# videosegmentation/video_segment

Measured on AMD Instinct MI355X. Metric: over-segmented frames/sec at 1080p, higher is better.
Workload: dtype f32

## Files before the change

include/vsg.h:

```cpp
#ifndef VSG_H_
#define VSG_H_

#include <stddef.h>
#include <stdint.h>

#ifdef __cplusplus
extern "C" {
#endif

#define VSG_OK 0
#define VSG_ERR_INVALID -1
#define VSG_ERR_DEVICE -2
#define VSG_ERR_STATE -3
#define VSG_ERR_INTERNAL -4

#define VSG_MEM_HOST 0
#define VSG_MEM_DEVICE 1

typedef struct vsg_stream vsg_stream;
typedef struct vsg_graph vsg_graph;

typedef struct vsg_options {
  int presmoothing;
  float frac_min_region_size;
  int chunk_size;
  float chunk_overlap_ratio;
  int num_constraint_frames;
  int enforce_n4_connectivity;
  int enforce_spatial_connectedness;
  int color_distance;
  int device;
  int two_stage_oversegment;
  int compute_vectorization;
} vsg_options;

typedef struct vsg_timings {
  float preprocess_ms;
  float edges_ms;
  float sort_ms;
  float merge_ms;
  float readout_ms;
  float host_post_ms;
  int64_t edges_total;
  int64_t edges_active;
  int64_t merges;
  int64_t preprocess_launches;
  int64_t edge_launches;
  float wave_kernel_ms;
  int64_t wave_kernel_launches;
  int64_t wave_kernel_edges;
  float filter_kernel_ms;
  int64_t filter_kernel_launches;
  float spine_kernel_ms;
  int64_t spine_kernel_launches;
  int64_t spine_kernel_edges;
} vsg_timings;

typedef struct vsg_diagnostics {
  double segment_wall_ms;
  double prepare_ms;
  double constrained_merge_ms;
  int64_t stages;
  int64_t optimistic_stages, rollbacks;
  int64_t slab_growths;
  double slab_growth_ms;
  int64_t spine_pool_growths;
  double spine_pool_growth_ms;
  int64_t runtime_mallocs;
  double runtime_malloc_ms;
  int64_t runtime_frees;
  double runtime_free_ms;
  int64_t cache_hits;
  int64_t device_syncs;
  double device_sync_ms;
  int64_t mail_waits;
  double mail_wait_ms;
  double mail_wait_longest_ms;
  int mail_mode;
} vsg_diagnostics;

typedef struct vsg_merge_paths {
  int64_t hub_stages;
  int64_t hub_absorbed;
  int64_t hub_cuts;
  int64_t hub_cuts_in_groups;
  int64_t hub_parts_in_later_bucket;
  int64_t spine_side_cuts;
  int64_t hub_retries;
  int64_t hub_reasons[6];
  int64_t hub_exclusion_reruns;
  int64_t hub_off_reruns;
  int64_t group_halvings;
  int64_t conservative_replays;
} vsg_merge_paths;

typedef struct vsg_spine_paths {
  int64_t replays;
  int64_t components;
  int64_t nested_replays;
  int64_t deepest_level;
  int64_t forest_rounds;
  int64_t forest_rounds_ahead;
  int64_t forest_compactions_ahead;
  int64_t forest_compactions_sync;
  int64_t forest_lists_refused;
  int64_t ranked_by_sampling;
  int64_t ranked_plain;
  int64_t rank_sampling_refused;
  int64_t jump_loops_ended_early;
  int64_t streamed_passes;
  int64_t streamed_refused;
  int64_t pool_fallbacks[4];
  int64_t top_level_fallbacks;
  int64_t nested_fallbacks;
  int64_t assumption_reruns;
  int64_t limit_bucket_moves;
  int64_t low_bucket_failures[2];
  int64_t low_bucket_skips[2];
  int64_t zero_pool_flips;
  int64_t windows_run;
  int64_t rle_stages;
  int64_t wide_launches;
  int64_t group_stages;
  int64_t sorts_hand;
  int64_t sorts_library;
} vsg_spine_paths;

typedef struct vsg_boundary_paths {
  int64_t halo_planes_in_pool;
} vsg_boundary_paths;

typedef struct vsg_memory_stats {
  int64_t bytes_in_use;
  int64_t bytes_in_use_peak;
  int64_t bytes_cached;
  int64_t limit_bytes;
  int64_t runtime_mallocs, runtime_frees, cache_hits, device_syncs;
  double runtime_malloc_ms, runtime_free_ms, device_sync_ms;
} vsg_memory_stats;
int vsg_device_memory_stats(int device, vsg_memory_stats* out);
int vsg_device_memory_trim(int device);
int vsg_device_memory_limit(int device, int64_t bytes);

const char* vsg_last_error(void);
int vsg_version(void);
void vsg_default_options(vsg_options* o);
int vsg_device_count(void);

int vsg_vectorize_id_image(const int32_t* ids, int width, int height, const uint8_t** data,
                           size_t* len);

int vsg_stream_create(const vsg_options* o, int width, int height, vsg_stream** out);
void vsg_stream_destroy(vsg_stream* s);
int vsg_stream_process_frame(vsg_stream* s, int flush, const uint8_t* bgr, size_t stride,
                             const float* flow, int has_flow_stream, int mem, int* num_results);
int vsg_stream_chunk_size(const vsg_stream* s);
int vsg_stream_result_bytes(vsg_stream* s, int i, const uint8_t** data, size_t* len);
int vsg_stream_result_id_image(vsg_stream* s, int i, int32_t* out);
int vsg_stream_last_merge_stats(const vsg_stream* s, int64_t* forced_regular_small);
int vsg_stream_keep_node_states(vsg_stream* s, int on);
int vsg_stream_last_node_states(const vsg_stream* s, int64_t* n, const int32_t** root, const float** mean,
                                const int32_t** size, const int32_t** constraint, const uint8_t** flags);
int vsg_stream_last_timings(const vsg_stream* s, vsg_timings* t);
int vsg_stream_last_diagnostics(const vsg_stream* s, vsg_diagnostics* d);
int vsg_stream_last_merge_paths(const vsg_stream* s, vsg_merge_paths* out);
int vsg_stream_last_spine_paths(const vsg_stream* s, vsg_spine_paths* out);
int vsg_stream_last_boundary_paths(const vsg_stream* s, vsg_boundary_paths* out);
int vsg_stream_last_smoothed(vsg_stream* s, float* out);

int vsg_stream_export_halo(vsg_stream* s, const int32_t** dev_labels_virtual,
                           const int32_t** dev_labels_constrained, int64_t scalars[4]);
int vsg_stream_import_halo(vsg_stream* s, const int32_t* labels_virtual,
                           const int32_t* labels_constrained, int mem, const int64_t scalars[4]);

int vsg_stream_expect_halo(vsg_stream* s);
int vsg_stream_restart(vsg_stream* s);

typedef struct vsg_chain vsg_chain;
int vsg_chain_create(int rank, int world, const char* id_file, uint64_t nonce, int device,
                     vsg_chain** out);
void vsg_chain_destroy(vsg_chain* c);
int vsg_chain_info(const vsg_chain* c, int* rank, int* world);
int vsg_chain_send_halo(vsg_chain* c, vsg_stream* from, int dst);
int vsg_chain_recv_halo(vsg_chain* c, vsg_stream* into, int src);
int vsg_chain_exchange_halo(vsg_chain* c, vsg_stream* from, int dst, vsg_stream* into, int src);

typedef struct vsg_regionseg vsg_regionseg;
typedef struct vsg_regionseg_options {
  int min_region_num;
  int max_region_num;
  float level_cutoff_fraction;
  float small_region_penalizer;
  int luminance_bins;
  int color_bins;
  int flow_bins;
  int chunk_set_size;
  int chunk_set_overlap;
  int constraint_chunks;
  int use_appearance;
  int use_flow;
  int use_size_penalizer;
  int compute_vectorization;
  int save_descriptors;
} vsg_regionseg_options;
void vsg_regionseg_default_options(vsg_regionseg_options* o);
int vsg_regionseg_create(const vsg_regionseg_options* o, int width, int height, vsg_regionseg** out);
void vsg_regionseg_destroy(vsg_regionseg* r);
int vsg_regionseg_process_frame(vsg_regionseg* r, int flush, const uint8_t* seg_desc, size_t seg_len,
                             const uint8_t* bgr, size_t stride, const float* flow, int* num_results);
int vsg_regionseg_result_bytes(vsg_regionseg* r, int i, const uint8_t** data, size_t* len);
int vsg_bgr_to_lab(const uint8_t* bgr, size_t stride, int width, int height, uint8_t* lab);

int vsg_graph_create(int width, int height, int max_frames, int l1, int device, vsg_graph** out);
void vsg_graph_destroy(vsg_graph* g);
int vsg_graph_add_frame_bgr(vsg_graph* g, const uint8_t* bgr, size_t stride, int presmoothing,
                            const int32_t* constraint_ids, int mem);
int vsg_graph_add_frame_features(vsg_graph* g, const float* feat, const int32_t* constraint_ids,
                                 int mem);
int vsg_graph_add_virtual_frame(vsg_graph* g, const int32_t* constraint_ids, int mem);
int vsg_graph_add_temporal(vsg_graph* g, const float* flow, int is_virtual, int mem);
int vsg_graph_add_frame_features_temporal(vsg_graph* g, const float* feat, const int32_t* constraint_ids,
                                          const float* flow, int is_virtual, int mem);
int vsg_graph_finish_building(vsg_graph* g);
int vsg_graph_segment_spatially(vsg_graph* g);
int vsg_graph_segment(vsg_graph* g, int min_region_size, int force_constraints);
int vsg_graph_obtain_results(vsg_graph* g, int use_flows, int enforce_n4,
                             int enforce_spatial_connectedness);
int vsg_graph_num_frames(const vsg_graph* g);
int vsg_graph_num_regions(const vsg_graph* g);
int64_t vsg_graph_num_neighbor_links(const vsg_graph* g);
int vsg_graph_region_sizes(const vsg_graph* g, int32_t* sizes, int32_t* constrained_ids);
int vsg_graph_index_image(const vsg_graph* g, int t, int32_t* out);
typedef struct vsg_region {
  int32_t index, size, constrained_id, first_frame, last_frame;
} vsg_region;
typedef struct vsg_interval {
  int32_t region_index, y, left_x, right_x;
} vsg_interval;
int vsg_graph_get_regions(vsg_graph* g, const vsg_region** regions, size_t* num_regions,
                          const int32_t** nbr_csr_ptr, const int32_t** nbr_csr_idx);
int vsg_graph_get_intervals(vsg_graph* g, int frame, const vsg_interval** intervals, size_t* n);
int vsg_graph_smoothed(vsg_graph* g, int t, float* out );
int vsg_graph_spatial_buckets(vsg_graph* g, int t, uint16_t* out );
int vsg_graph_temporal_buckets(vsg_graph* g, int t, uint16_t* out , int32_t* prev_idx);
int vsg_graph_list_slots(vsg_graph* g, int list, uint32_t* slots_out, int32_t* offsets_out);
// ... 23 lines not shown
```

video_segment_amd/_lib.py:

```python
import ctypes as C
import os
import subprocess

_HERE = os.path.dirname(os.path.abspath(__file__))
CSRC_DIR = os.path.join(_HERE, "csrc")
LIB_PATH = os.path.join(_HERE, "lib", "libvsg_hip.so")

VSG_OK = 0
VSG_ERR_INVALID, VSG_ERR_DEVICE, VSG_ERR_STATE, VSG_ERR_INTERNAL = -1, -2, -3, -4
VSG_MEM_HOST = 0
VSG_MEM_DEVICE = 1


class VsgOptions(C.Structure):
    _fields_ = [
        ("presmoothing", C.c_int),
        ("frac_min_region_size", C.c_float),
        ("chunk_size", C.c_int),
        ("chunk_overlap_ratio", C.c_float),
        ("num_constraint_frames", C.c_int),
        ("enforce_n4_connectivity", C.c_int),
        ("enforce_spatial_connectedness", C.c_int),
        ("color_distance", C.c_int),
        ("device", C.c_int),
        ("two_stage_oversegment", C.c_int),
        ("compute_vectorization", C.c_int),
    ]


class VsgTimings(C.Structure):
    _fields_ = [
        ("preprocess_ms", C.c_float),
        ("edges_ms", C.c_float),
        ("sort_ms", C.c_float),
        ("merge_ms", C.c_float),
        ("readout_ms", C.c_float),
        ("host_post_ms", C.c_float),
        ("edges_total", C.c_int64),
        ("edges_active", C.c_int64),
        ("merges", C.c_int64),
        ("preprocess_launches", C.c_int64),
        ("edge_launches", C.c_int64),
        ("wave_kernel_ms", C.c_float),
        ("wave_kernel_launches", C.c_int64),
        ("wave_kernel_edges", C.c_int64),
        ("filter_kernel_ms", C.c_float),
        ("filter_kernel_launches", C.c_int64),
        ("spine_kernel_ms", C.c_float),
        ("spine_kernel_launches", C.c_int64),
        ("spine_kernel_edges", C.c_int64),
    ]


class VsgDiagnostics(C.Structure):
    _fields_ = [
        ("segment_wall_ms", C.c_double), ("prepare_ms", C.c_double), ("constrained_merge_ms", C.c_double),
        ("stages", C.c_int64), ("optimistic_stages", C.c_int64), ("rollbacks", C.c_int64),
        ("slab_growths", C.c_int64), ("slab_growth_ms", C.c_double),
        ("spine_pool_growths", C.c_int64), ("spine_pool_growth_ms", C.c_double),
        ("runtime_mallocs", C.c_int64), ("runtime_malloc_ms", C.c_double),
        ("runtime_frees", C.c_int64), ("runtime_free_ms", C.c_double),
        ("cache_hits", C.c_int64), ("device_syncs", C.c_int64), ("device_sync_ms", C.c_double),
        ("mail_waits", C.c_int64), ("mail_wait_ms", C.c_double), ("mail_wait_longest_ms", C.c_double),
        ("mail_mode", C.c_int),
    ]

    def as_dict(self):
        return {k: getattr(self, k) for k, _ in self._fields_}


class VsgMergePaths(C.Structure):
    _fields_ = [
        ("hub_stages", C.c_int64), ("hub_absorbed", C.c_int64),
        ("hub_cuts", C.c_int64), ("hub_cuts_in_groups", C.c_int64), ("hub_parts_in_later_bucket", C.c_int64),
        ("spine_side_cuts", C.c_int64),
        ("hub_retries", C.c_int64), ("hub_reasons", C.c_int64 * 6),
        ("hub_exclusion_reruns", C.c_int64), ("hub_off_reruns", C.c_int64),
        ("group_halvings", C.c_int64), ("conservative_replays", C.c_int64),
    ]

    def as_dict(self):
        return {k: (list(getattr(self, k)) if k == "hub_reasons" else getattr(self, k)) for k, _ in self._fields_}


class VsgSpinePaths(C.Structure):
    _fields_ = [
        ("replays", C.c_int64), ("components", C.c_int64), ("nested_replays", C.c_int64),
        ("deepest_level", C.c_int64),
        ("forest_rounds", C.c_int64), ("forest_rounds_ahead", C.c_int64), ("forest_compactions_ahead", C.c_int64),
        ("forest_compactions_sync", C.c_int64), ("forest_lists_refused", C.c_int64),
        ("ranked_by_sampling", C.c_int64), ("ranked_plain", C.c_int64), ("rank_sampling_refused", C.c_int64),
        ("jump_loops_ended_early", C.c_int64), ("streamed_passes", C.c_int64), ("streamed_refused", C.c_int64),
        ("pool_fallbacks", C.c_int64 * 4), ("top_level_fallbacks", C.c_int64), ("nested_fallbacks", C.c_int64),
        ("assumption_reruns", C.c_int64), ("limit_bucket_moves", C.c_int64),
        ("low_bucket_failures", C.c_int64 * 2), ("low_bucket_skips", C.c_int64 * 2),
        ("zero_pool_flips", C.c_int64),
        ("windows_run", C.c_int64), ("rle_stages", C.c_int64), ("wide_launches", C.c_int64),
        ("group_stages", C.c_int64), ("sorts_hand", C.c_int64), ("sorts_library", C.c_int64),
    ]

    def as_dict(self):
        return {k: (list(getattr(self, k)) if issubclass(t, C.Array) else getattr(self, k)) for k, t in self._fields_}


class VsgBoundaryPaths(C.Structure):
    _fields_ = [
        ("halo_planes_in_pool", C.c_int64),
    ]

    def as_dict(self):
        return {k: getattr(self, k) for k, _ in self._fields_}


class VsgMemoryStats(C.Structure):
    _fields_ = [
        ("bytes_in_use", C.c_int64), ("bytes_in_use_peak", C.c_int64), ("bytes_cached", C.c_int64),
        ("limit_bytes", C.c_int64),
        ("runtime_mallocs", C.c_int64), ("runtime_frees", C.c_int64), ("cache_hits", C.c_int64),
        ("device_syncs", C.c_int64),
        ("runtime_malloc_ms", C.c_double), ("runtime_free_ms", C.c_double), ("device_sync_ms", C.c_double),
    ]

    def as_dict(self):
        return {k: getattr(self, k) for k, _ in self._fields_}


class VsgRegionOptions(C.Structure):
    _fields_ = [
        ("min_region_num", C.c_int), ("max_region_num", C.c_int),
        ("level_cutoff_fraction", C.c_float), ("small_region_penalizer", C.c_float),
        ("luminance_bins", C.c_int), ("color_bins", C.c_int), ("flow_bins", C.c_int),
        ("chunk_set_size", C.c_int), ("chunk_set_overlap", C.c_int), ("constraint_chunks", C.c_int),
        ("use_appearance", C.c_int), ("use_flow", C.c_int), ("use_size_penalizer", C.c_int),
        ("compute_vectorization", C.c_int), ("save_descriptors", C.c_int),
    ]


EXPORTED_SYMBOLS = [
    "vsg_last_error", "vsg_version", "vsg_default_options", "vsg_device_count",
    "vsg_device_memory_stats", "vsg_device_memory_trim", "vsg_device_memory_limit",
    "vsg_vectorize_id_image",
    "vsg_stream_create", "vsg_stream_destroy", "vsg_stream_process_frame", "vsg_stream_chunk_size",
    "vsg_stream_result_bytes", "vsg_stream_result_id_image", "vsg_stream_last_merge_stats",
    "vsg_stream_keep_node_states", "vsg_stream_last_node_states",
    "vsg_stream_last_timings", "vsg_stream_last_diagnostics", "vsg_stream_last_merge_paths", "vsg_stream_last_spine_paths",
    "vsg_stream_last_boundary_paths",
    "vsg_stream_last_smoothed", "vsg_stream_export_halo",
    "vsg_stream_import_halo", "vsg_stream_expect_halo", "vsg_stream_restart",
    "vsg_chain_create", "vsg_chain_destroy", "vsg_chain_info", "vsg_chain_send_halo",
    "vsg_chain_recv_halo", "vsg_chain_exchange_halo",
    "vsg_regionseg_default_options", "vsg_regionseg_create", "vsg_regionseg_destroy", "vsg_regionseg_process_frame",
    "vsg_regionseg_result_bytes", "vsg_bgr_to_lab",
    "vsg_graph_create", "vsg_graph_destroy", "vsg_graph_add_frame_bgr",
    "vsg_graph_add_frame_features", "vsg_graph_add_virtual_frame", "vsg_graph_add_temporal",
    "vsg_graph_add_frame_features_temporal", "vsg_graph_list_slots",
    "vsg_graph_finish_building", "vsg_graph_segment_spatially", "vsg_graph_segment", "vsg_graph_obtain_results",
    "vsg_graph_num_frames", "vsg_graph_num_regions", "vsg_graph_num_neighbor_links",
    "vsg_graph_region_sizes", "vsg_graph_index_image", "vsg_graph_get_regions",
    "vsg_graph_get_intervals", "vsg_graph_smoothed",
    "vsg_graph_spatial_buckets", "vsg_graph_temporal_buckets", "vsg_graph_node_roots",
    "vsg_graph_node_states",
    "vsg_graph_merge_stats", "vsg_graph_timings", "vsg_graph_diagnostics", "vsg_graph_merge_paths",
    "vsg_graph_spine_paths",
    "vsg_debug_sort_pairs", "vsg_debug_sort_pairs_timed", "vsg_debug_exclusive_sum", "vsg_debug_runs_of_sorted_keys",
]


def build(force=False):
    subprocess.check_call(["make", "-C", CSRC_DIR, "-j8", "-s"])
    return LIB_PATH


_lib = None


def lib():
    global _lib
    if _lib is not None:
        return _lib
    if not os.path.exists(LIB_PATH):
        raise RuntimeError(
            "libvsg_hip.so is missing (%s): build the HIP extension first; there is no fallback "
            "path" % LIB_PATH)
    try:
        import torch
    except ImportError:
        pass
    L = C.CDLL(LIB_PATH)
    vp = C.c_void_p
    L.vsg_last_error.restype = C.c_char_p
    L.vsg_version.restype = C.c_int
    L.vsg_default_options.argtypes = [C.POINTER(VsgOptions)]
    L.vsg_device_count.restype = C.c_int
    L.vsg_device_memory_stats.argtypes = [C.c_int, C.POINTER(VsgMemoryStats)]
    L.vsg_device_memory_trim.argtypes = [C.c_int]
    L.vsg_device_memory_limit.argtypes = [C.c_int, C.c_int64]
    L.vsg_vectorize_id_image.argtypes = [vp, C.c_int, C.c_int, C.POINTER(vp), C.POINTER(C.c_size_t)]
    L.vsg_stream_create.argtypes = [C.POINTER(VsgOptions), C.c_int, C.c_int, C.POINTER(vp)]
    L.vsg_stream_destroy.argtypes = [vp]
    L.vsg_stream_process_frame.argtypes = [vp, C.c_int, vp, C.c_size_t, vp, C.c_int, C.c_int,
                                           C.POINTER(C.c_int)]
    L.vsg_stream_chunk_size.argtypes = [vp]
    L.vsg_stream_result_bytes.argtypes = [vp, C.c_int, C.POINTER(vp), C.POINTER(C.c_size_t)]
    L.vsg_stream_result_id_image.argtypes = [vp, C.c_int, vp]
    L.vsg_stream_last_merge_stats.argtypes = [vp, vp]
    L.vsg_stream_keep_node_states.argtypes = [vp, C.c_int]
    L.vsg_stream_last_node_states.argtypes = [vp, C.POINTER(C.c_int64)] + [C.POINTER(vp)] * 5
    L.vsg_stream_last_timings.argtypes = [vp, C.POINTER(VsgTimings)]
    L.vsg_stream_last_diagnostics.argtypes = [vp, C.POINTER(VsgDiagnostics)]
    L.vsg_stream_last_merge_paths.argtypes = [vp, C.POINTER(VsgMergePaths)]
    L.vsg_stream_last_spine_paths.argtypes = [vp, C.POINTER(VsgSpinePaths)]
    L.vsg_stream_last_boundary_paths.argtypes = [vp, C.POINTER(VsgBoundaryPaths)]
    L.vsg_stream_last_smoothed.argtypes = [vp, vp]
    L.vsg_stream_export_halo.argtypes = [vp, C.POINTER(vp), C.POINTER(vp), vp]
    L.vsg_stream_import_halo.argtypes = [vp, vp, vp, C.c_int, vp]
    L.vsg_stream_expect_halo.argtypes = [vp]
    L.vsg_stream_restart.argtypes = [vp]
    L.vsg_chain_create.argtypes = [C.c_int, C.c_int, C.c_char_p, C.c_uint64, C.c_int, C.POINTER(vp)]
    L.vsg_chain_info.argtypes = [vp, C.POINTER(C.c_int), C.POINTER(C.c_int)]
    L.vsg_chain_exchange_halo.argtypes = [vp, vp, C.c_int, vp, C.c_int]
    L.vsg_chain_destroy.argtypes = [vp]
    L.vsg_chain_send_halo.argtypes = [vp, vp, C.c_int]
    L.vsg_chain_recv_halo.argtypes = [vp, vp, C.c_int]
    L.vsg_regionseg_default_options.argtypes = [C.POINTER(VsgRegionOptions)]
    L.vsg_regionseg_create.argtypes = [C.POINTER(VsgRegionOptions), C.c_int, C.c_int, C.POINTER(vp)]
    L.vsg_regionseg_destroy.argtypes = [vp]
    L.vsg_regionseg_process_frame.argtypes = [vp, C.c_int, vp, C.c_size_t, vp, C.c_size_t, vp, C.POINTER(C.c_int)]
    L.vsg_regionseg_result_bytes.argtypes = [vp, C.c_int, C.POINTER(vp), C.POINTER(C.c_size_t)]
    L.vsg_bgr_to_lab.argtypes = [vp, C.c_size_t, C.c_int, C.c_int, vp]
    L.vsg_debug_sort_pairs.argtypes = [vp, vp, C.c_int, C.c_int, vp, vp, C.c_int]
    L.vsg_debug_sort_pairs_timed.argtypes = [vp, vp, C.c_int, C.c_int, vp, vp, C.c_int, C.c_int, C.c_int,
# ... 63 lines not shown
```

video_segment_amd/csrc/capi.cpp:

```cpp
#include <algorithm>
#include <cstring>
#include <memory>
#include <string>
#include <vector>

#include <rccl/rccl.h>

#include <chrono>
#include <cstdio>
#include <fstream>
#include <thread>

#include "../../include/vsg.h"
#include "region_segmentation.h"
#include "scan_device.h"
#include "stream.h"

namespace {

thread_local std::string g_last_error;

template <class F>
int Guard(F&& f) {
  try {
    f();
    return VSG_OK;
  } catch (const vsg::Error& e) {
    g_last_error = e.what();
    return e.code;
  } catch (const std::exception& e) {
    g_last_error = e.what();
    return VSG_ERR_INTERNAL;
  }
}

class DeviceGuard {
 public:
  explicit DeviceGuard(int device) {
    if (device < 0) return;
    if (hipGetDevice(&prev_) != hipSuccess) return;
    if (prev_ != device) {
      VSG_HIP(hipSetDevice(device));
      changed_ = true;
    }
  }
  ~DeviceGuard() {
    if (changed_) (void)hipSetDevice(prev_);
  }
  DeviceGuard(const DeviceGuard&) = delete;
  DeviceGuard& operator=(const DeviceGuard&) = delete;

 private:
  int prev_ = -1;
  bool changed_ = false;
};

int ResolveDevice(int device) {
  if (device >= 0) return device;
  int cur = 0;
  VSG_HIP(hipGetDevice(&cur));
  return cur;
}

void RequireDevice(int device) {
  int n = 0;
  hipError_t e = hipGetDeviceCount(&n);
  if (e != hipSuccess || n <= 0) {
    vsg::Throw(VSG_ERR_DEVICE,
               "no usable HIP device (libvsg_hip has no CPU fallback): " +
                   std::string(e != hipSuccess ? hipGetErrorString(e) : "device count is 0"));
  }
  if (device >= n) vsg::Throw(VSG_ERR_DEVICE, "device ordinal out of range");
}

}

struct vsg_stream {
  int device = 0;
  std::unique_ptr<vsg::DenseSegmentationHip> impl;
  std::vector<int32_t> id_image;
};

struct vsg_regionseg {
  std::unique_ptr<vsg::RegionSegmentationHost> impl;
  int W = 0, H = 0;
};

struct vsg_graph {
  int device = 0;
  int W = 0, H = 0;
  size_t wh = 0;
  hipStream_t stream = nullptr;
  std::unique_ptr<vsg::DenseGraphHip> g;
  std::unique_ptr<vsg::Preprocessor> pre;
  std::vector<std::shared_ptr<vsg::DevBuf<float>>> feats;
  std::vector<std::shared_ptr<vsg::DevBuf<float>>> flows_dev;
  vsg::DevBuf<uint8_t> staging_bgr;
  vsg::DevBuf<float> staging_f32;
  vsg::DevBuf<int32_t> staging_ids;
  vsg_timings timings;
  std::vector<vsg_region> out_regions;
  std::vector<int32_t> out_nbr_ptr, out_nbr_idx;
  std::vector<vsg_interval> out_intervals;
  ~vsg_graph() {
    if (stream) (void)hipStreamSynchronize(stream);
    g.reset();
    pre.reset();
    if (stream) (void)hipStreamDestroy(stream);
  }
};

static void FillMergePaths(const vsg::MergePaths& mp, vsg_merge_paths* o) {
  std::memset(o, 0, sizeof(*o));
  o->hub_stages = mp.hub_stages;
  o->hub_absorbed = mp.hub_absorbed;
  o->hub_cuts = mp.hub_cuts;
  o->hub_cuts_in_groups = mp.hub_cuts_in_groups;
  o->hub_parts_in_later_bucket = mp.hub_parts_in_later_bucket;
  o->spine_side_cuts = mp.spine_side_cuts;
  o->hub_retries = mp.hub_retries;
  for (int q = 0; q < 6; ++q) o->hub_reasons[q] = mp.hub_reasons[q];
  o->hub_exclusion_reruns = mp.hub_exclusion_reruns;
  o->hub_off_reruns = mp.hub_off_reruns;
  o->group_halvings = mp.group_halvings;
  o->conservative_replays = mp.conservative_replays;
}

static void FillSpinePaths(const vsg::SpinePaths& sp, vsg_spine_paths* o) {
  std::memset(o, 0, sizeof(*o));
  o->replays = sp.replays;
  o->components = sp.components;
  o->nested_replays = sp.nested_replays;
  o->deepest_level = sp.deepest_level;
  o->forest_rounds = sp.forest_rounds;
  o->forest_rounds_ahead = sp.forest_rounds_ahead;
  o->forest_compactions_ahead = sp.forest_compactions_ahead;
  o->forest_compactions_sync = sp.forest_compactions_sync;
  o->forest_lists_refused = sp.forest_lists_refused;
  o->ranked_by_sampling = sp.ranked_by_sampling;
  o->ranked_plain = sp.ranked_plain;
  o->rank_sampling_refused = sp.rank_sampling_refused;
  o->jump_loops_ended_early = sp.jump_loops_ended_early;
  o->streamed_passes = sp.streamed_passes;
  o->streamed_refused = sp.streamed_refused;
  o->top_level_fallbacks = sp.top_level_fallbacks;
  o->nested_fallbacks = sp.nested_fallbacks;
  o->assumption_reruns = sp.assumption_reruns;
  o->limit_bucket_moves = sp.limit_bucket_moves;
  o->zero_pool_flips = sp.zero_pool_flips;
  o->windows_run = sp.windows_run;
  o->rle_stages = sp.rle_stages;
  o->wide_launches = sp.wide_launches;
  o->group_stages = sp.group_stages;
  o->sorts_hand = sp.sorts_hand;
  o->sorts_library = sp.sorts_library;
  for (int q = 0; q < 4; ++q) o->pool_fallbacks[q] = sp.pool_fallbacks[q];
  for (int q = 0; q < 2; ++q) {
    o->low_bucket_failures[q] = sp.low_bucket_failures[q];
    o->low_bucket_skips[q] = sp.low_bucket_skips[q];
  }
}

static void FillDiagnostics(const vsg::GraphTimings& gt, vsg_diagnostics* d) {
  std::memset(d, 0, sizeof(*d));
  d->segment_wall_ms = gt.segment_wall_ms;
  d->prepare_ms = gt.prepare_ms;
  d->constrained_merge_ms = gt.constrained_merge_ms;
  d->stages = gt.stages;
  d->optimistic_stages = gt.optimistic_stages;
  d->rollbacks = gt.rollbacks;
  d->slab_growths = gt.slab_growths;
  d->slab_growth_ms = gt.slab_growth_ms;
  d->spine_pool_growths = gt.spine_growths;
  d->spine_pool_growth_ms = gt.spine_growth_ms;
  d->runtime_mallocs = gt.runtime_mallocs;
  d->runtime_malloc_ms = gt.runtime_malloc_ms;
  d->runtime_frees = gt.runtime_frees;
  d->runtime_free_ms = gt.runtime_free_ms;
  d->cache_hits = gt.cache_hits;
  d->device_syncs = gt.device_syncs;
  d->device_sync_ms = gt.device_sync_ms;
  d->mail_waits = gt.mail_waits;
  d->mail_wait_ms = gt.mail_wait_ms;
  d->mail_wait_longest_ms = gt.mail_wait_longest_ms;
  d->mail_mode = gt.mail_mode;
}

extern "C" {

const char* vsg_last_error(void) { return g_last_error.c_str(); }

int vsg_device_memory_stats(int device, vsg_memory_stats* out) {
  return Guard([&] {
    VSG_REQUIRE(out, VSG_ERR_INVALID, "null argument");
    const int dev = ResolveDevice(device);
    const vsg::CacheStats s = vsg::CacheGetStats(dev);
    out->bytes_in_use = s.bytes_in_use;
    out->bytes_in_use_peak = s.bytes_in_use_peak;
    out->bytes_cached = s.bytes_cached;
    out->limit_bytes = s.limit_bytes;
    out->runtime_mallocs = s.runtime_mallocs;
    out->runtime_frees = s.runtime_frees;
    out->cache_hits = s.cache_hits;
    out->device_syncs = s.device_syncs;
    out->runtime_malloc_ms = s.runtime_malloc_ms;
    out->runtime_free_ms = s.runtime_free_ms;
    out->device_sync_ms = s.device_sync_ms;
  });
}

int vsg_device_memory_trim(int device) {
  return Guard([&] {
    const int dev = ResolveDevice(device);
    DeviceGuard dg(dev);
    vsg::CacheTrim(dev);
  });
}

int vsg_device_memory_limit(int device, int64_t bytes) {
  return Guard([&] {
    const int dev = ResolveDevice(device);
    DeviceGuard dg(dev);
    vsg::CacheSetLimit(dev, (long long)bytes);
  });
}
int vsg_version(void) { return 100; }

void vsg_default_options(vsg_options* o) {
  o->presmoothing = 2;
  o->frac_min_region_size = 0.01f;
  o->chunk_size = 20;
  o->chunk_overlap_ratio = 0.2f;
  o->num_constraint_frames = 1;
  o->enforce_n4_connectivity = 1;
  o->enforce_spatial_connectedness = 1;
  o->color_distance = 1;
  o->device = -1;
  o->two_stage_oversegment = 0;
  o->compute_vectorization = 0;
}

int vsg_device_count(void) {
  int n = 0;
  if (hipGetDeviceCount(&n) != hipSuccess) return 0;
  return n;
}

int vsg_vectorize_id_image(const int32_t* ids, int width, int height, const uint8_t** data,
                           size_t* len) {
  return Guard([&] {
    VSG_REQUIRE(ids && data && len && width >= 1 && height >= 1, VSG_ERR_INVALID, "bad argument");
    thread_local std::string wire;
    std::vector<std::pair<int32_t, vsg::Interval>> runs;
    for (int y = 0; y < height; ++y) {
      const int32_t* row = ids + (size_t)y * width;
      for (int x = 0; x < width;) {
        int x2 = x;
        while (x2 + 1 < width && row[x2 + 1] == row[x]) ++x2;
        VSG_REQUIRE(row[x] >= 0, VSG_ERR_INVALID, "negative region id");
        runs.emplace_back(row[x], vsg::Interval{y, x, x2});
        x = x2 + 1;
      }
    }
    std::stable_sort(runs.begin(), runs.end(),
                     [](const std::pair<int32_t, vsg::Interval>& a,
                        const std::pair<int32_t, vsg::Interval>& b) { return a.first < b.first; });
    vsg::SegDesc d;
    d.frame_width = width;
    d.frame_height = height;
    for (const auto& r : runs) {
      if (d.regions.empty() || d.regions.back().id != r.first) {
        d.regions.emplace_back();
        d.regions.back().id = r.first;
      }
      d.regions.back().raster.push_back(r.second);
    }
    for (auto& r : d.regions) vsg::MomentsFromRaster(r.raster, &r.moments);
// ... 940 lines not shown
```

video_segment_amd/csrc/dense_graph.cpp:

```cpp
#include "dense_graph.h"
#include "scan_device.h"

#include <algorithm>
#include <chrono>
#include <cmath>
#include <cstring>
#include <atomic>
#include <functional>
#include <thread>
#include <unordered_set>

namespace vsg {

namespace {
template <class T>
DevBuf<T>& Grow(DevBuf<T>& b, size_t n) {
  if (b.size() < n) b.alloc(n + n / 2 + 1024);
  return b;
}
double NowMs() {
  using clk = std::chrono::steady_clock;
  return std::chrono::duration<double, std::milli>(clk::now().time_since_epoch()).count();
}
template <class T>
// ... 326 lines not shown
  min_region_size_ = min_region_size;
  const int L = (int)lists_.size();
  const size_t N = wh_ * (size_t)num_frames_;
  const double t_enter = NowMs();
  const ThreadAllocCounters alloc0 = ThreadAllocSnapshot();
  MailWaitResetLongest();
  const MailWaitCounters mail0 = MailWaitSnapshot();
  int64_t diag_stages = 0, diag_slab_growths = 0, diag_spine_growths = 0, diag_hub_stages = 0, diag_hub_absorbed = 0;
  double diag_slab_ms = 0, diag_spine_ms = 0;

  std::vector<ListDesc> desc(L);
  list_slot_base_.assign(L + 1, 0);
  uint32_t acc = 0;
  int64_t edges_total = 0;
  for (int l = 0; l < L; ++l) {
    ListBuf& lb = lists_[l];
    list_slot_base_[l] = acc;
    ListDesc d = {};
    if (lb.used) {
      d.slots = lb.slots.get();
      d.kept = kept_all_.get() + acc;
      d.prev_idx = lb.type == 1 ? lb.prev_idx.get() : nullptr;
      d.offsets = (pass == 1 && lb.type == 1) ? nullptr : lb.offsets.get();
      d.type = lb.type;
      d.base_a = lb.base_a;
      d.base_b = lb.base_b;
      d.n = lb.n;
      acc += (uint32_t)lb.n;
    }
    desc[l] = d;
  }
  list_slot_base_[L] = acc;
  H2D(list_desc_dev_.get(), desc.data(), (size_t)L, stream_);
  H2D(list_slot_base_dev_.get(), list_slot_base_.data(), (size_t)L + 1, stream_);
  if (pass == 2) {
    kept_spatial_pass_.ensure(kept_all_.size());
    VSG_HIP(hipMemcpyAsync(kept_spatial_pass_.get(), kept_all_.get(), acc, hipMemcpyDeviceToDevice,
                           stream_));
  }
  VSG_HIP(hipMemsetAsync(kept_all_.get(), 0, acc, stream_));
  LaunchBuildBucketTable(list_desc_dev_.get(), L, bucket_base_dev_.get(), stream_);
  bucket_base_host_.resize((size_t)(kNumBuckets + 1) * (L + 1));
  D2H(bucket_base_host_.data(), bucket_base_dev_.get(), bucket_base_host_.size(), stream_);
  VSG_HIP(hipMemsetAsync(stats_.get(), 0, 96 * sizeof(unsigned long long), stream_));
  VSG_HIP(hipMemsetAsync(zero_pool_.base, 0, zero_pool_.cap * sizeof(int32_t), stream_));
  zero_pool_.used = 0;
  zero_pool_.second_half = false;
  zero_pool_.arena_used = 0;
  LaunchInitIdentity(cc_.get(), N, stream_);
  VSG_HIP(hipStreamSynchronize(stream_));

  const bool group_buckets = !getenv("VSG_GROUP_BUCKETS") || atoi(getenv("VSG_GROUP_BUCKETS")) != 0;
  std::vector<int32_t> bucket_prefix(kNumBuckets + 2, 0);
  int first_plain = kNumBuckets;
  {
    const float scale = 2048.0f / (1.0f + 1e-6f);
    const float inv_scale = (float)(1.0 / (double)scale);
    const float force_w = l1_ ? 0.002f : 0.001f;
    for (int b = 0; b < kNumBuckets; ++b) {
      if (!((float)b * inv_scale < force_w)) {
        first_plain = b;
        break;
      }
    }
  }
  int64_t n_max = 0;
  for (int b = 0; b <= kNumBuckets; ++b) {
    const int tot = bucket_base_host_[(size_t)b * (L + 1) + L];
    edges_total += tot;
    bucket_prefix[b + 1] = bucket_prefix[b] + tot;
  }
  for (int b = 0; b < kNumBuckets; ++b) n_max = std::max<int64_t>(n_max, bucket_prefix[b + 1] - bucket_prefix[b]);
  VSG_REQUIRE(bucket_prefix[kNumBuckets] >= 0, -1, "too many edges");
  EnsureScratch((size_t)std::max<int64_t>(n_max, 1));
  if (const char* e = getenv("VSG_ACTIVE_CAP")) {
    EnsureActiveScratch((size_t)std::max(1, atoi(e)));
  } else {
    EnsureActiveScratch(std::min<size_t>((size_t)std::max<int64_t>(n_max, 1),
                                         std::max<size_t>((size_t)n_max / 6, (size_t)1 << 20)));
  }
  bucket_prefix_dev_.ensure(bucket_prefix.size());
  H2D(bucket_prefix_dev_.get(), bucket_prefix.data(), bucket_prefix.size(), stream_);

  MergeScratch S = {};
  auto bind_scratch = [this, &S]() {
    S.e_ra = e_ra_.get();
    S.e_rb = e_rb_.get();
    S.e_gpos = e_gpos_.get();
    S.e_active = act_.e_active;
    S.e_apos = act_.e_apos;
    S.a_ra = act_.a_ra;
    S.a_rb = act_.a_rb;
    S.a_gpos = act_.a_gpos;
    S.a_comp = act_.a_comp;
    S.a_idx = act_.a_idx;
    S.s_comp = act_.s_comp;
    S.s_idx = act_.s_idx;
    S.seg_key = act_.seg_key;
    S.seg_cnt = act_.seg_cnt;
    S.seg_off = act_.seg_off;
    S.lead_pos = act_.lead_pos;
    S.l_ra = act_.l_ra;
    S.l_rb = act_.l_rb;
    S.l_gpos = act_.l_gpos;
    S.bk_ds = act_.bk_ds;
    S.bk_cons = act_.bk_cons;
    S.bk_flags = act_.bk_flags;
    S.cub_temp = cub_temp_.get();
    S.cub_temp_bytes = cub_temp_.size();
    S.scan = ScanScratch{scan_sums_.get(), stream_};
    S.active_cap = (int)std::min<size_t>(scratch_active_, 0x7fffffff);
  };
  bind_scratch();
  S.grow_active = [this, bind_scratch, &diag_slab_growths, &diag_slab_ms](long long need) {
    const double tg0 = NowMs();
    VSG_HIP(hipStreamSynchronize(stream_));
    VSG_HIP(hipStreamSynchronize(aux_stream_));
    VSG_HIP(hipStreamSynchronize(aux2_stream_));
    const size_t before = scratch_active_;
    EnsureActiveScratch((size_t)need);
    bind_scratch();
    ++diag_slab_growths;
    diag_slab_ms += NowMs() - tg0;
    if (getenv("VSG_DEBUG_STATS")) {
      std::fprintf(stderr, "[vsg] stage scratch: %zu -> %zu active edges (needed %lld), %.2f ms\n", before,
                   scratch_active_, need, NowMs() - tg0);
    }
    return true;
  };
  S.num_active = scalars_.get();
  S.num_segs = scalars_.get() + 1;
  S.node_key_bits = 1;
  while (S.node_key_bits < 32 && ((size_t)1 << S.node_key_bits) < N) ++S.node_key_bits;
  {
    const size_t words = 4 * ((scratch_edges_ + 255) / 256) + 4;
    S.masks.active = filter_masks_.get();
    S.masks.settled = filter_masks_.get() + words;
    S.masks.tentative = filter_masks_.get() + 2 * words;
    S.masks.block_cnt = block_cnt_.get();
    S.block_off = block_off_.get();
  }
  S.force_rollback = getenv("VSG_FORCE_ROLLBACK") ? 1 : 0;
  S.small_seg = getenv("VSG_SMALL_SEG") ? std::max(1, atoi(getenv("VSG_SMALL_SEG"))) : 24;
  S.wide_min = getenv("VSG_WIDE_MIN") ? atoi(getenv("VSG_WIDE_MIN")) : 0;
  S.wide_waves = getenv("VSG_WIDE_WAVES") ? atoi(getenv("VSG_WIDE_WAVES")) : 4;
  S.chain_relax = getenv("VSG_CHAIN_RELAX") ? atoi(getenv("VSG_CHAIN_RELAX")) : 1;
  const int hubs_default = getenv("VSG_HUBS") ? atoi(getenv("VSG_HUBS")) : 1;
  S.hubs = hubs_default;
  S.hub_excl = hub_excl_.get();
  S.hub_max_splits = getenv("VSG_HUB_SPLITS") ? std::max(0, atoi(getenv("VSG_HUB_SPLITS"))) : kHubMaxSplits;
  S.hub_cut_min_work = getenv("VSG_CUT_MIN_WORK") ? atoi(getenv("VSG_CUT_MIN_WORK")) : 0;
  S.hub_cut_ratio = getenv("VSG_CUT_RATIO") ? std::max(0, atoi(getenv("VSG_CUT_RATIO"))) : 1500;
  S.hub_check = (getenv("VSG_HUB_CHECK") && atoi(getenv("VSG_HUB_CHECK")) != 0) ? 1 : 0;
  VSG_HIP(hipMemsetAsync(hub8_.get(), 0, N, stream_));
  S.spine_min = getenv("VSG_SPINE_MIN") ? atoi(getenv("VSG_SPINE_MIN")) : 2048;
  if (S.spine_min > 0) S.spine_min = std::max(S.spine_min, S.small_seg + 2);
  {
    const double want = 1.15 * (double)wh_ * (double)capacity_frames_;
    const int by_graph = (int)std::min<double>(std::max<double>(want, 1 << 20), 120 << 20);
    S.spine_max_edges = getenv("VSG_SPINE_MAX_EDGES") ? atoi(getenv("VSG_SPINE_MAX_EDGES"))
                                                      : std::max(by_graph, spine_max_edges_grown_);
  }
  S.spine_off = 0;
  if (spine_limit_bucket_ != 0x7fffffff && ++spine_limit_age_ > 8) {
    spine_limit_bucket_ = 0x7fffffff;
    spine_limit_age_ = 0;
  }
  S.spine_limit_bucket = &spine_limit_bucket_;
  int spine_low_failed[2] = {0, 0}, spine_low_skip[2] = {0, 0};
  for (int b = 0; b < 2; ++b) {
    if (spine_low_cooldown_[b] > 0) {
      --spine_low_cooldown_[b];
      spine_low_skip[b] = 1;
      ++S.sp.low_bucket_skips[b];
    }
  }
  S.spine_low_failed = spine_low_failed;
  S.spine_low_skip = spine_low_skip;
  S.spine_nested_factor = getenv("VSG_SPINE_NESTED") ? std::max(1, atoi(getenv("VSG_SPINE_NESTED"))) : 1;
  S.spine_debug = getenv("VSG_SPINE_DEBUG") ? 1 : 0;
  S.spine_check = getenv("VSG_SPINE_CHECK") ? 1 : 0;
  S.rank_split_min = getenv("VSG_RANK_SPLIT_MIN") ? atoi(getenv("VSG_RANK_SPLIT_MIN")) : (1 << 20);
  S.spine_fast = getenv("VSG_SPINE_FAST") ? atoi(getenv("VSG_SPINE_FAST")) : 2;
  S.spine_fast_min = getenv("VSG_SPINE_FAST_MIN") ? atoi(getenv("VSG_SPINE_FAST_MIN")) : 32768;
  if (S.spine_min > 0) {
    const size_t ints = SpinePoolInts((size_t)S.spine_max_edges);
    if (spine_pool_.size() < ints) spine_pool_.alloc(ints);
  }
  S.spine_pool = spine_pool_.get();
  S.spine_pool_ints = spine_pool_.size();
  S.grow_spine_pool = [this, &S, &diag_spine_growths, &diag_spine_ms](long long edges) {
    if (getenv("VSG_SPINE_MAX_EDGES") || edges >= (120ll << 20)) return false;
    const long long want = std::min<long long>(edges + edges / 8, 120ll << 20);
    const long long nodes = (long long)wh_ * (long long)std::max(capacity_frames_, 1);
    const size_t ints = SpinePoolInts((size_t)want) + (size_t)(29 * std::min(want, nodes));
    if (ints <= spine_pool_.size()) return false;
    const double tg0 = NowMs();
    size_t free_b = 0, total_b = 0;
    VSG_HIP(hipMemGetInfo(&free_b, &total_b));
    if (free_b + spine_pool_.size() * sizeof(int32_t) < 2 * ints * sizeof(int32_t)) {
      int dev = 0;
      VSG_HIP(hipGetDevice(&dev));
      CacheTrim(dev);
      VSG_HIP(hipMemGetInfo(&free_b, &total_b));
      if (free_b + spine_pool_.size() * sizeof(int32_t) < 2 * ints * sizeof(int32_t)) return false;
    }
    VSG_HIP(hipStreamSynchronize(stream_));
    VSG_HIP(hipStreamSynchronize(aux_stream_));
    VSG_HIP(hipStreamSynchronize(aux2_stream_));
    spine_pool_.alloc(ints);
    ++diag_spine_growths;
    diag_spine_ms += NowMs() - tg0;
    S.spine_pool = spine_pool_.get();
    S.spine_pool_ints = spine_pool_.size();
    S.spine_max_edges = (int)want;
    spine_max_edges_grown_ = S.spine_max_edges;
    return true;
  };
  S.nmap[0] = label_uf_.get();
  S.nmap[1] = label_img_.get();
  S.nmap[2] = adjust_.get();
  S.aux_stream = aux_stream_;
  S.aux2_stream = aux2_stream_;
  S.aux_fork = aux_fork_;
  S.aux_join = aux_join_;
  S.use_rle = getenv("VSG_RLE") ? atoi(getenv("VSG_RLE")) : 1;
  S.wave_dbg = getenv("VSG_WAVE_DBG") ? atoi(getenv("VSG_WAVE_DBG")) : 0;
  S.wave_debug = (S.wave_dbg != 0 || getenv("VSG_DEBUG_STAGES") || getenv("VSG_DEBUG_STATS")) ? 1 : 0;
  optimistic_stages_ = 0;
  rollbacks_ = 0;
  S.optimistic_stages = &optimistic_stages_;
  S.rollbacks = &rollbacks_;
  S.cc = cc_.get();
  S.stats = stats_.get();
  ev_used_ = 0;
  ev_wave_.clear();
  ev_filter_.clear();
  ev_spine_.clear();
  S.ev_pool = &ev_pool_;
  S.ev_wave = &ev_wave_;
  S.ev_filter = &ev_filter_;
  S.ev_spine = &ev_spine_;
  S.ev_used = &ev_used_;
  S.mail = &mail_;
  S.zeros = &zero_pool_;
  S.main_stream = stream_;

  MergeParams P;
  P.spatial_survivors = pass == 2 ? kept_spatial_pass_.get() : nullptr;
  P.W = W_;
  P.H = H_;
  P.num_lists = L;
  P.min_region_size = min_region_size;
  P.force_merge_weight = l1_ ? 0.002f : 0.001f;
  const float scale = 2048.0f / (1.0f + 1e-6f);
  P.inv_scale = (float)(1.0 / (double)scale);
  auto largest_s = [](double t, bool inclusive) {
    auto ok = [&](float s) {
      const double r = (double)std::sqrt(s);
      return inclusive ? r <= t : r < t;
    };
    float s = (float)(t * t);
    while (!ok(s)) s = std::nextafter(s, 0.0f);
    while (ok(std::nextafter(s, 10.0f))) s = std::nextafter(s, 10.0f);
    return s;
  };
  P.s_lt_005 = largest_s((double)0.05f, false);
  P.s_lt_02 = largest_s(0.2, false);
  P.s_le_015 = largest_s((double)0.15f, true);

  const double t0 = NowMs();
  int inert_mode = has_constraints_ ? 2 : 1;
  if (const char* e = getenv("VSG_INERT_MODE")) inert_mode = std::min(inert_mode, atoi(e));
  const bool debug_stages = getenv("VSG_DEBUG_STAGES") != nullptr;
  const double frame_ratio = (double)W_ * (double)H_ / (1920.0 * 1080.0);
  const int default_windows = std::max(6, std::min(12, (int)std::lround(6.0 * frame_ratio)));
  const int num_windows = getenv("VSG_WINDOWS") ? std::max(1, atoi(getenv("VSG_WINDOWS"))) : default_windows;
  const int window_bushy = getenv("VSG_WINDOW_BUSHY") ? atoi(getenv("VSG_WINDOW_BUSHY")) : 64;
  const bool adapt_windows = !getenv("VSG_ADAPT_WINDOWS") || atoi(getenv("VSG_ADAPT_WINDOWS")) != 0;
  const int window_min_edges =
      getenv("VSG_WINDOW_MIN") ? atoi(getenv("VSG_WINDOW_MIN")) : (int)std::min<size_t>(2 * wh_, 1u << 30);
  const int window_min_replayed =
      getenv("VSG_WINDOW_MIN_REPLAYED") ? atoi(getenv("VSG_WINDOW_MIN_REPLAYED"))
                                        : (getenv("VSG_WINDOW_MIN") ? 0 : (int)std::min<size_t>(wh_ / 2, 1u << 30));
  S.bucket_prefix = bucket_prefix_dev_.get();
  S.bucket_prefix_host = bucket_prefix.data();
  {
    list_off_host_.assign((size_t)L * (kNumBuckets + 2), 0);
    for (int l = 0; l < L; ++l) {
      int32_t* off = list_off_host_.data() + (size_t)l * (kNumBuckets + 2);
      int acc_l = 0;
      for (int b = 0; b <= kNumBuckets; ++b) {
        off[b] = acc_l;
        const int32_t* row = bucket_base_host_.data() + (size_t)b * (L + 1);
        acc_l += row[l + 1] - row[l];
      }
      off[kNumBuckets + 1] = acc_l;
    }
    const size_t cap = (size_t)3 * 65536;
    if (seg_table_dev_.size() < cap) seg_table_dev_.alloc(cap);
    S.filter_segs_mode = getenv("VSG_FILTER_SEGS") ? atoi(getenv("VSG_FILTER_SEGS")) : 2;
    S.bucket_base_host = S.filter_segs_mode == 0 ? nullptr : bucket_base_host_.data();
    S.lists_host = desc.data();
    S.list_off_host = list_off_host_.data();
    S.list_slot_base_host = list_slot_base_.data();
    S.seg_dev = seg_table_dev_.get();
// ... 104 lines not shown
      return want;
    };
    const bool big_enough = n_b >= (1 << 18);
    int pos = 0;
    for (int w = 0; w < windows && pos < n_b; ++w) {
      const int j1 = (int)((int64_t)n_b * (w + 1) / windows);
      if (j1 <= pos) continue;
      const bool probe = windows > 1 && w == 0 && window_bushy > 0;
      bool rest_mode = false;
      while (pos < j1) {
        bool limited = false;
        const int take = (int)limit(j1 - pos, &limited);
        const StageInfo info = run(w, pos, take,
                                   probe ? 2 : ((big_enough && (limited || windows == 1)) ||
                                                wave_target_active_ != kNoWindowTarget) ? 1 : 0, limited);
        pos += take;
        if (probe && ((int64_t)info.replayed >= (int64_t)window_bushy * std::max(info.components, 1) ||
                      info.replayed < (int64_t)window_min_replayed * take / std::max(j1, 1))) {
          rest_mode = true;
        }
      }
      if (rest_mode) {
        const int64_t rest_default = std::min<int64_t>(
            119ll << 20, std::max<int64_t>(16ll << 20, (int64_t)(1.4 * (double)wh_ * (double)capacity_frames_)));
        const int64_t rest_cap = getenv("VSG_REST_CAP") ? atoll(getenv("VSG_REST_CAP")) : rest_default;
        const int64_t rest_n = (int64_t)n_b - pos;
        const int pieces = (int)std::max<int64_t>(1, (rest_n + rest_cap - 1) / rest_cap);
        const int64_t piece = (rest_n + pieces - 1) / pieces;
        for (int q = 0; pos < n_b; ++q) {
          bool limited = false;
          const int take = (int)limit(std::min<int64_t>(piece, n_b - pos), &limited);
          run(-1 - q, pos, take, big_enough ? 1 : 0, limited);
          pos += take;
        }
      }
    }
    window_target_[b] = wave_target_active_;
    if (hub_bucket_stages_[b] > 0 && hub_bucket_absorbed_[b] < hub_bucket_stages_[b]) hub_bucket_pause_[b] = 8;
    if (debug_stages && wave_target_active_ != kNoWindowTarget) {
      std::fprintf(stderr, "[vsg]   bucket %d leaves target %lld (frozen %d, unpaid %d, last %d, peak %d)\n", b,
                   (long long)wave_target_active_, (int)window_frozen_[b], (int)window_unpaid_[b], window_last_seg_[b],
                   window_peak_[b]);
    }
    if (b >= first_plain) {
      if (group_active < 2048) {
        group_width = std::min(group_width * 4, 512);
      } else if (group_active > 16384) {
        group_width = std::max(group_width / 4, 1);
      }
    }
  }
  for (int b = 0; b < 2; ++b) {
    if (++spine_low_cost_age_[b] > 64) {
      spine_low_cost_age_[b] = 0;
      spine_low_cost_fail_[b] = spine_low_cost_skip_[b] = 0;
    }
    if (spine_low_skip[b]) {
      spine_low_cost_skip_[b] = low_bucket_ms[b];
      if (spine_low_cost_fail_[b] > 0 && spine_low_cost_skip_[b] >= spine_low_cost_fail_[b]) spine_low_cooldown_[b] = 0;
      continue;
    }
    if (spine_low_failed[b]) spine_low_cost_fail_[b] = low_bucket_ms[b];
    spine_low_fails_[b] = spine_low_failed[b] ? spine_low_fails_[b] + 1 : 0;
    if (spine_low_fails_[b] >= 2) {
      spine_low_fails_[b] = 0;
      if (spine_low_cost_skip_[b] <= 0) {
        spine_low_cooldown_[b] = 1;
      } else if (spine_low_cost_skip_[b] < spine_low_cost_fail_[b]) {
        spine_low_cooldown_[b] = 8;
      }
    }
  }
  timings_.optimistic_stages = optimistic_stages_;
  timings_.rollbacks = rollbacks_;
  LaunchKeepVirtualBucket(list_desc_dev_.get(), L, stream_);
  ResetHubExclusions(S, nodes(), stream_);
  VSG_HIP(hipStreamSynchronize(stream_));
  const double t_buckets = NowMs();
  if (getenv("VSG_DEBUG_HASH")) DebugHash("after buckets");
  if (force_constraints && has_constraints_) MergeConstrainedHostAssisted();
  if (getenv("VSG_DEBUG_HASH")) DebugHash("after constrained merge");
  const double t_mc = NowMs();
  if (getenv("VSG_DEBUG_STATS")) {
    std::fprintf(stderr, "[vsg] segment: buckets %.1f ms, merge-constrained %.1f ms\n",
                 t_buckets - t0, t_mc - t_buckets);
  }
  unsigned long long st[80] = {0};
  D2H(st, stats_.get(), 80, stream_);
  VSG_HIP(hipStreamSynchronize(stream_));
  if (st[23] != 0) {
    std::fprintf(stderr, "[vsg] chain self check: %llu mismatches\n", st[23]);
    throw Error(-4 , "merge worker: the chain self check found mismatches");
  }
  if (st[22] != 0) throw Error(-4 , "merge worker: a batch did not converge");
  if (getenv("VSG_DEBUG_STATS")) {
    std::fprintf(stderr, "[vsg] wave: edges %llu batches %llu rounds %llu generic %llu (solo %llu) chain %llu "
                 "cuts %llu; optimistic stages %lld rollbacks %lld\n",
                 st[3], st[7], st[5], st[4], st[6], st[20], st[21], (long long)optimistic_stages_,
                 (long long)rollbacks_);
    std::fprintf(stderr, "[vsg] hubs: %lld stages used hub regions, %lld regions absorbed through them, %lld stages cut at an edge, %lld redone "
                 "(broken %lld, inherit %lld, shape %lld, marked %lld, pair %lld, split %lld)\n",
                 (long long)diag_hub_stages, (long long)diag_hub_absorbed, S.hub_splits, S.hub_retries, S.hub_reasons[0],
                 S.hub_reasons[1], S.hub_reasons[2], S.hub_reasons[3], S.hub_reasons[4], S.hub_reasons[5]);
    std::fprintf(stderr, "[vsg] wide: edges %llu batches %llu (%.1f lanes each) rounds %llu (%.1f per batch), chain lanes %llu, "
                 "kept-lane iterations %llu; kcyc per batch: staging %.1f rounds %.1f (%.2f per round)\n",
                 st[31], st[45], (double)st[72] / std::max(1.0, (double)st[45]), st[44],
                 (double)st[44] / std::max(1.0, (double)st[45]), st[73], st[74],
                 st[46] / 1e3 / std::max(1.0, (double)st[45]), st[47] / 1e3 / std::max(1.0, (double)st[45]),
                 st[47] / 1e3 / std::max(1.0, (double)st[44]));
  }
  timings_.merge_ms = (float)(NowMs() - t0);
  for (auto& pr : ev_wave_) {
    float ms = 0;
    VSG_HIP(hipEventElapsedTime(&ms, ev_pool_[pr.first], ev_pool_[pr.second]));
    timings_.wave_ms += ms;
  }
  for (auto& pr : ev_filter_) {
    float ms = 0;
    VSG_HIP(hipEventElapsedTime(&ms, ev_pool_[pr.first], ev_pool_[pr.second]));
    timings_.filter_ms += ms;
  }
  for (auto& pr : ev_spine_) {
    float ms = 0;
    VSG_HIP(hipEventElapsedTime(&ms, ev_pool_[pr.first], ev_pool_[pr.second]));
    timings_.spine_ms += ms;
  }
  timings_.spine_launches += (int64_t)ev_spine_.size();
  timings_.spine_edges += (int64_t)st[24];
  timings_.wave_launches += (int64_t)ev_wave_.size();
  timings_.filter_launches += (int64_t)ev_filter_.size();
  timings_.wave_edges += (int64_t)st[3];
  timings_.edges_active += (int64_t)st[3];
  timings_.edges_total = edges_total;
  timings_.merges[0] += (int64_t)st[0];
  timings_.merges[1] += (int64_t)st[1];
  timings_.merges[2] += (int64_t)st[2];
  {
    const ThreadAllocCounters a1 = ThreadAllocSnapshot();
    const MailWaitCounters m1 = MailWaitSnapshot();
    timings_.stages = diag_stages;
    MergePaths& mp = timings_.paths;
    mp = MergePaths();
    mp.hub_stages = diag_hub_stages;
    mp.hub_absorbed = diag_hub_absorbed;
    mp.hub_cuts = S.hub_splits;
    mp.hub_cuts_in_groups = S.hub_cuts_in_groups;
    mp.hub_parts_in_later_bucket = S.hub_parts_in_later_bucket;
    mp.spine_side_cuts = S.spine_side_cuts;
    mp.hub_retries = S.hub_retries;
    for (int q = 0; q < 6; ++q) mp.hub_reasons[q] = S.hub_reasons[q];
    mp.hub_exclusion_reruns = S.hub_exclusion_reruns;
    mp.hub_off_reruns = S.hub_off_reruns;
    mp.group_halvings = S.group_halvings;
    mp.conservative_replays = S.conservative_replays;
    timings_.spine_paths = S.sp;
    timings_.slab_growths = diag_slab_growths;
    timings_.slab_growth_ms = diag_slab_ms;
    timings_.spine_growths = diag_spine_growths;
    timings_.spine_growth_ms = diag_spine_ms;
    timings_.runtime_mallocs = a1.runtime_mallocs - alloc0.runtime_mallocs;
    timings_.runtime_malloc_ms = a1.runtime_malloc_ms - alloc0.runtime_malloc_ms;
    timings_.runtime_frees = a1.runtime_frees - alloc0.runtime_frees;
    timings_.runtime_free_ms = a1.runtime_free_ms - alloc0.runtime_free_ms;
    timings_.cache_hits = a1.cache_hits - alloc0.cache_hits;
    timings_.device_syncs = a1.device_syncs - alloc0.device_syncs;
    timings_.device_sync_ms = a1.device_sync_ms - alloc0.device_sync_ms;
    timings_.mail_waits = m1.waits - mail0.waits;
    timings_.mail_wait_ms = m1.wait_ms - mail0.wait_ms;
    timings_.mail_wait_longest_ms = m1.longest_ms;
    timings_.mail_mode = MailYieldMode();
    timings_.prepare_ms = t0 - t_enter;
    timings_.constrained_merge_ms = t_mc - t_buckets;
    timings_.segment_wall_ms = NowMs() - t_enter;
  }
}

namespace {
struct SimRegion {
  int parent;
  float d[3];
  int sz, cons, flags;
  bool dirty;
};
}

void DenseGraphHip::DebugHash(const char* where) {
  const size_t N = wh_ * (size_t)num_frames_;
  std::vector<int32_t> parent(N), cons(N);
  std::vector<float4> ds(N);
  std::vector<uint8_t> flags(N);
  D2H(parent.data(), parent_.get(), N, stream_);
  D2H(cons.data(), cons_.get(), N, stream_);
  D2H(ds.data(), desc_sz_.get(), N, stream_);
  D2H(flags.data(), flags_.get(), N, stream_);
  VSG_HIP(hipStreamSynchronize(stream_));
  auto fnv = [](uint64_t h, const void* p, size_t n) {
    const uint8_t* b = static_cast<const uint8_t*>(p);
    for (size_t i = 0; i < n; ++i) { h ^= b[i]; h *= 1099511628211ull; }
    return h;
  };
  std::vector<int32_t> root(N), canon(N, -1);
  uint64_t h_part = 1469598103934665603ull, h_root = h_part, h_state = h_part, h_cons = h_part;
  int next = 0, nroots = 0;
  for (size_t i = 0; i < N; ++i) {
    int r = (int)i;
    while (parent[(size_t)r] != r) r = parent[(size_t)r];
    root[i] = r;
    if (canon[(size_t)r] < 0) canon[(size_t)r] = next++;
    const int32_t c = canon[(size_t)r];
    h_part = fnv(h_part, &c, 4);
    h_root = fnv(h_root, &r, 4);
  }
  for (size_t i = 0; i < N; ++i) {
    if (parent[i] != (int)i) continue;
    ++nroots;
    h_state = fnv(h_state, &ds[i], 16);
    h_state = fnv(h_state, &flags[i], 1);
    h_cons = fnv(h_cons, &cons[i], 4);
  }
  std::fprintf(stderr, "[vsg] hash %s: roots %d partition %016llx root-ids %016llx states %016llx cons %016llx\n",
               where, nroots, (unsigned long long)h_part, (unsigned long long)h_root,
               (unsigned long long)h_state, (unsigned long long)h_cons);
}

void DenseGraphHip::MergeConstrainedHostAssisted() {
  const int N = (int)(wh_ * (size_t)num_frames_);
  std::vector<std::pair<int, int>> vranges;
  for (int t : virtual_slices_) vranges.emplace_back((int)(wh_ * t), (int)(wh_ * (t + 1)));
  std::sort(vranges.begin(), vranges.end());
  std::vector<std::pair<int, int>> nvranges;
  int cursor = 0;
  for (auto& vr : vranges) {
    if (vr.first > cursor) nvranges.emplace_back(cursor, vr.first);
    cursor = vr.second;
  }
  if (cursor < N) nvranges.emplace_back(cursor, N);

  int32_t* d_flags = label_uf_.get();
  int32_t* d_vals = label_img_.get();
  int32_t* d_offs = adjust_.get();
  struct Runs {
    std::vector<int32_t> node, value;
  };
  auto collect = [&](int begin, int end, Runs* out) {
    const int n = end - begin;
    if (n <= 0) return;
    LaunchConstrainedRuns(nodes(), begin, end, d_vals, d_flags, stream_);
    ExclusiveSum(ScanScratch{scan_sums_.get()}, d_flags, d_offs, n, stream_);
    int last_off = 0, last_flag = 0;
    D2H(&last_off, d_offs + (n - 1), 1, stream_);
    D2H(&last_flag, d_flags + (n - 1), 1, stream_);
    VSG_HIP(hipStreamSynchronize(stream_));
    const int k = last_off + last_flag;
    const size_t old = out->node.size();
    if (k > 0) {
      EnsureActiveScratch((size_t)k);
      LaunchCompactIndexValue(d_flags, d_offs, d_vals, n, act_.a_ra, act_.a_rb, stream_);
      out->node.resize(old + k);
      out->value.resize(old + k);
      D2H(out->node.data() + old, act_.a_ra, (size_t)k, stream_);
      D2H(out->value.data() + old, act_.a_rb, (size_t)k, stream_);
      VSG_HIP(hipStreamSynchronize(stream_));
      for (size_t i = old; i < old + (size_t)k; ++i) out->node[i] += begin;
    }
    out->node.push_back(end);
    out->value.push_back(-1);
  };

  const double tm0 = NowMs();
  Runs nv, vr;
  for (auto& r : nvranges) collect(r.first, r.second, &nv);
  for (auto& r : vranges) collect(r.first, r.second, &vr);
  const double tm1 = NowMs();

  std::vector<int32_t> ids;
  {
    std::unordered_set<int32_t> seen;
    for (const Runs* v : {&nv, &vr}) {
      for (int32_t r : v->value) {
        if (r >= 0 && seen.insert(r).second) ids.push_back(r);
      }
    }
    std::sort(ids.begin(), ids.end());
  }
  const int m = (int)ids.size();
  if (m == 0) return;
  small_i32_a_.ensure((size_t)m);
  small_i32_b_.ensure((size_t)m);
  small_i32_c_.ensure((size_t)m);
  small_f4_.ensure((size_t)m);
  H2D(small_i32_a_.get(), ids.data(), (size_t)m, stream_);
  LaunchGatherStates(nodes(), small_i32_a_.get(), m, small_f4_.get(), small_i32_b_.get(),
                     small_i32_c_.get(), stream_);
  std::vector<float4> h_ds(m);
  std::vector<int32_t> h_cons(m), h_flags(m);
  D2H(h_ds.data(), small_f4_.get(), (size_t)m, stream_);
  D2H(h_cons.data(), small_i32_b_.get(), (size_t)m, stream_);
  D2H(h_flags.data(), small_i32_c_.get(), (size_t)m, stream_);
  VSG_HIP(hipStreamSynchronize(stream_));

  const double tm2 = NowMs();
  std::unordered_map<int, SimRegion> sim;
  sim.reserve((size_t)m * 2);
  for (int i = 0; i < m; ++i) {
    SimRegion r;
    r.parent = ids[i];
// ... 769 lines not shown
```

video_segment_amd/csrc/dense_graph.h:

```cpp
#ifndef VSG_DENSE_GRAPH_H_
#define VSG_DENSE_GRAPH_H_

#include <memory>
#include <unordered_map>
#include <vector>

#include "device_graph.h"
#include "host_model.h"

namespace vsg {

struct MergePaths {
  int64_t hub_stages = 0, hub_absorbed = 0;
  int64_t hub_cuts = 0, hub_cuts_in_groups = 0, hub_parts_in_later_bucket = 0, spine_side_cuts = 0;
  int64_t hub_retries = 0, hub_reasons[6] = {0, 0, 0, 0, 0, 0};
  int64_t hub_exclusion_reruns = 0, hub_off_reruns = 0, group_halvings = 0, conservative_replays = 0;
};

struct GraphTimings {
  float edges_ms = 0, sort_ms = 0, merge_ms = 0, readout_ms = 0, host_post_ms = 0;
  int64_t edges_total = 0, edges_active = 0;
  int64_t merges[3] = {0, 0, 0};
  float wave_ms = 0, filter_ms = 0, spine_ms = 0;
  int64_t wave_launches = 0, filter_launches = 0, wave_edges = 0, spine_launches = 0, spine_edges = 0;
  int64_t optimistic_stages = 0, rollbacks = 0;
  int64_t stages = 0;
  int64_t slab_growths = 0, spine_growths = 0;
  double slab_growth_ms = 0, spine_growth_ms = 0;
  int64_t runtime_mallocs = 0, runtime_frees = 0, cache_hits = 0, device_syncs = 0;
  double runtime_malloc_ms = 0, runtime_free_ms = 0, device_sync_ms = 0;
  int64_t mail_waits = 0;
  double mail_wait_ms = 0, mail_wait_longest_ms = 0;
  int mail_mode = 0;
  double segment_wall_ms = 0, prepare_ms = 0, constrained_merge_ms = 0;
  MergePaths paths;
  SpinePaths spine_paths = {};
};

class DenseGraphHip {
 public:
  DenseGraphHip(int W, int H, int max_frames, bool l1, hipStream_t stream);
  ~DenseGraphHip();

  int W() const { return W_; }
  int H() const { return H_; }
  int max_frames() const { return max_frames_; }
  int num_frames() const { return num_frames_; }
  hipStream_t stream() const { return stream_; }
  hipStream_t aux_stream() const { return aux_stream_; }

  void Reset(int max_frames);
  void ForgetLearned();

  void AddFrame(const float* feat_planar_dev, const int32_t* cons_dev);
  void AddVirtualFrame(const int32_t* ids_dev, int max_label);
  void AddVirtualFrameDeferred();
  void SetHaloLabels(const int32_t* virtual_ids_dev, const int32_t* constrained_ids_dev,
                     int max_label);
  bool halo_pending() const { return halo_pending_; }
  void AddTemporal(const float* cur_dev, const float* prev_dev, const float* flow_dev,
                   bool is_virtual);
  void AddFrameAndTemporal(const float* feat_planar_dev, const int32_t* cons_dev, const float* prev_dev,
                           const float* flow_dev, bool is_virtual);
  void FinishBuilding();
  void Segment(int min_region_size, bool force_constraints) {
    SegmentLists(min_region_size, force_constraints, spatial_pass_done_ ? 2 : 0);
  }
  void SegmentSpatially() {
    SegmentLists(0, false, 1);
    spatial_pass_done_ = true;
  }
  void ObtainResults(const std::vector<const float*>* dev_flows, bool enforce_n4,
                     bool enforce_spatial_connectedness);

  std::vector<RegionInfo>& regions() { return regions_; }
  const std::vector<RegionInfo>& regions() const { return regions_; }
  const GraphTimings& timings() const { return timings_; }

  void CopySpatialBuckets(int t, uint16_t* out_host);
  void CopyTemporalBuckets(int t, uint16_t* out_host, int32_t* prev_idx_host);
  void CopyNodeRoots(int32_t* out_host);
  int CopyListSlots(int list, uint32_t* slots_host, int32_t* offsets_host);
  void CopyNodeStates(int32_t* root, float* mean, int32_t* size, int32_t* cons, uint8_t* flags);

 private:
  struct ListBuf {
    DevBuf<uint32_t> slots;
    DevBuf<int32_t> offsets;
    DevBuf<int32_t> prev_idx;
    DevBuf<uint16_t> keys_dbg;
    int type = 0;
    int n = 0;
    int base_a = 0, base_b = 0;
    bool used = false;
  };

  void EnsureScratch(size_t n_edges_max);
  void EnsureActiveScratch(size_t n_active_max);
  void DebugHash(const char* where);
  ListBuf& PrepareSpatialList(const float* feat, const int32_t* cons_dev);
  ListBuf& PrepareTemporalList(const float* cur, const float* prev, const float* flow, bool is_virtual);
  EdgeSortList SortEntry(ListBuf& lb, int per_px);
  void MergeConstrainedHostAssisted();
  NodeArrays nodes() {
    return NodeArrays{parent_.get(), desc_sz_.get(), cons_.get(), flags_.get(), hub8_.get()};
  }

  QuiesceGuard quiesce_;
  int W_, H_, capacity_frames_, max_frames_;
  bool l1_;
  hipStream_t stream_;
  hipStream_t aux_stream_ = nullptr;
  hipStream_t aux2_stream_ = nullptr;
  hipEvent_t aux_fork_ = nullptr, aux_join_ = nullptr;
  int num_frames_ = 0;
  size_t wh_;
  bool has_constraints_ = false;
  std::vector<int> virtual_slices_;
  int min_region_size_ = 0;
  bool flattened_ = false;

  DevBuf<int32_t> parent_;
  DevBuf<float4> desc_sz_;
  DevBuf<int32_t> cons_;
  DevBuf<uint8_t> flags_;
  DevBuf<uint8_t> hub8_;
  DevBuf<int32_t> cc_, label_uf_, label_img_, adjust_;
  std::vector<ListBuf> lists_;
  DevBuf<ListDesc> list_desc_dev_;
  DevBuf<uint32_t> list_slot_base_dev_;
  std::vector<uint32_t> list_slot_base_;
  DevBuf<uint8_t> kept_all_;
  DevBuf<uint8_t> kept_spatial_pass_;
  bool spatial_pass_done_ = false;
  bool halo_pending_ = false;
  int deferred_virtual_slice_ = -1, deferred_constrained_slice_ = -1;
  void SegmentLists(int min_region_size, bool force_constraints, int pass);
  void RunStageDebug(int b, int w, int windows, int j0, int n, const MergeParams& P, int inert_mode,
                     MergeScratch& S, bool debug_stages, StageInfo* info);
  DevBuf<int32_t> bucket_base_dev_;
  std::vector<int32_t> bucket_base_host_;
  DevBuf<uint16_t> keys_tmp_[2];
  DevBuf<int32_t> hist_tmp_[2], hist_chunk_[2];
  DevBuf<int32_t> first_label_scratch_;
  DevBuf<int32_t> e_ra_, e_rb_;
  DevBuf<uint32_t> e_gpos_;
  DevBuf<uint8_t> active_slab_;
  struct ActiveArrays {
    int32_t *e_active = nullptr, *e_apos = nullptr, *a_ra = nullptr, *a_rb = nullptr, *seg_cnt = nullptr,
            *seg_off = nullptr, *lead_pos = nullptr, *l_ra = nullptr, *l_rb = nullptr, *bk_cons = nullptr;
    uint32_t *a_gpos = nullptr, *a_comp = nullptr, *a_idx = nullptr, *s_comp = nullptr, *s_idx = nullptr,
             *seg_key = nullptr, *l_gpos = nullptr;
    float4* bk_ds = nullptr;
    uint8_t* bk_flags = nullptr;
  } act_;
  DevBuf<unsigned long long> filter_masks_;
  DevBuf<int32_t> block_cnt_, block_off_;
  int64_t optimistic_stages_ = 0, rollbacks_ = 0;
  DevBuf<int32_t> scalars_;
  DevBuf<int32_t> seg_table_dev_;
  DevBuf<int32_t> hub_excl_;
  PinnedBuf<int32_t> iv_host_;
  std::vector<int32_t> seg_table_host_, list_off_host_;
  size_t stage_ring_used_ = 0;
  PinnedBuf<int32_t> stage_ring_;
  Mailbox mail_;
  void* mail_mem_ = nullptr;
  DevBuf<int32_t> zero_pool_mem_;
  ZeroPool zero_pool_;
// ... 54 lines not shown
```

video_segment_amd/csrc/device_graph.h:

```cpp
#ifndef VSG_DEVICE_GRAPH_H_
#define VSG_DEVICE_GRAPH_H_

#include <functional>

#include "common.h"

namespace vsg {

constexpr uint8_t kFlagFinalized = 1;
constexpr uint8_t kFlagNoDesc = 2;
constexpr uint8_t kFlagTentative = 4;
constexpr uint8_t kFlagHub = 8;
constexpr uint8_t kFlagHubBroken = 16;
constexpr uint8_t kFlagHubExcluded = 32;
constexpr int kHubExclCap = 16384;
constexpr int kHubMaxAttempts = 4;
constexpr int kHubMaxSplits = 64;
constexpr int kHubCutCap = 64;
constexpr int kHubListInts = 4 + kHubExclCap + 3 * kHubCutCap;

struct NodeArrays {
  int32_t* parent;
  float4* desc_sz;
  int32_t* cons;
  uint8_t* flags;
  uint8_t* hub8;
};

struct ListDesc {
  const uint32_t* slots;
  uint8_t* kept;
  const int32_t* prev_idx;
  const int32_t* offsets;
  int32_t type;
  int32_t base_a;
  int32_t base_b;
  int32_t n;
};

struct MergeParams {
  int W, H;
  int num_lists;
  int min_region_size;
  float force_merge_weight;
  float inv_scale;
  float s_lt_005, s_lt_02, s_le_015;
  const uint8_t* spatial_survivors;
};

void UploadSpaceWeights(const float* w49, hipStream_t stream);
void LaunchMinMax(const uint8_t* bgr, size_t stride, int W, int H, int* mm, hipStream_t s);
void LaunchBilateral(const uint8_t* bgr, size_t stride, int W, int H, const float* lut,
                     float scale, float* planes, hipStream_t s);
void LaunchGaussian3(const uint8_t* bgr, size_t stride, int W, int H, float k0, float k1, float* planes,
                     hipStream_t s);
void LaunchConvertPlanar(const uint8_t* bgr, size_t stride, int W, int H, float* planes,
                         hipStream_t s);
void LaunchInterleavedToPlanar(const float* in, size_t n, float* planes, hipStream_t s);
void LaunchPlanarToInterleaved(const float* planes, size_t n, float* out, hipStream_t s);
size_t EdgeSortHistInts(size_t n_px, int per_px);
size_t EdgeSortChunkInts(size_t n_px, int per_px);
struct EdgeSortList {
  const uint16_t* keys;
  int32_t* hist;
  int32_t* chunk;
  int32_t* offsets;
  uint32_t* slots;
  int per_px;
};
constexpr int kEdgeSortMaxLists = 2;
void LaunchSpatialKeys(const float* feat, int W, int H, int l1, uint16_t* keys, int32_t* hist,
                       hipStream_t s);
void LaunchTemporalKeys(const float* cur, const float* prev, const float* flow, int W, int H,
                        int l1, int is_virtual, uint16_t* keys, int32_t* prev_idx, int32_t* hist,
                        hipStream_t s);
void LaunchBucketSort(const EdgeSortList* lists, int n_lists, size_t n_px, hipStream_t s);
void LaunchInitNodes(const float* feat, size_t n, int base, const int32_t* cons_in,
                     NodeArrays nodes, hipStream_t s);
void LaunchInitVirtualNodes(const int32_t* labels, size_t n, int base, int num_labels,
                            int32_t* first_scratch, NodeArrays nodes, hipStream_t s);

constexpr int kScanMaxTiles = 4096;
struct ScanScratch {
  int32_t* sums;
  hipStream_t owner = nullptr;
};

void DebugExclusiveSum(const ScanScratch& sc, const int32_t* in, int32_t* out, int n, int32_t* total, hipStream_t s);

size_t SortPairsU32HandTempBytes(int n);
void SortPairsU32Hand(void* temp, size_t temp_bytes, const uint32_t* keys_in, uint32_t* keys_out,
                      const uint32_t* vals_in, uint32_t* vals_out, int n, int end_bit, hipStream_t s);
size_t SortPairsU32LibTempBytes(int n);
void SortPairsU32Lib(void* temp, size_t temp_bytes, const uint32_t* keys_in, uint32_t* keys_out,
                     const uint32_t* vals_in, uint32_t* vals_out, int n, int end_bit, hipStream_t s);
size_t SortPairsU32TempBytes(int n);
void SortPairsU32(void* temp, size_t temp_bytes, const uint32_t* keys_in, uint32_t* keys_out,
                  const uint32_t* vals_in, uint32_t* vals_out, int n, int end_bit, hipStream_t s);
bool SortPairsU32TakesHand(int n);
size_t SortKeysU64TempBytes(int n);
void SortKeysU64(void* temp, size_t temp_bytes, const unsigned long long* in,
                 unsigned long long* out, int n,
                 hipStream_t s);
size_t UniqueU64TempBytes(int n);
void UniqueU64(void* temp, size_t temp_bytes, const unsigned long long* in,
               unsigned long long* out,
               int32_t* num_out, int n, hipStream_t s);

constexpr int kMailValues = 4;
struct MailSlot {
  unsigned long long* dev;
  volatile unsigned long long* host;
  unsigned seq;
};
struct Mailbox {
  unsigned long long* dev = nullptr;
  volatile unsigned long long* host = nullptr;
  int slots = 0;
  int next = 0;
  unsigned seq = 0;
  int32_t* list_dev = nullptr;
  volatile int32_t* list_host = nullptr;
  int list_cap = 0;
};
inline MailSlot NextMail(Mailbox& m) {
  MailSlot s{m.dev + (size_t)kMailValues * m.next, m.host + (size_t)kMailValues * m.next, ++m.seq};
  m.next = (m.next + 1) % m.slots;
  return s;
}
void MailWait(const MailSlot& slot, int count, int* values, hipStream_t s);
void MailRegisterGraph(int delta);
int MailYieldMode();
struct MailWaitCounters {
  long long waits = 0;
  double wait_ms = 0, longest_ms = 0;
};
MailWaitCounters MailWaitSnapshot();
void MailWaitResetLongest();
void LaunchMailPost(const MailSlot& slot, const int32_t* p0, const int32_t* p1, const int32_t* p2,
                    const int32_t* p3, hipStream_t s);

constexpr size_t kZeroArenaInts = 1024;
struct ZeroPool {
  int32_t* base = nullptr;
  size_t cap = 0, used = 0;
  bool second_half = false;
  size_t arena_used = 0;
};

struct FilterMasks {
  unsigned long long* active;
  unsigned long long* settled;
  unsigned long long* tentative;
  int32_t* block_cnt;
};
struct FilterSegRec {
  const uint32_t* slots;
  const int32_t* prev;
  int32_t start, pos0, type, base_a, base_b;
  uint32_t slot_base;
};
constexpr int kFilterArgSegs = 64;
struct FilterSegArgs {
  FilterSegRec r[kFilterArgSegs];
};
struct FilterSegs {
  const FilterSegRec* rec;
  int n;
};
constexpr size_t kStageRingInts = (size_t)1 << 18;
struct SpinePaths {
  int64_t replays, components, nested_replays, deepest_level;
  int64_t forest_rounds, forest_rounds_ahead, forest_compactions_ahead, forest_compactions_sync, forest_lists_refused;
  int64_t ranked_by_sampling, ranked_plain, rank_sampling_refused;
  int64_t jump_loops_ended_early, streamed_passes, streamed_refused;
  int64_t pool_fallbacks[4], top_level_fallbacks, nested_fallbacks;
  int64_t assumption_reruns, limit_bucket_moves, low_bucket_failures[2], low_bucket_skips[2];
  int64_t zero_pool_flips;
  int64_t windows_run, rle_stages, wide_launches, group_stages, sorts_hand, sorts_library;
};
struct MergeScratch {
  int active_cap;
  std::function<bool(long long need)> grow_active;
  int32_t* e_ra;
  int32_t* e_rb;
  uint32_t* e_gpos;
  int32_t* e_active;
  int32_t* e_apos;
  FilterMasks masks;
  int32_t* block_off;
  int32_t* a_ra;
  int32_t* a_rb;
  uint32_t* a_gpos;
  uint32_t* a_comp;
  uint32_t* a_idx;
  uint32_t* s_comp;
  uint32_t* s_idx;
  uint32_t* seg_key;
  int32_t* seg_cnt;
  int32_t* seg_off;
  int32_t* num_active;
  int32_t* num_segs;
  float4* bk_ds;
  int32_t* bk_cons;
  uint8_t* bk_flags;
  int force_rollback;
  int32_t* lead_pos;
  int32_t* l_ra;
  int32_t* l_rb;
  uint32_t* l_gpos;
  int use_rle;
  int group_hi;
  const int32_t* bucket_prefix;
  const int32_t* bucket_prefix_host;
  const int32_t* bucket_base_host;
  const int32_t* list_off_host;
  int32_t* seg_dev;
  size_t seg_cap;
  std::vector<int32_t>* seg_host;
  const ListDesc* lists_host;
  int filter_segs_mode;
  int32_t* ring_host;
  size_t ring_cap, *ring_used;
  int spine_min;
  int spine_off;
  int* spine_low_failed;
  const int* spine_low_skip;
  int* spine_limit_bucket;
  int spine_nested_factor;
  int spine_max_edges;
  int spine_debug, spine_check;
  int rank_split_min;
  int spine_fast;
  int spine_fast_min;
  int32_t* spine_pool;
  size_t spine_pool_ints;
  std::function<bool(long long edges)> grow_spine_pool;
  int32_t* nmap[3];
  hipStream_t aux_stream;
  hipStream_t aux2_stream;
  hipEvent_t aux_fork, aux_join;
  int small_seg;
  int wide_min;
  int wide_waves;
  int chain_relax;
  int hubs;
  int hubs_off;
  int hub_attempt;
  int hub_splits_left;
  int hub_split_depth;
  int hub_list_dirty;
  int hub_max_splits;
  int hub_cut_min_work;
  long long hub_splits;
  const uint32_t* list_slot_base_host;
  int32_t* hub_excl;
  long long hub_retries;
  long long hub_reasons[6];
  long long hub_cuts_in_groups;
  long long hub_parts_in_later_bucket;
  long long spine_side_cuts;
  long long hub_exclusion_reruns;
  long long hub_off_reruns;
  long long group_halvings;
  long long conservative_replays;
  long long hub_cut_ratio;
  int hub_check;
  SpinePaths sp;
  int wave_debug;
  int wave_dbg;
  int64_t* optimistic_stages;
  int64_t* rollbacks;
  int32_t* cc;
  unsigned long long* stats;
  void* cub_temp;
  size_t cub_temp_bytes;
  ScanScratch scan;
  int node_key_bits;
  std::vector<hipEvent_t>* ev_pool;
  std::vector<std::pair<int, int>>* ev_wave;
  std::vector<std::pair<int, int>>* ev_filter;
  std::vector<std::pair<int, int>>* ev_spine;
  int* ev_used;
  Mailbox* mail;
  ZeroPool* zeros;
  hipStream_t main_stream;
};
int32_t* TakeZeroed(MergeScratch& S, size_t n);

int32_t* TakeStageScalars(MergeScratch& S, size_t n);

int32_t* TakeStageRing(MergeScratch& S, size_t n);

void LaunchBuildBucketTable(const ListDesc* lists, int num_lists, int32_t* bucket_base,
                            hipStream_t s);
void LaunchInitIdentity(int32_t* a, size_t n, hipStream_t s);
struct StageInfo {
  int want_components = 0;
  int replayed = 0;
  int components = 0;
  int max_wave_segment = 0;
  int hub_stages = 0;
  long long hub_absorbed = 0;
  int hub_retries = 0;
};
void ResetHubExclusions(MergeScratch& S, NodeArrays nodes, hipStream_t s);
void RunBucketStage(int bucket, int j0, int n_b, const ListDesc* lists, const int32_t* bucket_base,
                    const uint32_t* list_slot_base, uint8_t* kept_all, NodeArrays nodes,
                    const MergeParams& P, int inert_mode, MergeScratch& S, hipStream_t s,
                    StageInfo* info = nullptr);
size_t SpinePoolInts(size_t max_edges);
void LaunchKeepVirtualBucket(const ListDesc* lists, int num_lists, hipStream_t s);

void LaunchFlatten(NodeArrays nodes, size_t n, int32_t* label_uf, hipStream_t s);
void LaunchEnforceN4(int32_t* label_img, int W, int H, const int32_t* frames_dev, int num_frames,
                     int32_t* row_flags , int32_t* adjust ,
                     hipStream_t s);
void LaunchRowRunCounts(const int32_t* label_img, int W, int H, const int32_t* frames_dev, int num_frames,
                        int32_t* row_counts , hipStream_t s);
struct IntervalArrays {
  int32_t* label;
  uint32_t* ty;
  int32_t* lx;
  int32_t* rx;
};
void LaunchWriteIntervals(const int32_t* label_img, int W, int H, const int32_t* frames_dev, int num_frames,
                          const int32_t* row_offsets ,
                          IntervalArrays out, hipStream_t s);
void LaunchRelabelIntervals(const uint32_t* ty, const int32_t* lx, const int32_t* rx,
                            const int32_t* new_label, int n, int W, int H, int32_t* label_uf,
                            hipStream_t s);
struct PairTable {
  unsigned long long* key;
  unsigned long long* order;
  unsigned mask;
};
void LaunchNeighborPairsHashed(const ListDesc* lists, int num_lists, const int32_t* label_uf, int W,
                               PairTable table, int32_t* distinct, hipStream_t s);
void LaunchPairTableCompact(PairTable table, unsigned long long* pairs, unsigned long long* order_keys,
                            int32_t* out_count, hipStream_t s);
void LaunchNeighborPairs(const ListDesc* lists, int num_lists, const int32_t* label_uf, int W,
                         unsigned long long* pairs, unsigned long long* order_keys,
                         int32_t* count, int capacity, hipStream_t s);
void LaunchGatherStates(NodeArrays nodes, const int32_t* ids, int n, float4* desc_sz_out,
                        int32_t* cons_out, int32_t* flags_out, hipStream_t s);
void LaunchScatterStates(NodeArrays nodes, const int32_t* ids, int n, const int32_t* parent_in,
                         const float4* desc_sz_in, const int32_t* cons_in, const int32_t* flags_in,
                         hipStream_t s);
void LaunchConstrainedRoots(NodeArrays nodes, int begin, int end, int32_t* flag_out,
                            int32_t* root_out, hipStream_t s);
void LaunchConstrainedRuns(NodeArrays nodes, int begin, int end, int32_t* value_out,
                           int32_t* flag_out, hipStream_t s);
void LaunchCompactI32(const int32_t* flags, const int32_t* offsets, const int32_t* values, int n,
                      int32_t* out, hipStream_t s);
void LaunchGatherI32(const int32_t* src, const int32_t* idx, int n, int32_t* out, hipStream_t s);
void LaunchGatherFlow(const int32_t* req, int n, const float* const* flows, int W, float2* out,
                      hipStream_t s);

void LaunchNonzeroFlags(const int32_t* a, int n, int32_t* flags, hipStream_t s);
void LaunchCompactIndexValue(const int32_t* flags, const int32_t* offsets, const int32_t* values,
                             int n, int32_t* out_idx, int32_t* out_val, hipStream_t s);
void LaunchFirstOrderOfKeys(const unsigned long long* pairs, const unsigned long long* order_keys,
                            int m, const int32_t* keys_sorted, int num_keys,
                            unsigned long long* out_min, hipStream_t s);

}

#endif
```

video_segment_amd/csrc/merge_stage.hip:

```cpp
#include <sched.h>
#include <time.h>

#include <algorithm>
#include <atomic>
#include <chrono>
#include <cstring>
#include <thread>
#include <type_traits>
#include <vector>

#include "merge_common.h"
#include "scan_device.h"

namespace vsg {

__global__ __launch_bounds__(256) void k_build_bucket_table(const ListDesc* __restrict__ lists,
                                                             int num_lists,
                                                             int32_t* __restrict__ bucket_base) {
  const int b = blockIdx.x * 256 + threadIdx.x;
  if (b > kNumBuckets) return;
  int acc = 0;
  int32_t* row = bucket_base + (size_t)b * (num_lists + 1);
  for (int l = 0; l < num_lists; ++l) {
    row[l] = acc;
// ... 12 lines not shown

__global__ __launch_bounds__(256) void k_init_identity(int32_t* a, size_t n) {
  const size_t i = (size_t)blockIdx.x * 256 + threadIdx.x;
  if (i < n) a[i] = (int32_t)i;
}

void LaunchInitIdentity(int32_t* a, size_t n, hipStream_t s) {
  hipLaunchKernelGGL(k_init_identity, dim3((unsigned)((n + 255) / 256)), dim3(256), 0, s, a, n);
  VSG_HIP(hipGetLastError());
}

__global__ void k_mail_post(unsigned long long* slot, unsigned seq, const int32_t* p0, const int32_t* p1,
                            const int32_t* p2, const int32_t* p3) {
  if (p0) MailPost(slot, seq, 0, *p0);
  if (p1) MailPost(slot, seq, 1, *p1);
  if (p2) MailPost(slot, seq, 2, *p2);
  if (p3) MailPost(slot, seq, 3, *p3);
}

void LaunchMailPost(const MailSlot& slot, const int32_t* p0, const int32_t* p1, const int32_t* p2,
                    const int32_t* p3, hipStream_t s) {
  hipLaunchKernelGGL(k_mail_post, dim3(1), dim3(1), 0, s, slot.dev, slot.seq, p0, p1, p2, p3);
  VSG_HIP(hipGetLastError());
}

static std::atomic<int> g_live_graphs{0};
void MailRegisterGraph(int delta) { g_live_graphs.fetch_add(delta, std::memory_order_relaxed); }

static int UsableCores() {
  cpu_set_t set;
  CPU_ZERO(&set);
  if (sched_getaffinity(0, sizeof(set), &set) == 0 && CPU_COUNT(&set) > 0) return (int)CPU_COUNT(&set);
  const unsigned h = std::thread::hardware_concurrency();
  return h ? (int)h : 1;
}

int MailYieldMode() {
  if (const char* e = getenv("VSG_MAIL_YIELD")) return std::max(0, std::min(2, atoi(e)));
  return 2 * g_live_graphs.load(std::memory_order_relaxed) > UsableCores() ? 1 : 0;
}

static thread_local MailWaitCounters t_mail_counters;
MailWaitCounters MailWaitSnapshot() { return t_mail_counters; }
void MailWaitResetLongest() { t_mail_counters.longest_ms = 0; }

namespace {
struct MailWaitTimer {
  std::chrono::steady_clock::time_point t0 = std::chrono::steady_clock::now();
  ~MailWaitTimer() {
    const double ms = std::chrono::duration<double, std::milli>(std::chrono::steady_clock::now() - t0).count();
    t_mail_counters.waits += 1;
    t_mail_counters.wait_ms += ms;
    if (ms > t_mail_counters.longest_ms) t_mail_counters.longest_ms = ms;
  }
};
}

void MailWait(const MailSlot& slot, int count, int* values, hipStream_t s) {
  using clk = std::chrono::steady_clock;
  MailWaitTimer wait_timer;
  clk::time_point t0;
  bool timed = false;
  const int mode = MailYieldMode();
  constexpr unsigned long long kBriefSpins = 512;
  long sleep_ns = 20000;
  for (int i = 0; i < count; ++i) {
    for (unsigned long long spins = 0;; ++spins) {
      const unsigned long long w = slot.host[i];
      if ((unsigned)(w >> 32) == slot.seq) {
        values[i] = (int)(unsigned)(w & 0xffffffffull);
        break;
      }
#if defined(__x86_64__)
      __builtin_ia32_pause();
#endif
      if (mode != 0 && spins >= kBriefSpins) {
        if (mode == 1) {
          std::this_thread::yield();
        } else {
          const timespec ts = {0, sleep_ns};
          nanosleep(&ts, nullptr);
          sleep_ns = std::min(sleep_ns * 2, 200000l);
        }
      }
      if ((mode == 0 && (spins & 0xffffull) == 0xffffull) || (mode != 0 && (spins & 0x3ffull) == 0x3ffull)) {
        const hipError_t e = hipStreamQuery(s);
        if (e != hipSuccess && e != hipErrorNotReady) VSG_HIP(e);
        if (!timed) {
          t0 = clk::now();
          timed = true;
        } else if (e == hipSuccess && clk::now() - t0 > std::chrono::seconds(2)) {
          const unsigned long long w2 = slot.host[i];
          if ((unsigned)(w2 >> 32) != slot.seq) throw Error(-4 , "mailbox: a value never arrived");
        }
        if (mode == 0) std::this_thread::yield();
      }
    }
  }
}

static void DrainStreams(MergeScratch& S) {
  VSG_HIP(hipStreamSynchronize(S.main_stream));
  if (S.aux_stream) VSG_HIP(hipStreamSynchronize(S.aux_stream));
  if (S.aux2_stream) VSG_HIP(hipStreamSynchronize(S.aux2_stream));
}

int32_t* TakeZeroed(MergeScratch& S, size_t n) {
  ZeroPool& z = *S.zeros;
  n = (n + 3) & ~(size_t)3;
  VSG_REQUIRE(z.cap > 2 * kZeroArenaInts, -4, "zero pool: too small");
  const size_t half = (z.cap - kZeroArenaInts) / 2;
  VSG_REQUIRE(n <= half, -4, "zero pool: request too large");
  if (z.used + n > half) {
    DrainStreams(S);
    z.second_half = !z.second_half;
    z.used = 0;
    ++S.sp.zero_pool_flips;
    VSG_HIP(hipMemsetAsync(z.base + kZeroArenaInts + (z.second_half ? half : 0), 0, half * sizeof(int32_t),
                           S.main_stream));
  }
  int32_t* p = z.base + kZeroArenaInts + (z.second_half ? half : 0) + z.used;
  z.used += n;
  return p;
}

int32_t* TakeStageScalars(MergeScratch& S, size_t n) {
  ZeroPool& z = *S.zeros;
  n = (n + 3) & ~(size_t)3;
  VSG_REQUIRE(n <= kZeroArenaInts, -4, "zero pool: stage scalars too large");
  if (z.arena_used + n > kZeroArenaInts) {
    DrainStreams(S);
    VSG_HIP(hipMemsetAsync(z.base, 0, kZeroArenaInts * sizeof(int32_t), S.main_stream));
    z.arena_used = 0;
  }
  int32_t* p = z.base + z.arena_used;
  z.arena_used += n;
  return p;
}

int32_t* TakeStageRing(MergeScratch& S, size_t n) {
  n = (n + 15) & ~(size_t)15;
  if (!S.ring_host || n > S.ring_cap) return nullptr;
  if (*S.ring_used + n > S.ring_cap) {
    DrainStreams(S);
    *S.ring_used = 0;
  }
  int32_t* p = S.ring_host + *S.ring_used;
  *S.ring_used += n;
  return p;
}

constexpr int kFilterPer = 2;
constexpr int kFilterEdges = 256 * kFilterPer;

template <bool kArgs>
__global__ __launch_bounds__(256) void k_filter(int bucket, int bucket_hi, int j0, int n_b,
                                                 const ListDesc* __restrict__ lists,
                                                 const int32_t* __restrict__ bucket_base,
                                                 const int32_t* __restrict__ bucket_prefix,
                                                 const uint32_t* __restrict__ list_slot_base,
                                                 uint8_t* __restrict__ kept_all, NodeArrays nodes,
                                                 MergeParams P, int inert_mode,
                                                 int32_t* __restrict__ cc,
                                                 int32_t* __restrict__ e_ra,
                                                 int32_t* __restrict__ e_rb,
                                                 uint32_t* __restrict__ e_gpos,
                                                 FilterMasks M,
                                                 int32_t* __restrict__ num_ti, FilterSegs segs,
                                                 std::conditional_t<kArgs, FilterSegArgs, int> A, int hubs,
                                                 int32_t* __restrict__ num_hub, int32_t* __restrict__ hub_excl,
                                                 float split_s) {
  constexpr int kSegCap = kArgs ? 1 : kFilterEdges;
  __shared__ int wave_cnt[kFilterPer][4], wave_kept[kFilterPer][4];
  __shared__ int s_start[kSegCap], s_pos0[kSegCap];
  __shared__ const uint32_t* s_slots[kSegCap];
  __shared__ const int32_t* s_prev[kSegCap];
  __shared__ int s_type[kSegCap], s_base_a[kSegCap], s_base_b[kSegCap];
  __shared__ uint32_t s_slot_base[kSegCap];
  const int jf = blockIdx.x * kFilterEdges;
  const bool have_segs = kArgs || segs.rec != nullptr;
  int m_segs = 0;
  if constexpr (!kArgs) {
    if (segs.rec) {
      int first = 0;
      if (segs.n > kFilterEdges) {
        const int stride = (segs.n + 255) / 256;
        const int t1 = threadIdx.x * stride;
        const int c1 = __syncthreads_count(t1 < segs.n && segs.rec[t1].start <= jf);
        const int base = (c1 - 1) * stride;
        const int t2 = base + threadIdx.x;
        const int c2 = __syncthreads_count(threadIdx.x < stride && t2 < segs.n && segs.rec[t2].start <= jf);
        first = base + c2 - 1;
      }
      m_segs = min(kFilterEdges, segs.n - first);
      for (int i = threadIdx.x; i < m_segs; i += 256) {
        const FilterSegRec R = segs.rec[first + i];
        s_start[i] = R.start;
        s_pos0[i] = R.pos0;
        s_slots[i] = R.slots;
        s_prev[i] = R.prev;
        s_type[i] = R.type;
        s_base_a[i] = R.base_a;
        s_base_b[i] = R.base_b;
        s_slot_base[i] = R.slot_base;
      }
      __syncthreads();
    }
  }
  bool valid[kFilterPer];
  int a[kFilterPer], b[kFilterPer], l_type[kFilterPer];
  uint32_t gpos[kFilterPer];
  if (have_segs) {
    const uint32_t* slots_p[kFilterPer];
    const int32_t* prev_p[kFilterPer];
    int pos[kFilterPer], base_a[kFilterPer], base_b[kFilterPer];
    int jc[kFilterPer];
#pragma unroll
    for (int e = 0; e < kFilterPer; ++e) {
      const int j = jf + e * 256 + threadIdx.x;
      valid[e] = j < n_b;
      jc[e] = valid[e] ? j : n_b - 1;
    }
    if constexpr (kArgs) {
      const int lane = threadIdx.x & 63;
      const int st = lane < segs.n ? A.r[lane].start : 0x7fffffff;
      const int first = max(0, (int)__popcll(__ballot(st <= jf)) - 1);
      const int end = max(first + 1, (int)__popcll(__ballot(st < min(jf + kFilterEdges, n_b))));
      for (int k = first; k < end; ++k) {
        const FilterSegRec R = A.r[k];
#pragma unroll
        for (int e = 0; e < kFilterPer; ++e) {
          if (k == first || jc[e] >= R.start) {
            pos[e] = R.pos0 + (jc[e] - R.start);
            slots_p[e] = R.slots;
            prev_p[e] = R.prev;
            l_type[e] = R.type;
            base_a[e] = R.base_a;
            base_b[e] = R.base_b;
            gpos[e] = R.slot_base + (uint32_t)pos[e];
          }
        }
      }
    } else {
#pragma unroll
      for (int e = 0; e < kFilterPer; ++e) {
        int lo = 0, hi = m_segs;
        while (hi - lo > 1) {
          const int mid = (lo + hi) >> 1;
          if (s_start[mid] <= jc[e]) lo = mid; else hi = mid;
        }
        pos[e] = s_pos0[lo] + (jc[e] - s_start[lo]);
        slots_p[e] = s_slots[lo];
        prev_p[e] = s_prev[lo];
        l_type[e] = s_type[lo];
        base_a[e] = s_base_a[lo];
        base_b[e] = s_base_b[lo];
        gpos[e] = s_slot_base[lo] + (uint32_t)pos[e];
      }
    }
    uint32_t slot[kFilterPer];
#pragma unroll
    for (int e = 0; e < kFilterPer; ++e) slot[e] = slots_p[e][pos[e]];
    uint32_t pix[kFilterPer];
    int pv[kFilterPer];
#pragma unroll
    for (int e = 0; e < kFilterPer; ++e) {
      const uint32_t tm = (uint32_t)-(int)(l_type[e] != 0);
      pix[e] = ((slot[e] / 9u) & tm) | ((slot[e] >> 2) & ~tm);
      pv[e] = prev_p[e][pix[e]];
    }
#pragma unroll
    for (int e = 0; e < kFilterPer; ++e) {
      a[e] = base_a[e] + (int)pix[e];
      const int kt = (int)(slot[e] - pix[e] * 9u);
      const int dy = kt / 3 - 1, dx = kt - (kt / 3) * 3 - 1;
      const int bt = base_b[e] + pv[e] + dy * P.W + dx;
      const int ks = (int)(slot[e] & 3u);
      const int bs = a[e] + (ks != 0 ? P.W : 0) + (ks == 0 || ks == 3 ? 1 : 0) - (ks == 2 ? 1 : 0);
      const int tm = -(int)(l_type[e] != 0);
      b[e] = (bt & tm) | (bs & ~tm);
    }
  } else {
#pragma unroll
    for (int e = 0; e < kFilterPer; ++e) {
      const int j = jf + e * 256 + threadIdx.x;
      valid[e] = j < n_b;
      const int jc = valid[e] ? j : n_b - 1;
      int bk = bucket;
      int jb = j0 + jc;
      if (bucket_hi > bucket + 1) {
        const int jg = bucket_prefix[bucket] + jb;
        int lo = bucket, hi = bucket_hi;
        while (hi - lo > 1) {
          const int mid = (lo + hi) >> 1;
          if (bucket_prefix[mid] <= jg) lo = mid; else hi = mid;
        }
        bk = lo;
        jb = jg - bucket_prefix[bk];
      }
      const int32_t* base_row = bucket_base + (size_t)bk * (P.num_lists + 1);
      const int l = LocateList(base_row, P.num_lists, jb);
      const int pos = lists[l].offsets[bk] + (jb - base_row[l]);
      const ListDesc L = lists[l];
      l_type[e] = L.type;
      DecodeEdge(L, L.slots[pos], P.W, a[e], b[e]);
      gpos[e] = list_slot_base[l] + (uint32_t)pos;
    }
  }
  constexpr int kChains = 2 * kFilterPer;
  int x0[kChains], root[kChains];
#pragma unroll
  for (int e = 0; e < kFilterPer; ++e) {
    x0[2 * e] = a[e];
    x0[2 * e + 1] = b[e];
  }
  int hop[kChains];
#pragma unroll
  for (int c = 0; c < kChains; ++c) hop[c] = nodes.parent[x0[c]];
  bool any = false;
#pragma unroll
  for (int c = 0; c < kChains; ++c) {
    root[c] = hop[c];
    any = any || (hop[c] != x0[c]);
  }
  while (any) {
    int p[kChains];
#pragma unroll
    for (int c = 0; c < kChains; ++c) p[c] = nodes.parent[root[c]];
    any = false;
#pragma unroll
    for (int c = 0; c < kChains; ++c) {
      if (p[c] != root[c]) {
        root[c] = p[c];
        any = true;
      }
    }
  }
  {
    int cur[kChains];
#pragma unroll
    for (int c = 0; c < kChains; ++c) {
      cur[c] = root[c];
      if (x0[c] != root[c] && hop[c] != root[c]) {
        nodes.parent[x0[c]] = root[c];
        cur[c] = hop[c];
        any = true;
      }
    }
    while (any) {
      int nx[kChains];
#pragma unroll
      for (int c = 0; c < kChains; ++c) nx[c] = cur[c] != root[c] ? nodes.parent[cur[c]] : root[c];
      any = false;
#pragma unroll
      for (int c = 0; c < kChains; ++c) {
        if (cur[c] != root[c]) {
          if (nx[c] != root[c]) nodes.parent[cur[c]] = root[c];
          cur[c] = nx[c];
          any = any || (cur[c] != root[c]);
        }
      }
    }
  }
  int ti[kFilterPer], active[kFilterPer], settled[kFilterPer];
#pragma unroll
  for (int e = 0; e < kFilterPer; ++e) {
    ti[e] = active[e] = settled[e] = 0;
    const int ra = root[2 * e], rb = root[2 * e + 1];
    if (!valid[e] || ra == rb) continue;
    if (P.spatial_survivors && l_type[e] == 0 && !P.spatial_survivors[gpos[e]]) continue;
    bool inert = false;
    int f1 = 0, f2 = 0, s1 = 0, s2 = 0, c1 = -1, c2 = -1;
    if (inert_mode != 0) {
      f1 = nodes.flags[ra];
      f2 = nodes.flags[rb];
      if (f1 & kFlagFinalized) s1 = __float_as_int(nodes.desc_sz[ra].w);
      if (f2 & kFlagFinalized) s2 = __float_as_int(nodes.desc_sz[rb].w);
      const bool both_final_large = (f1 & kFlagFinalized) && (f2 & kFlagFinalized) &&
                                    (s1 >= P.min_region_size) && (s2 >= P.min_region_size);
      if (inert_mode == 1) {
        inert = both_final_large;
      } else {
        c1 = nodes.cons[ra];
        c2 = nodes.cons[rb];
        if (c1 >= 0 && c2 >= 0) {
          inert = (c1 != c2);
        } else {
          inert = both_final_large;
        }
        if (inert) {
          ti[e] = 1;
          if (!(f1 & kFlagTentative)) nodes.flags[ra] = (uint8_t)(f1 | kFlagTentative);
          if (!(f2 & kFlagTentative)) nodes.flags[rb] = (uint8_t)(f2 | kFlagTentative);
        }
      }
    }
    if (inert) {
      kept_all[gpos[e]] = 1;
      settled[e] = 1;
    } else {
      active[e] = 1;
      bool hub_edge = false;
      if (hubs) {
        constexpr int kNoHub = kFlagNoDesc | kFlagHubExcluded;
        const bool h1 = (f1 & kFlagFinalized) && !(f1 & kNoHub) && s1 >= P.min_region_size;
        const bool h2 = (f2 & kFlagFinalized) && !(f2 & kNoHub) && s2 >= P.min_region_size;
        if (h1 != h2) {
          const int h = h1 ? ra : rb, x = h1 ? rb : ra;
          const int fx = h1 ? f2 : f1, cx = h1 ? c2 : c1, fh = h1 ? f1 : f2;
          const int ch = h1 ? c1 : c2;
          if ((cx < 0 || cx == ch) && !(fx & kFlagNoDesc)) {
            hub_edge = true;
            root[2 * e] = x;
            root[2 * e + 1] = h;
            if (!nodes.hub8[h]) nodes.hub8[h] = 1;
            if (!(*num_hub & 1)) atomicOr(num_hub, 1);
            if (cx >= 0) {
              const float4 dx = nodes.desc_sz[x], dh = nodes.desc_sz[h];
              const float u = dh.x - dx.x, v = dh.y - dx.y, w = dh.z - dx.z;
              if ((u * u + v * v + w * w) * (1.0f / 3.0f) > split_s) {
                HubViolationAt(hub_excl, 0, jf + e * 256 + (int)threadIdx.x);
                if (!(*num_hub & 16)) atomicOr(num_hub, 16);
              }
            }
          } else {
            HubViolationAt(hub_excl, 0, jf + e * 256 + (int)threadIdx.x);
            if (!(fh & kFlagHubBroken)) HubExclude(hub_excl, nodes.flags, h);
          }
        } else if (h1 && h2) {
          HubViolationAt(hub_excl, 0, jf + e * 256 + (int)threadIdx.x);
          if (s1 <= s2 && !(f1 & kFlagHubBroken)) HubExclude(hub_excl, nodes.flags, ra);
          if (s2 <= s1 && !(f2 & kFlagHubBroken)) HubExclude(hub_excl, nodes.flags, rb);
        }
      }
      if (!hub_edge) CcUnion(cc, ra, rb);
    }
  }
  const int w = threadIdx.x >> 6, lane = threadIdx.x & 63;
  const int n_blocks = (n_b + 255) >> 8;
  unsigned long long ma[kFilterPer], ms[kFilterPer];
#pragma unroll
  for (int e = 0; e < kFilterPer; ++e) {
    ma[e] = __ballot(active[e] != 0);
    ms[e] = __ballot(settled[e] != 0);
    const unsigned long long mt = __ballot(ti[e] != 0);
    const int vb = blockIdx.x * kFilterPer + e;
    if (lane == 0 && vb < n_blocks) {
      const size_t gw = (size_t)vb * 4 + w;
      M.active[gw] = ma[e];
      M.settled[gw] = ms[e];
      M.tentative[gw] = mt;
      wave_cnt[e][w] = (int)__popcll(ma[e]);
      wave_kept[e][w] = (int)__popcll(ma[e] | ms[e]);
      if (mt != 0 && *num_ti == 0) *num_ti = 1;
    }
  }
  __syncthreads();
#pragma unroll
  for (int e = 0; e < kFilterPer; ++e) {
    const int vb = blockIdx.x * kFilterPer + e;
    if (active[e] | settled[e]) {
      int rank = (int)__popcll((ma[e] | ms[e]) & ((1ull << lane) - 1ull));
      for (int k = 0; k < w; ++k) rank += wave_kept[e][k];
      const int slot = vb * 256 + rank;
      e_ra[slot] = root[2 * e];
      e_rb[slot] = root[2 * e + 1];
      e_gpos[slot] = gpos[e];
    }
    if (threadIdx.x == 0 && vb < n_blocks) {
      M.block_cnt[vb] = wave_cnt[e][0] + wave_cnt[e][1] + wave_cnt[e][2] + wave_cnt[e][3];
    }
  }
}

__device__ __forceinline__ int FilterSlot(const FilterMasks& M, int j) {
  const int block = j >> 8, w = (j >> 6) & 3, lane = j & 63;
  const size_t gw0 = (size_t)block * 4;
  int rank = (int)__popcll((M.active[gw0 + w] | M.settled[gw0 + w]) & ((1ull << lane) - 1ull));
  for (int k = 0; k < w; ++k) rank += (int)__popcll(M.active[gw0 + k] | M.settled[gw0 + k]);
  return block * 256 + rank;
}

__global__ __launch_bounds__(256) void k_clear_tentative(int n_b, FilterMasks M,
                                                          const int32_t* __restrict__ e_ra,
                                                          const int32_t* __restrict__ e_rb,
                                                          NodeArrays nodes) {
  const int j = blockIdx.x * 256 + threadIdx.x;
  if (j >= n_b || !((M.tentative[j >> 6] >> (j & 63)) & 1ull)) return;
  const int slot = FilterSlot(M, j);
  int r[2] = {e_ra[slot], e_rb[slot]};
  for (int k = 0; k < 2; ++k) {
    int x = r[k];
    for (;;) {
      const int f = nodes.flags[x];
      if (f & kFlagTentative) nodes.flags[x] = (uint8_t)(f & ~kFlagTentative);
      const int p = nodes.parent[x];
      if (p == x) break;
      x = p;
    }
  }
}

__global__ __launch_bounds__(256) void k_backup_roots(int n, const int32_t* __restrict__ a_ra,
                                                       const int32_t* __restrict__ a_rb,
                                                       NodeArrays nodes, float4* __restrict__ bk_ds,
                                                       int32_t* __restrict__ bk_cons,
                                                       uint8_t* __restrict__ bk_flags,
                                                       unsigned long long* __restrict__ stats) {
  const int i = blockIdx.x * 256 + threadIdx.x;
  if (i < 8) stats[8 + i] = stats[i];
  if (i >= n) return;
  const int ra = a_ra[i], rb = a_rb[i];
  bk_ds[2 * i] = nodes.desc_sz[ra];
  bk_cons[2 * i] = nodes.cons[ra];
  bk_flags[2 * i] = nodes.flags[ra];
  bk_ds[2 * i + 1] = nodes.desc_sz[rb];
  bk_cons[2 * i + 1] = nodes.cons[rb];
  bk_flags[2 * i + 1] = nodes.flags[rb];
}

__global__ __launch_bounds__(256) void k_restore_roots(int n, const int32_t* __restrict__ a_ra,
                                                        const int32_t* __restrict__ a_rb,
                                                        NodeArrays nodes,
                                                        const float4* __restrict__ bk_ds,
                                                        const int32_t* __restrict__ bk_cons,
                                                        const uint8_t* __restrict__ bk_flags,
                                                        unsigned long long* __restrict__ stats) {
  const int i = blockIdx.x * 256 + threadIdx.x;
  if (i < 8) stats[i] = stats[8 + i];
  if (i >= n) return;
  const int ra = a_ra[i], rb = a_rb[i];
  nodes.parent[ra] = ra;
  nodes.desc_sz[ra] = bk_ds[2 * i];
  nodes.cons[ra] = bk_cons[2 * i];
  nodes.flags[ra] = bk_flags[2 * i];
  nodes.parent[rb] = rb;
  nodes.desc_sz[rb] = bk_ds[2 * i + 1];
  nodes.cons[rb] = bk_cons[2 * i + 1];
  nodes.flags[rb] = bk_flags[2 * i + 1];
}

__global__ __launch_bounds__(256) void k_clear_kept(int n_b, FilterMasks M,
                                                     const uint32_t* __restrict__ e_gpos,
                                                     uint8_t* __restrict__ kept_all) {
  const int j = blockIdx.x * 256 + threadIdx.x;
  if (j >= n_b) return;
  if (((M.active[j >> 6] | M.settled[j >> 6]) >> (j & 63)) & 1ull) kept_all[e_gpos[FilterSlot(M, j)]] = 0;
}

__global__ __launch_bounds__(256) void k_compact_active(int n_b, FilterMasks M,
                                                         const int32_t* __restrict__ block_off,
                                                         const int32_t* __restrict__ e_ra,
                                                         const int32_t* __restrict__ e_rb,
                                                         const uint32_t* __restrict__ e_gpos,
                                                         int32_t* __restrict__ a_ra,
                                                         int32_t* __restrict__ a_rb,
                                                         uint32_t* __restrict__ a_gpos,
                                                         int32_t* __restrict__ num_active,
                                                         const int32_t* __restrict__ num_ti,
                                                         unsigned long long* __restrict__ mail, unsigned mail_seq,
                                                         int a_cap, const int32_t* __restrict__ num_hub) {
  const int j = blockIdx.x * 256 + threadIdx.x;
  const int w = threadIdx.x >> 6, lane = threadIdx.x & 63;
  const size_t gw0 = (size_t)blockIdx.x * 4;
  const unsigned long long m = M.active[gw0 + w];
  int base = block_off[blockIdx.x];
  for (int k = 0; k < w; ++k) base += (int)__popcll(M.active[gw0 + k]);
  if ((m >> lane) & 1ull) {
    const int p = base + (int)__popcll(m & ((1ull << lane) - 1ull));
    if (p < a_cap) {
      const int slot = FilterSlot(M, j);
      a_ra[p] = e_ra[slot];
      a_rb[p] = e_rb[slot];
      a_gpos[p] = e_gpos[slot];
    }
  }
  if (blockIdx.x == gridDim.x - 1 && threadIdx.x == 255) {
    const int total = base + (int)__popcll(m);
    *num_active = total;
    MailPost(mail, mail_seq, 0, total);
    MailPost(mail, mail_seq, 1, *num_ti);
    MailPost(mail, mail_seq, 2, *num_hub);
  }
}

__global__ __launch_bounds__(256) void k_component_ids(int n, const int32_t* __restrict__ a_ra,
                                                        int32_t* __restrict__ cc,
                                                        uint32_t* __restrict__ a_comp,
                                                        uint32_t* __restrict__ a_idx) {
  const int i = blockIdx.x * 256 + threadIdx.x;
  if (i >= n) return;
  a_comp[i] = (uint32_t)CcFind(cc, a_ra[i]);
  a_idx[i] = (uint32_t)i;
}

__global__ __launch_bounds__(256) void k_reset_cc(int n, const int32_t* __restrict__ a_ra,
                                                   const int32_t* __restrict__ a_rb,
                                                   int32_t* __restrict__ cc,
                                                   const int32_t* __restrict__ violation,
                                                   unsigned long long* __restrict__ mail, unsigned mail_seq,
                                                   const int32_t* __restrict__ decomp) {
  const int i = blockIdx.x * 256 + threadIdx.x;
  if (i == 0 && mail) {
    MailPost(mail, mail_seq, 0, *violation);
    if (decomp) {
      MailPost(mail, mail_seq, 1, decomp[1]);
      MailPost(mail, mail_seq, 2, decomp[0]);
    }
  }
  if (i >= n) return;
  const int ra = a_ra[i], rb = a_rb[i];
  cc[ra] = ra;
  cc[rb] = rb;
}

__global__ __launch_bounds__(256) void k_gather_sorted(int n, const uint32_t* __restrict__ s_idx,
                                                        const int32_t* __restrict__ a_ra,
                                                        const int32_t* __restrict__ a_rb,
                                                        const uint32_t* __restrict__ a_gpos,
                                                        int32_t* __restrict__ s_ra,
                                                        int32_t* __restrict__ s_rb,
                                                        uint32_t* __restrict__ s_gpos,
                                                        const int32_t* __restrict__ num_segs,
                                                        const int32_t* __restrict__ seg_cnt, int below,
                                                        int32_t* __restrict__ decomp) {
  const int p = blockIdx.x * 256 + threadIdx.x;
  if (p < n) {
    const uint32_t i = s_idx[p];
    s_ra[p] = a_ra[i];
    s_rb[p] = a_rb[i];
    s_gpos[p] = a_gpos[i];
  }
  if (decomp) {
    const int m = *num_segs;
    int v = p < n && p < m ? seg_cnt[p] : 0;
    if (v >= below) v = 0;
    for (int off = 32; off > 0; off >>= 1) v = max(v, __shfl_xor(v, off));
    if ((threadIdx.x & 63) == 0 && v > decomp[0]) atomicMax(decomp, v);
    if (p == 0) decomp[1] = m;
  }
}


__global__ __launch_bounds__(256) void k_merge_small(const int32_t* __restrict__ num_segs,
                                                      const int32_t* __restrict__ seg_off,
                                                      const int32_t* __restrict__ seg_cnt,
                                                      const int32_t* __restrict__ s_ra,
                                                      const int32_t* __restrict__ s_rb,
                                                      const uint32_t* __restrict__ s_gpos,
                                                      NodeArrays nodes, uint8_t* __restrict__ kept_all,
                                                      StageThr T, int optimistic,
                                                      int32_t* __restrict__ violation,
                                                      unsigned long long* __restrict__ stats,
                                                      int small_seg, int wave_max,
                                                      uint32_t* __restrict__ work_list,
                                                      int work_cap, int32_t* __restrict__ work_ctl,
                                                      int cls_min0, int32_t* __restrict__ hub_mark,
                                                      const uint32_t* __restrict__ s_seq,
                                                      int32_t* __restrict__ hub_excl) {
  const int seg = blockIdx.x * 256 + threadIdx.x;
  unsigned n_forced = 0, n_regular = 0, n_small = 0;
  const int cnt = seg < *num_segs ? seg_cnt[seg] : 0;
  if (work_list) {
    const int cls = (cnt > small_seg && cnt < wave_max) ? (cnt >= cls_min0 ? 0 : (cnt >= kWaveClassMin1 ? 1 : 2)) : -1;
    const int lane = threadIdx.x & 63;
#pragma unroll
    for (int c = 0; c < kWaveClasses; ++c) {
      const unsigned long long m = __ballot(cls == c);
      if (!m) continue;
      int base = 0;
      if (lane == (int)__builtin_ctzll(m)) base = atomicAdd(&work_ctl[c], (int)__popcll(m));
      base = __shfl(base, (int)__builtin_ctzll(m));
      if (cls == c) work_list[(size_t)c * work_cap + base + (int)__popcll(m & ((1ull << lane) - 1ull))] = (uint32_t)seg;
    }
  }
  if (seg < *num_segs) {
    if (cnt <= small_seg) {
      const int beg = seg_off[seg];
      for (int p = beg; p < beg + cnt; ++p) {
        const int r1 = optimistic ? FindReadOnly(nodes.parent, s_ra[p])
                                  : FindCompress(nodes.parent, s_ra[p]);
        const int r2 = optimistic ? FindReadOnly(nodes.parent, s_rb[p])
                                  : FindCompress(nodes.parent, s_rb[p]);
        if (r1 == r2) continue;
        RState s1 = LoadState(nodes, r1);
        RState s2 = LoadState(nodes, r2);
        if (T.hubs) {
          if (nodes.hub8[r1]) s1.flags |= kFlagHub;
          if (nodes.hub8[r2]) s2.flags |= kFlagHub;
        }
        if (T.hubs && ((s1.flags | s2.flags) & kFlagHub)) {
          const bool hub1 = (s1.flags & kFlagHub) != 0, hub2 = (s2.flags & kFlagHub) != 0;
          const RState& x = hub1 ? s2 : s1;
          const RState& h = hub1 ? s1 : s2;
          const int act = (hub1 && hub2) ? HubHubEdge(s1.cons, s1.flags, s2.cons, s2.flags)
                                         : HubEdge(x, h.cons, h.flags, h.sz, T);
          if (act >= kHubViolation) {
            atomicOr(violation, act);
            WorkerViolationAt(hub_excl, T, s_seq, s_gpos, p);
            if (hub1) HubExclude(hub_excl, nodes.flags, r1);
            if (hub2) HubExclude(hub_excl, nodes.flags, r2);
          } else if (act == kHubKeep) {
            kept_all[s_gpos[p]] = 1;
          } else {
            const int xr = hub1 ? r2 : r1, hr = hub1 ? r1 : r2;
            nodes.parent[xr] = hr;
            if (x.flags & kFlagTentative) AtomicOrFlags(nodes.flags, hr, kFlagTentative);
            hub_mark[s_seq[p]] = xr | (act == kHubAbsorbTest ? kHubTestBit : 0);
            if (act == kHubAbsorbTest) ++n_forced; else ++n_small;
          }
          continue;
        }
        const RState o1 = s1, o2 = s2;
        int stat;
        const int out = DecideEdge(s1, s2, T, stat);
        if (optimistic) {
          const bool v = (out == kOutKeep)     ? TentativeViolated(o1, o2, s1, s2)
                         : (out == kOutMerge1) ? TentativeViolated(o1, o2, s1, s1)
                                               : TentativeViolated(o1, o2, s2, s2);
          if (v) {
            atomicOr(violation, kVioCut);
            WorkerViolationAt(hub_excl, T, s_seq, s_gpos, p);
          }
        }
        if (stat == 4 && T.rle) {
          atomicOr(violation, kVioCut);
          WorkerViolationAt(hub_excl, T, s_seq, s_gpos, p);
        }
        n_forced += (stat == 1);
        n_regular += (stat == 2);
        n_small += (stat == 3);
        if (out == kOutKeep) {
          if (T.side) {
            atomicOr(violation, 2);
            HubViolationAt(hub_excl, 2, (int)s_gpos[p]);
// ... 96 lines not shown
    MailPost(mail, mail_seq, 0, total);
  }
};

constexpr int kHubWaveMin = 32;
__global__ __launch_bounds__(64) void k_hub_apply_wave(const int32_t* __restrict__ num_runs,
                                                        const int32_t* __restrict__ run_off,
                                                        const int32_t* __restrict__ run_cnt,
                                                        const uint32_t* __restrict__ hub_sorted,
                                                        const uint32_t* __restrict__ seq_sorted,
                                                        const int32_t* __restrict__ mark, NodeArrays nodes,
                                                        float split_s, int32_t* __restrict__ violation,
                                                        int32_t* __restrict__ hub_excl) {
  __shared__ float coef[64][4];
  __shared__ float before[64][4];
  const int lane = threadIdx.x;
  const int n_runs = *num_runs;
  for (int r = blockIdx.x; r < n_runs; r += gridDim.x) {
    const int cnt = run_cnt[r];
    if (cnt < kHubWaveMin) continue;
    const int off = run_off[r];
    const int hub = (int)hub_sorted[off];
    const float4 hs = nodes.desc_sz[hub];
    float h = lane == 0 ? hs.x : lane == 1 ? hs.y : hs.z;
    int S = __float_as_int(hs.w);
    int bad_seq = -1;
    for (int base = 0; base < cnt; base += 64) {
      const int i = base + lane;
      const bool valid = i < cnt;
      uint32_t sq = 0, xv = 0;
      float4 o = make_float4(0.f, 0.f, 0.f, 0.f);
      if (valid) {
        sq = seq_sorted[off + i];
        xv = (uint32_t)mark[sq];
        o = nodes.desc_sz[xv & ~(uint32_t)kHubTestBit];
      }
      const int osz = valid ? __float_as_int(o.w) : 0;
      const int incl = WaveInclusiveSum(osz);
      const int Sb = S + incl - osz;
      float4 q = make_float4(0.f, 0.f, 0.f, 1.f);
      if (valid) {
        const float denom = 1.0f / (float)(osz + Sb);
        const float ca = (float)osz * denom;
        const float cb = (float)Sb * denom;
        q = make_float4(ca * o.x, ca * o.y, ca * o.z, cb);
      }
      coef[lane][0] = q.x;
      coef[lane][1] = q.y;
      coef[lane][2] = q.z;
      coef[lane][3] = q.w;
      __builtin_amdgcn_fence(__ATOMIC_SEQ_CST, "wavefront");
      __builtin_amdgcn_wave_barrier();
      if (lane < 3) {
#pragma unroll 8
        for (int l = 0; l < 64; ++l) {
          before[l][lane] = h;
          h = coef[l][lane] + coef[l][3] * h;
        }
      }
      __builtin_amdgcn_fence(__ATOMIC_SEQ_CST, "wavefront");
      __builtin_amdgcn_wave_barrier();
      bool fails = false;
      if (valid && (xv & (uint32_t)kHubTestBit)) {
        const float x = before[lane][0] - o.x, y = before[lane][1] - o.y, z = before[lane][2] - o.z;
        fails = (x * x + y * y + z * z) * (1.0f / 3.0f) > split_s;
      }
      const unsigned long long fm = __ballot(fails);
      if (fm && bad_seq < 0) bad_seq = __builtin_amdgcn_readlane((int)sq, (int)__builtin_ctzll(fm));
      S += __builtin_amdgcn_readlane(incl, 63);
      __builtin_amdgcn_wave_barrier();
    }
    const float r0 = ReadLaneF(h, 0), r1 = ReadLaneF(h, 1), r2 = ReadLaneF(h, 2);
    if (lane == 0) {
      if (bad_seq >= 0) {
        atomicOr(violation, kHubVioSplit);
        HubViolationAt(hub_excl, 1, bad_seq);
        HubExclude(hub_excl, nodes.flags, hub);
      }
      nodes.desc_sz[hub] = make_float4(r0, r1, r2, __int_as_float(S));
    }
  }
}

__global__ __launch_bounds__(64) void k_hub_apply(const int32_t* __restrict__ num_runs,
                                                   const int32_t* __restrict__ run_off,
                                                   const int32_t* __restrict__ run_cnt,
                                                   const uint32_t* __restrict__ hub_sorted,
                                                   const uint32_t* __restrict__ seq_sorted,
                                                   const int32_t* __restrict__ mark,
                                                   NodeArrays nodes, float split_s,
                                                   int32_t* __restrict__ violation,
                                                   int32_t* __restrict__ hub_excl) {
  const int r = blockIdx.x * 64 + threadIdx.x;
  if (r >= *num_runs) return;
  const int off = run_off[r], cnt = run_cnt[r];
  if (cnt >= kHubWaveMin) return;
  const int hub = (int)hub_sorted[off];
  const float4 hs = nodes.desc_sz[hub];
  float h0 = hs.x, h1 = hs.y, h2 = hs.z;
  int S = __float_as_int(hs.w);
  int bad_seq = -1;
  auto absorb = [&](const float4& o, bool test, uint32_t seq) {
    if (test) {
      const float x = h0 - o.x, y = h1 - o.y, z = h2 - o.z;
      if ((x * x + y * y + z * z) * (1.0f / 3.0f) > split_s && bad_seq < 0) bad_seq = (int)seq;
    }
    const int osz = __float_as_int(o.w);
    const float denom = 1.0f / (float)(osz + S);
    const float ca = (float)osz * denom;
    const float cb = (float)S * denom;
    h0 = ca * o.x + cb * h0;
    h1 = ca * o.y + cb * h1;
    h2 = ca * o.z + cb * h2;
    S += osz;
  };
  int k = 0;
  for (; k + 4 <= cnt; k += 4) {
    float4 o[4];
    uint32_t xv[4], sq[4];
#pragma unroll
    for (int q = 0; q < 4; ++q) sq[q] = seq_sorted[off + k + q];
#pragma unroll
    for (int q = 0; q < 4; ++q) xv[q] = (uint32_t)mark[sq[q]];
#pragma unroll
    for (int q = 0; q < 4; ++q) o[q] = nodes.desc_sz[xv[q] & ~(uint32_t)kHubTestBit];
#pragma unroll
    for (int q = 0; q < 4; ++q) absorb(o[q], (xv[q] & (uint32_t)kHubTestBit) != 0, sq[q]);
  }
  for (; k < cnt; ++k) {
    const uint32_t sq = seq_sorted[off + k];
    const uint32_t xv = (uint32_t)mark[sq];
    absorb(nodes.desc_sz[xv & ~(uint32_t)kHubTestBit], (xv & (uint32_t)kHubTestBit) != 0, sq);
  }
  if (bad_seq >= 0) {
    atomicOr(violation, kHubVioSplit);
    HubViolationAt(hub_excl, 1, bad_seq);
    HubExclude(hub_excl, nodes.flags, hub);
  }
  nodes.desc_sz[hub] = make_float4(h0, h1, h2, __int_as_float(S));
}

__global__ __launch_bounds__(256) void k_hub_clear(int n, const int32_t* __restrict__ a_ra,
                                                    const int32_t* __restrict__ a_rb, NodeArrays nodes) {
  const int i = blockIdx.x * 256 + threadIdx.x;
  if (i >= n) return;
  const int ra = a_ra[i], rb = a_rb[i];
  if (nodes.hub8[ra]) nodes.hub8[ra] = 0;
  if (nodes.hub8[rb]) nodes.hub8[rb] = 0;
  const int fa = nodes.flags[ra], fb = nodes.flags[rb];
  if (fa & kFlagHubBroken) nodes.flags[ra] = (uint8_t)(fa & ~(int)kFlagHubBroken);
  if (fb & kFlagHubBroken) nodes.flags[rb] = (uint8_t)(fb & ~(int)kFlagHubBroken);
}

__global__ __launch_bounds__(256) void k_hub_exclude(const int32_t* __restrict__ excl, NodeArrays nodes) {
  const int n = min(excl[0], kHubExclCap);
  for (int i = blockIdx.x * 256 + threadIdx.x; i < n; i += gridDim.x * 256) {
    const int r = excl[4 + i];
    if (!(nodes.flags[r] & kFlagHubExcluded)) AtomicOrFlags(nodes.flags, r, kFlagHubExcluded);
  }
}

__global__ __launch_bounds__(256) void k_hub_check(const int32_t* __restrict__ excl, NodeArrays nodes,
                                                    int32_t* __restrict__ num_hub) {
  const int cnt = excl[0];
  if (blockIdx.x == 0 && threadIdx.x == 0) {
    const int bits = (cnt > 0 ? (cnt > kHubExclCap ? 12 : 8) : 0) | (min(excl[1], 0xfffff) << 8);
    if (bits) atomicOr(num_hub, bits);
  }
  const int n = min(cnt, kHubExclCap);
  for (int i = blockIdx.x * 256 + threadIdx.x; i < n; i += gridDim.x * 256) {
    if (nodes.hub8[excl[4 + i]]) {
      atomicOr(num_hub, 2);
      break;
    }
  }
}

__global__ __launch_bounds__(256) void k_hub_unexclude(int32_t* __restrict__ excl, NodeArrays nodes) {
  const int n = min(excl[0], kHubExclCap);
  for (int i = blockIdx.x * 256 + threadIdx.x; i < n; i += gridDim.x * 256) {
    AtomicAndFlags(nodes.flags, excl[4 + i], 0xff & ~(kFlagHubExcluded | kFlagHubBroken));
  }
}
__global__ void k_hub_excl_reset(int32_t* __restrict__ excl) { excl[0] = excl[1] = excl[2] = excl[3] = 0; }
__global__ void k_hub_cut_gpos(int32_t* __restrict__ list, const uint32_t* __restrict__ work_gpos) {
  const int n = min(list[2], kHubCutCap);
  int32_t* at = list + 4 + kHubExclCap + kHubCutCap;
  for (int i = threadIdx.x; i < n; i += blockDim.x) at[i] = (int32_t)work_gpos[at[i]];
}
void ResetHubExclusions(MergeScratch& S, NodeArrays nodes, hipStream_t s) {
  if (!S.hub_excl) return;
  hipLaunchKernelGGL(k_hub_unexclude, dim3(16), dim3(256), 0, s, S.hub_excl, nodes);
  hipLaunchKernelGGL(k_hub_excl_reset, dim3(1), dim3(1), 0, s, S.hub_excl);
  VSG_HIP(hipGetLastError());
}

__global__ void k_plain_edge(int bucket, int jb, const ListDesc* __restrict__ lists,
                             const int32_t* __restrict__ bucket_base, const uint32_t* __restrict__ list_slot_base,
                             uint8_t* __restrict__ kept_all, NodeArrays nodes, MergeParams P, StageThr T,
                             unsigned long long* __restrict__ stats) {
  const int32_t* base_row = bucket_base + (size_t)bucket * (P.num_lists + 1);
  const int l = LocateList(base_row, P.num_lists, jb);
  const int pos = lists[l].offsets[bucket] + (jb - base_row[l]);
  const ListDesc L = lists[l];
  int a, b;
  DecodeEdge(L, L.slots[pos], P.W, a, b);
  const uint32_t gpos = list_slot_base[l] + (uint32_t)pos;
  if (P.spatial_survivors && L.type == 0 && !P.spatial_survivors[gpos]) return;
  int r1 = a, r2 = b;
  for (int p; (p = nodes.parent[r1]) != r1;) r1 = p;
  for (int p; (p = nodes.parent[r2]) != r2;) r2 = p;
  if (r1 == r2) return;
  RState s1 = LoadState(nodes, r1), s2 = LoadState(nodes, r2);
  int stat;
  const int out = DecideEdge(s1, s2, T, stat);
  if (stat >= 1 && stat <= 3) atomicAdd(&stats[stat - 1], 1ull);
  if (out == kOutKeep) {
    kept_all[gpos] = 1;
    StoreState(nodes, r1, s1);
    StoreState(nodes, r2, s2);
  } else if (out == kOutMerge1) {
    StoreState(nodes, r1, s1);
    nodes.parent[r2] = r1;
  } else {
    StoreState(nodes, r2, s2);
    nodes.parent[r1] = r2;
  }
}

static long long SequencePosition(const MergeScratch& S, const MergeParams& P, int b_lo, int b_hi, uint32_t gpos) {
  const int L = P.num_lists;
  int lo = 0, hi = L;
  while (hi - lo > 1) {
    const int mid = (lo + hi) >> 1;
    if (S.list_slot_base_host[mid] <= gpos) lo = mid; else hi = mid;
  }
  const int l = lo;
  const long long p = (long long)gpos - (long long)S.list_slot_base_host[l];
  const int32_t* off = S.list_off_host + (size_t)l * (kNumBuckets + 2);
  int b0 = b_lo, b1 = b_hi;
  while (b1 - b0 > 1) {
    const int mid = (b0 + b1) >> 1;
    if (off[mid] <= p) b0 = mid; else b1 = mid;
  }
  const int32_t* row = S.bucket_base_host + (size_t)b0 * (L + 1);
  return (long long)S.bucket_prefix_host[b0] + row[l] + (p - (long long)off[b0]);
}
static int BucketOfPosition(const MergeScratch& S, int b_lo, int b_hi, long long g) {
  int b0 = b_lo, b1 = b_hi;
  while (b1 - b0 > 1) {
    const int mid = (b0 + b1) >> 1;
    if ((long long)S.bucket_prefix_host[mid] <= g) b0 = mid; else b1 = mid;
  }
  return b0;
}

static inline unsigned Blocks(int n) { return (unsigned)((n + 255) / 256); }

__global__ void k_max_segment(int max_segs, const int32_t* __restrict__ num_segs,
                              const int32_t* __restrict__ seg_cnt, int below, int32_t* __restrict__ out);

void RunBucketStage(int bucket, int j0, int n_b, const ListDesc* lists, const int32_t* bucket_base,
                    const uint32_t* list_slot_base, uint8_t* kept_all, NodeArrays nodes,
                    const MergeParams& P, int inert_mode, MergeScratch& S, hipStream_t s,
                    StageInfo* info) {
  if (info) {
    info->replayed = 0;
    info->components = 0;
  }
  if (n_b <= 0) return;
  const int bucket_hi = S.group_hi > bucket ? S.group_hi : bucket + 1;
  int32_t* d_num_ti = TakeStageScalars(S, 8);
  int32_t* d_violation = d_num_ti + 1;
  int32_t* d_num_hub = d_num_ti + 2;
  int32_t* d_hub_count = d_num_ti + 3;
  int32_t* d_hub_runs = d_num_ti + 4;
  const bool spine_possible = S.spine_min > 0 && !S.spine_off && bucket < *S.spine_limit_bucket &&
                              !(bucket < 2 && S.spine_low_skip[bucket]);
  const bool try_hubs = S.hubs && !S.hubs_off && inert_mode != 0 && !spine_possible && S.wide_min <= 0;
  if (S.hub_excl && S.hub_list_dirty) {
    if (S.hub_attempt == 0) {
      VSG_HIP(hipMemsetAsync(S.hub_excl, 0, 4 * sizeof(int32_t), s));
      S.hub_list_dirty = 0;
    } else {
      VSG_HIP(hipMemsetAsync(S.hub_excl + 1, 0, 3 * sizeof(int32_t), s));
    }
  }
  if (S.hub_excl && S.hub_check) {
    int head[4] = {0, 0, 0, 0};
    VSG_HIP(hipMemcpyAsync(head, S.hub_excl, sizeof(head), hipMemcpyDeviceToHost, s));
    VSG_HIP(hipStreamSynchronize(s));
    for (int k = 1; k < 4; ++k) {
      if (head[k] != 0) {
        Throw(-4 , "hub check: stage b=" + std::to_string(bucket) + " j0=" + std::to_string(j0) +
                                             " n=" + std::to_string(n_b) + " starts with " + std::to_string(head[k]) +
                                             " stale entries of kind " + std::to_string(k - 1) + " on the hub list");
      }
    }
  }
  if (S.hub_attempt == 0 && S.hub_split_depth == 0) S.hub_splits_left = S.hub_max_splits;
  int32_t* d_num_leaders = S.num_active + 5;
  FilterSegs segs = {nullptr, 0};
  FilterSegArgs seg_args;
  bool segs_in_args = false;
  if (S.bucket_base_host && S.list_off_host && S.lists_host && S.list_slot_base_host && S.seg_dev) {
    const int L = P.num_lists;
    constexpr size_t kRecInts = sizeof(FilterSegRec) / sizeof(int32_t);
    const int64_t g0 = (int64_t)S.bucket_prefix_host[bucket] + j0, g1 = g0 + n_b;
    std::vector<FilterSegRec> recs;
    for (int b = bucket; b < bucket_hi; ++b) {
      const int32_t* row = S.bucket_base_host + (size_t)b * (L + 1);
      const int64_t bstart = S.bucket_prefix_host[b];
      if (bstart + row[L] <= g0) continue;
      if (bstart >= g1) break;
      for (int l = 0; l < L; ++l) {
        const int cnt = row[l + 1] - row[l];
        if (cnt == 0) continue;
        const int64_t s0 = bstart + row[l], s1 = s0 + cnt;
        if (s1 <= g0 || s0 >= g1) continue;
        const int64_t first = std::max(s0, g0);
        const ListDesc& D = S.lists_host[l];
        FilterSegRec R;
        R.slots = D.slots;
        R.prev = D.type != 0 ? D.prev_idx : reinterpret_cast<const int32_t*>(D.slots);
        R.start = (int32_t)(first - g0);
        R.pos0 = S.list_off_host[(size_t)l * (kNumBuckets + 2) + b] + (int32_t)(first - s0);
        R.type = D.type;
        R.base_a = D.base_a;
        R.base_b = D.base_b;
        R.slot_base = S.list_slot_base_host[l];
        recs.push_back(R);
      }
    }
    const int nseg = (int)recs.size();
    if (nseg > 0 && nseg <= kFilterArgSegs && S.filter_segs_mode != 1) {
      std::copy(recs.begin(), recs.end(), seg_args.r);
      segs.n = nseg;
      segs_in_args = true;
    } else if (nseg > 0 && nseg <= 65536 && kRecInts * nseg <= S.seg_cap) {
      int32_t* src = TakeStageRing(S, kRecInts * nseg);
      if (!src) {
        S.seg_host->resize(kRecInts * nseg);
        src = S.seg_host->data();
      }
      std::memcpy(src, recs.data(), (size_t)nseg * sizeof(FilterSegRec));
      VSG_HIP(hipMemcpyAsync(S.seg_dev, src, (size_t)nseg * sizeof(FilterSegRec), hipMemcpyHostToDevice, s));
      segs.rec = reinterpret_cast<const FilterSegRec*>(S.seg_dev);
      segs.n = nseg;
    }
  }
  const float split_s = ((float)bucket * P.inv_scale < P.force_merge_weight) ? P.s_lt_02 : P.s_le_015;
  const int ef0 = NextEvent(S);
  if (ef0 >= 0) VSG_HIP(hipEventRecord((*S.ev_pool)[ef0], s));
  const dim3 filter_grid((unsigned)((n_b + kFilterEdges - 1) / kFilterEdges));
  if (segs_in_args) {
    hipLaunchKernelGGL(k_filter<true>, filter_grid, dim3(256), 0, s, bucket, bucket_hi, j0, n_b, lists, bucket_base,
                       S.bucket_prefix, list_slot_base, kept_all, nodes, P, inert_mode, S.cc, S.e_ra, S.e_rb, S.e_gpos,
                       S.masks, d_num_ti, segs, seg_args, try_hubs ? 1 : 0, d_num_hub, S.hub_excl, split_s);
  } else {
    hipLaunchKernelGGL(k_filter<false>, filter_grid, dim3(256), 0, s, bucket, bucket_hi, j0, n_b, lists, bucket_base,
                       S.bucket_prefix, list_slot_base, kept_all, nodes, P, inert_mode, S.cc, S.e_ra, S.e_rb, S.e_gpos,
                       S.masks, d_num_ti, segs, 0, try_hubs ? 1 : 0, d_num_hub, S.hub_excl, split_s);
  }
  const int ef1 = NextEvent(S);
  if (ef1 >= 0) {
    VSG_HIP(hipEventRecord((*S.ev_pool)[ef1], s));
    S.ev_filter->emplace_back(ef0, ef1);
  }
  if (try_hubs) hipLaunchKernelGGL(k_hub_check, dim3(16), dim3(256), 0, s, S.hub_excl, nodes, d_num_hub);
  ExclusiveSum(S.scan, S.masks.block_cnt, S.block_off, (int)Blocks(n_b), s);
  int h[3] = {0, 0, 0};
  for (int attempt = 0;; ++attempt) {
    const MailSlot m_active = NextMail(*S.mail);
    hipLaunchKernelGGL(k_compact_active, dim3(Blocks(n_b)), dim3(256), 0, s, n_b, S.masks, S.block_off,
                       S.e_ra, S.e_rb, S.e_gpos, S.a_ra, S.a_rb, S.a_gpos, S.num_active, d_num_ti, m_active.dev,
                       m_active.seq, S.active_cap, d_num_hub);
    VSG_HIP(hipGetLastError());
    MailWait(m_active, 3, h, s);
    if (h[0] <= S.active_cap) break;
    VSG_REQUIRE(attempt == 0 && S.grow_active && S.grow_active(h[0]) && h[0] <= S.active_cap, -4,
                "stage scratch: cannot hold the active edges");
  }
  const int n_active = h[0];
  const int n_ti = h[1];
  const bool hubs_used = try_hubs && (h[2] & 1) != 0;
  if (h[2] & (8 | 16)) S.hub_list_dirty = 1;
  auto clear_hub_marks = [&]() {
    if (try_hubs && (h[2] & 9) != 0 && n_active > 0) {
      hipLaunchKernelGGL(k_hub_clear, dim3(Blocks(n_active)), dim3(256), 0, s, n_active, S.a_ra, S.a_rb, nodes);
    }
  };
  auto clear_marks = [&]() {
    if (n_ti > 0) {
      hipLaunchKernelGGL(k_clear_tentative, dim3(Blocks(n_b)), dim3(256), 0, s, n_b, S.masks, S.e_ra,
                         S.e_rb, nodes);
    }
  };
  if (n_active == 0) {
    clear_marks();
    return;
  }
  auto can_cut = [&](int work, long long violations) {
    return work >= S.hub_cut_min_work && (long long)n_b > S.hub_cut_ratio * (violations + 1) && S.hub_splits_left > 0 &&
           S.bucket_base_host && S.bucket_prefix_host && S.list_off_host && S.list_slot_base_host;
  };
  auto retry_without_broken_hubs = [&](int violated, int work, bool list_complete, const uint32_t* work_gpos) -> bool {
    for (int q = 0; q < 6; ++q) S.hub_reasons[q] += (violated >> (2 + q)) & 1;
    ++S.hub_retries;
    if (info) ++info->hub_retries;
    std::vector<int> cuts;
    const long long g_stage = (long long)S.bucket_prefix_host[bucket] + j0;
    int head[4] = {0, 0, 0, 0};
    if (can_cut(work, 0)) {
      VSG_HIP(hipMemcpyAsync(head, S.hub_excl, sizeof(head), hipMemcpyDeviceToHost, s));
      VSG_HIP(hipStreamSynchronize(s));
    }
    if (can_cut(work, (long long)head[1] + (work_gpos ? head[2] + head[3] : 0))) {
      int at[3 * kHubCutCap];
      int raw1[kHubCutCap];
      if (S.hub_check && work_gpos) {
        VSG_HIP(hipMemcpyAsync(raw1, S.hub_excl + 4 + kHubExclCap + kHubCutCap, sizeof(raw1), hipMemcpyDeviceToHost, s));
        VSG_HIP(hipStreamSynchronize(s));
        for (int i = 0; i < std::min(head[2], kHubCutCap); ++i) {
          if (raw1[i] < 0 || raw1[i] >= work) {
            Throw(-4 , "hub check: stage b=" + std::to_string(bucket) + " j0=" + std::to_string(j0) +
                                                 " n=" + std::to_string(n_b) + ": cut entry " + std::to_string(i) +
                                                 " of kind 1 is work edge " + std::to_string(raw1[i]) + " of " +
                                                 std::to_string(work));
          }
        }
      }
      if (work_gpos) hipLaunchKernelGGL(k_hub_cut_gpos, dim3(1), dim3(64), 0, s, S.hub_excl, work_gpos);
      VSG_HIP(hipMemcpyAsync(at, S.hub_excl + 4 + kHubExclCap, sizeof(at), hipMemcpyDeviceToHost, s));
      VSG_HIP(hipStreamSynchronize(s));
      auto check_at = [&](int kind, int i, long long v, long long lo, long long hi) {
        if (S.hub_check && (v < lo || v >= hi)) {
          Throw(-4 , "hub check: stage b=" + std::to_string(bucket) + " j0=" + std::to_string(j0) +
                                               " n=" + std::to_string(n_b) + ": cut entry " + std::to_string(i) +
                                               " of kind " + std::to_string(kind) + " is " + std::to_string(v) +
                                               ", outside [" + std::to_string(lo) + ", " + std::to_string(hi) + ")");
        }
      };
      auto in_stage = [&](int kind, int i, uint32_t gpos) {
        if (!S.hub_check) return;
        const long long g = SequencePosition(S, P, bucket, bucket_hi, gpos) - g_stage;
        check_at(kind, i, g, 0, n_b);
        const long long gg = g_stage + g;
        const int b = BucketOfPosition(S, bucket, bucket_hi, gg);
        const int32_t* row = S.bucket_base_host + (size_t)b * (P.num_lists + 1);
        const int jb = (int)(gg - S.bucket_prefix_host[b]);
        int l = 0;
        while (l + 1 < P.num_lists && row[l + 1] <= jb) ++l;
        if ((uint32_t)(S.list_slot_base_host[l] + S.list_off_host[(size_t)l * (kNumBuckets + 2) + b] + (jb - row[l])) != gpos) {
          Throw(-4 , "hub check: stage b=" + std::to_string(bucket) + " j0=" + std::to_string(j0) +
                                               " n=" + std::to_string(n_b) + ": cut entry " + std::to_string(i) +
                                               " of kind " + std::to_string(kind) + " is kept position " +
                                               std::to_string(gpos) + ", not an edge of the stage");
        }
      };
      for (int i = 0; i < std::min(head[1], kHubCutCap); ++i) {
        check_at(0, i, at[i], 0, n_b);
        cuts.push_back(at[i]);
      }
      if (work_gpos) {
        for (int i = 0; i < std::min(head[2], kHubCutCap); ++i) {
          in_stage(1, i, (uint32_t)at[kHubCutCap + i]);
          cuts.push_back((int)(SequencePosition(S, P, bucket, bucket_hi, (uint32_t)at[kHubCutCap + i]) - g_stage));
        }
        for (int i = 0; i < std::min(head[3], kHubCutCap); ++i) {
          in_stage(2, i, (uint32_t)at[2 * kHubCutCap + i]);
          cuts.push_back((int)(SequencePosition(S, P, bucket, bucket_hi, (uint32_t)at[2 * kHubCutCap + i]) - g_stage));
        }
      }
      std::sort(cuts.begin(), cuts.end());
      cuts.erase(std::unique(cuts.begin(), cuts.end()), cuts.end());
      while (!cuts.empty() && cuts.back() >= n_b) cuts.pop_back();
      while (!cuts.empty() && cuts.front() < 0) cuts.erase(cuts.begin());
      if (!work_gpos && cuts.size() > 1) cuts.resize(1);
      if ((int)cuts.size() > S.hub_splits_left) cuts.resize((size_t)S.hub_splits_left);
    }
    if (getenv("VSG_DEBUG_STAGES")) {
      int cnt = 0;
      VSG_HIP(hipMemcpyAsync(&cnt, S.hub_excl, sizeof(int), hipMemcpyDeviceToHost, s));
      VSG_HIP(hipStreamSynchronize(s));
      std::fprintf(stderr, "[vsg]   hub rule violated (mask %x) in b=%d j0=%d n=%d work %d, attempt %d, %d regions on the "
                   "list, %zu cuts (first at %d, %d left)\n", violated, bucket, j0, n_b, work, S.hub_attempt, cnt,
                   cuts.size(), cuts.empty() ? -1 : cuts[0], S.hub_splits_left);
    }
    if (!cuts.empty()) {
      S.hub_splits_left -= (int)cuts.size();
      S.hub_splits += (long long)cuts.size();
      if (bucket_hi > bucket + 1) S.hub_cuts_in_groups += (long long)cuts.size();
      if (violated == 2 && bucket < 2) S.spine_side_cuts += (long long)cuts.size();
      int replayed = 0;
      auto part = [&](int off, int n, bool plain) {
        if (n <= 0) return;
        StageInfo sub;
        if (info) sub.want_components = info->want_components;
        ++S.hub_split_depth;
        if (plain) ++S.hubs_off;
        const int b_at = BucketOfPosition(S, bucket, bucket_hi, g_stage + off);
        if (b_at > bucket) ++S.hub_parts_in_later_bucket;
        RunBucketStage(b_at, (int)(g_stage + off - S.bucket_prefix_host[b_at]), n, lists, bucket_base, list_slot_base,
                       kept_all, nodes, P, inert_mode, S, s, info ? &sub : nullptr);
        if (plain) --S.hubs_off;
        --S.hub_split_depth;
        replayed += sub.replayed;
        if (info) {
          info->hub_stages += sub.hub_stages;
          info->hub_absorbed += sub.hub_absorbed;
          info->hub_retries += sub.hub_retries;
          info->components += sub.components;
          info->max_wave_segment = std::max(info->max_wave_segment, sub.max_wave_segment);
        }
      };
      StageThr plain;
      plain.pass_s = ((float)bucket * P.inv_scale < P.force_merge_weight) ? P.s_lt_02 : P.s_lt_005;
      plain.split_s = split_s;
      plain.min_size = P.min_region_size;
      plain.rle = 0;
      plain.side = 0;
      plain.hubs = 0;
      int prev = 0;
      for (const int c : cuts) {
        part(prev, c - prev, false);
        const int b_c = BucketOfPosition(S, bucket, bucket_hi, g_stage + c);
        hipLaunchKernelGGL(k_plain_edge, dim3(1), dim3(1), 0, s, b_c, (int)(g_stage + c - S.bucket_prefix_host[b_c]), lists,
                           bucket_base, list_slot_base, kept_all, nodes, P, plain, S.stats);
        ++replayed;
        prev = c + 1;
      }
      part(prev, n_b - prev, false);
      if (info) info->replayed = replayed;
      return true;
    }
    if (violated & (kVioCut | 2)) return false;
    int& depth = (list_complete && S.hub_attempt + 1 < kHubMaxAttempts) ? S.hub_attempt : S.hubs_off;
    if (&depth == &S.hub_attempt) {
      hipLaunchKernelGGL(k_hub_exclude, dim3(16), dim3(256), 0, s, S.hub_excl, nodes);
      ++S.hub_exclusion_reruns;
    } else {
      ++S.hub_off_reruns;
    }
    ++depth;
    RunBucketStage(bucket, j0, n_b, lists, bucket_base, list_slot_base, kept_all, nodes, P, inert_mode, S, s, info);
    --depth;
    if (S.hub_attempt == 0 && S.hubs_off == 0) ResetHubExclusions(S, nodes, s);
    return true;
  };
  if (hubs_used && ((h[2] & 6) != 0 || ((h[2] & 16) != 0 && can_cut(n_active, (long long)(h[2] >> 8))))) {
    hipLaunchKernelGGL(k_reset_cc, dim3(Blocks(n_active)), dim3(256), 0, s, n_active, S.a_ra, S.a_rb, S.cc,
                       d_violation, nullptr, 0u, nullptr);
    hipLaunchKernelGGL(k_clear_kept, dim3(Blocks(n_b)), dim3(256), 0, s, n_b, S.masks, S.e_gpos, kept_all);
    clear_marks();
    clear_hub_marks();
    VSG_HIP(hipGetLastError());
    if (retry_without_broken_hubs(kHubVioBroken, n_active, (h[2] & 4) == 0, nullptr)) return;
    VSG_REQUIRE(false, -4, "hub stage: no way to rerun it");
  }
  if (hubs_used && info) ++info->hub_stages;

  const bool rle = S.use_rle && inert_mode != 0 && n_active >= 64;
  const int32_t* w_ra = S.a_ra;
  const int32_t* w_rb = S.a_rb;
  const uint32_t* w_gpos = S.a_gpos;
  int n_work = n_active;
  int32_t* lead = S.e_active;
  if (rle) {
    ++S.sp.rle_stages;
    const MailSlot m_lead = NextMail(*S.mail);
    FusedScan(S.scan, LeaderValue{S.a_ra, S.a_rb},
              LeaderEmit{S.a_ra, S.a_rb, S.a_gpos, lead, S.lead_pos, S.l_ra, S.l_rb, S.l_gpos},
              LeaderFinish{d_num_leaders, m_lead.dev, m_lead.seq}, n_active, s);
    MailWait(m_lead, 1, &n_work, s);
    w_ra = S.l_ra;
    w_rb = S.l_rb;
    w_gpos = S.l_gpos;
  }

  hipLaunchKernelGGL(k_component_ids, dim3(Blocks(n_work)), dim3(256), 0, s, n_work, w_ra, S.cc,
                     S.a_comp, S.a_idx);
  ++(SortPairsU32TakesHand(n_work) ? S.sp.sorts_hand : S.sp.sorts_library);
  SortPairsU32(S.cub_temp, S.cub_temp_bytes, S.a_comp, S.s_comp, S.a_idx, S.s_idx, n_work, S.node_key_bits, s);
  RunsOfSortedKeys(S.scan, S.s_comp, n_work, S.seg_off, S.seg_cnt, S.num_segs, s);

  SpineInput spine_in;
  int spine_thr = 0x7fffffff;
  if (S.spine_min > 0 && !S.spine_off && bucket < *S.spine_limit_bucket &&
      !(bucket < 2 && S.spine_low_skip[bucket]) && inert_mode != 0 && n_work >= S.spine_min) {
    long long wanted = 0;
    spine_thr = SelectLargeSegments(n_work, S.num_segs, S.seg_off, S.seg_cnt, S.spine_min,
                                    S.spine_max_edges, S, s, &spine_in, &wanted);
    if (wanted > S.spine_max_edges && S.grow_spine_pool && S.grow_spine_pool(wanted)) {
      spine_thr = SelectLargeSegments(n_work, S.num_segs, S.seg_off, S.seg_cnt, S.spine_min,
                                      S.spine_max_edges, S, s, &spine_in, nullptr);
    }
  }
  const bool spine = !spine_in.segs.empty();
  VSG_REQUIRE(!(spine && hubs_used), -4, "merge stage: hub regions in a stage with a tree replay");
  const bool optimistic = ((inert_mode == 2) && (n_ti > 0 || rle)) || spine || hubs_used;
  if (optimistic) {
    hipLaunchKernelGGL(k_backup_roots, dim3(Blocks(n_work)), dim3(256), 0, s, n_work, w_ra, w_rb,
                       nodes, S.bk_ds, S.bk_cons, S.bk_flags, S.stats);
  }

  const float weight = (float)bucket * P.inv_scale;
  const bool force = weight < P.force_merge_weight;
  StageThr T;
  T.pass_s = force ? P.s_lt_02 : P.s_lt_005;
  T.split_s = force ? P.s_lt_02 : P.s_le_015;
  T.min_size = P.min_region_size;
  T.rle = rle ? 1 : 0;
  T.side = 0;
  T.relax = S.chain_relax;
  T.hubs = hubs_used ? 1 : 0;
  int32_t* s_ra = reinterpret_cast<int32_t*>(S.a_comp);
  int32_t* s_rb = reinterpret_cast<int32_t*>(S.a_idx);
  uint32_t* s_gpos = reinterpret_cast<uint32_t*>(S.e_apos);
  const bool report = info && info->want_components && (info->want_components > 1 || n_work > 16384);
  int32_t* d_decomp = report && optimistic ? d_num_ti + 5 : nullptr;
  hipLaunchKernelGGL(k_gather_sorted, dim3(Blocks(n_work)), dim3(256), 0, s, n_work, S.s_idx, w_ra,
                     w_rb, w_gpos, s_ra, s_rb, s_gpos, S.num_segs, S.seg_cnt, spine ? spine_thr : 0x7fffffff, d_decomp);
  const int small_seg = S.small_seg;
  auto WaveGrid = [small_seg](int n) {
    const int g = n / (small_seg + 1);
    return g < 1 ? 1 : (g > 8192 ? 8192 : g);
  };
  const int wave_grid = WaveGrid(n_work);
  WorkerArgs wa;
  wa.num_segs = S.num_segs;
  wa.seg_off = S.seg_off;
  wa.seg_cnt = S.seg_cnt;
  wa.s_ra = s_ra;
  wa.s_rb = s_rb;
  wa.s_gpos = s_gpos;
  wa.nodes = nodes;
  wa.kept_all = kept_all;
  wa.T = T;
  wa.optimistic = optimistic ? 1 : 0;
  wa.violation = d_violation;
  wa.stats = S.stats;
  wa.small_seg = small_seg;
  wa.wave_min = small_seg;
  wa.wave_max = spine_thr;
  wa.work_cap = n_work / (small_seg + 1) + 1;
  wa.work_list = (size_t)kWaveClasses * wa.work_cap <= (size_t)n_work ? S.seg_key : nullptr;
  wa.work_ctl = wa.work_list ? TakeZeroed(S, 2 * kWaveClasses) : nullptr;
  wa.wide_min = S.wide_min;
  wa.wide_waves = S.wide_waves;
  wa.s_seq = S.s_idx;
  wa.hub_excl = S.hub_excl;
  if (hubs_used) {
    wa.hub_mark = reinterpret_cast<int32_t*>(S.s_comp);
    VSG_HIP(hipMemsetAsync(wa.hub_mark, 0xFF, (size_t)n_work * sizeof(int32_t), s));
  }
  auto general_workers = [&](const WorkerArgs& w, int small_threads, int grid, hipStream_t s) {
    VSG_REQUIRE(!w.T.hubs || (w.s_seq && w.hub_mark), -4, "merge stage: hub workers without work-edge numbers");
    if (w.wave_min == w.small_seg) {
      hipLaunchKernelGGL(k_merge_small, dim3(Blocks(small_threads)), dim3(256), 0, s, w.num_segs,
                         w.seg_off, w.seg_cnt, w.s_ra, w.s_rb, w.s_gpos, w.nodes, w.kept_all, w.T,
                         w.optimistic, w.violation, w.stats, w.small_seg, w.wave_max, w.work_list, w.work_cap,
                         w.work_ctl,
                         (w.wide_min > 0 && w.wide_min < kWaveClassMin0) ? std::max(w.wide_min, w.small_seg + 1)
                                                                        : kWaveClassMin0,
                         w.hub_mark, w.s_seq, w.hub_excl);
    }
    const int ew0 = NextEvent(S);
    if (ew0 >= 0) VSG_HIP(hipEventRecord((*S.ev_pool)[ew0], s));
    const bool wide = w.work_list != nullptr && w.wide_min > 0 && w.wide_min < w.wave_max &&
                      small_threads >= w.wide_min && w.wave_min == w.small_seg;
    if (wide) {
      ++S.sp.wide_launches;
      WorkerArgs narrow = w;
      narrow.wave_max = w.wide_min;
      LaunchMergeWave(grid, narrow, S.wave_debug != 0, S.wave_dbg, s);
      const int wide_grid = std::min(small_threads / w.wide_min + 1, 1024);
      LaunchMergeWide(wide_grid, w, w.wide_waves, s);
    } else {
      LaunchMergeWave(grid, w, S.wave_debug != 0, S.wave_dbg, s);
    }
    const int ew1 = NextEvent(S);
    if (ew1 >= 0) {
      VSG_HIP(hipEventRecord((*S.ev_pool)[ew1], s));
      S.ev_wave->emplace_back(ew0, ew1);
    }
  };
  if (!spine) {
    general_workers(wa, n_work, wave_grid, s);
  } else {
    VSG_HIP(hipEventRecord(S.aux_fork, s));
    VSG_HIP(hipStreamWaitEvent(S.aux_stream, S.aux_fork, 0));
    general_workers(wa, n_work, wave_grid, S.aux_stream);
    VSG_HIP(hipEventRecord(S.aux_join, S.aux_stream));
    const bool done = RunSpineComponents(spine_in, wa, S, s, [&](const WorkerArgs& w, int n, hipStream_t st) {
      general_workers(w, n, WaveGrid(n), st);
    }, 0, 0);
    if (!done) {
      ++S.sp.top_level_fallbacks;
      WorkerArgs w3 = wa;
      w3.wave_min = spine_thr - 1;
      w3.wave_max = 0x7fffffff;
      w3.work_list = nullptr;
      general_workers(w3, n_work, wave_grid, s);
    }
    VSG_HIP(hipStreamWaitEvent(s, S.aux_join, 0));
  }
  if (hubs_used) {
    uint32_t* seq_list = S.a_comp;
    uint32_t* key_list = S.a_idx;
    uint32_t* key_sorted = reinterpret_cast<uint32_t*>(S.e_apos);
    uint32_t* seq_sorted = S.s_idx;
    int32_t* run_off = reinterpret_cast<int32_t*>(S.seg_key);
    int32_t* run_cnt = S.seg_off;
    const MailSlot m_hub = NextMail(*S.mail);
    FusedScan(S.scan, HubMarkValue{wa.hub_mark}, HubMarkEmit{wa.hub_mark, nodes.parent, seq_list, key_list},
              HubMarkFinish{d_hub_count, m_hub.dev, m_hub.seq}, n_work, s);
    int n_abs = 0;
    MailWait(m_hub, 1, &n_abs, s);
    if (n_abs > 0) {
      ++(SortPairsU32TakesHand(n_abs) ? S.sp.sorts_hand : S.sp.sorts_library);
      SortPairsU32(S.cub_temp, S.cub_temp_bytes, key_list, key_sorted, seq_list, seq_sorted, n_abs, S.node_key_bits, s);
      RunsOfSortedKeys(S.scan, key_sorted, n_abs, run_off, run_cnt, d_hub_runs, s);
      hipLaunchKernelGGL(k_hub_apply, dim3((unsigned)((n_abs + 63) / 64)), dim3(64), 0, s, d_hub_runs, run_off,
                         run_cnt, key_sorted, seq_sorted, wa.hub_mark, nodes, T.split_s, d_violation, S.hub_excl);
      if (n_abs >= kHubWaveMin) {
        hipLaunchKernelGGL(k_hub_apply_wave, dim3((unsigned)std::min(n_abs / kHubWaveMin, 2048)), dim3(64), 0, s,
                           d_hub_runs, run_off, run_cnt, key_sorted, seq_sorted, wa.hub_mark, nodes, T.split_s,
                           d_violation, S.hub_excl);
      }
    }
    if (info) info->hub_absorbed += n_abs;
  }
  MailSlot m_vio = {nullptr, nullptr, 0};
  if (optimistic) m_vio = NextMail(*S.mail);
  hipLaunchKernelGGL(k_reset_cc, dim3(Blocks(n_work)), dim3(256), 0, s, n_work, w_ra, w_rb, S.cc, d_violation,
                     m_vio.dev, m_vio.seq, d_decomp);
  VSG_HIP(hipGetLastError());
  int decomp[2] = {0, 0};
  if (optimistic) {
    int vio[3] = {0, 0, 0};
    MailWait(m_vio, d_decomp ? 3 : 1, vio, s);
    const int violated = vio[0];
    decomp[0] = vio[1];
    decomp[1] = vio[2];
    ++*S.optimistic_stages;
    if (violated || S.force_rollback) {
      ++*S.rollbacks;
      S.hub_list_dirty = 1;
      hipLaunchKernelGGL(k_restore_roots, dim3(Blocks(n_work)), dim3(256), 0, s, n_work, w_ra, w_rb,
                         nodes, S.bk_ds, S.bk_cons, S.bk_flags, S.stats);
      hipLaunchKernelGGL(k_clear_kept, dim3(Blocks(n_b)), dim3(256), 0, s, n_b, S.masks, S.e_gpos, kept_all);
      clear_marks();
      clear_hub_marks();
      VSG_HIP(hipGetLastError());
      if (spine && violated == 2 && bucket < 2 && !S.force_rollback && retry_without_broken_hubs(2, n_work, true, w_gpos)) {
        return;
      }
      if (spine && violated == 2 && !S.force_rollback) {
        ++S.sp.assumption_reruns;
        if (bucket >= 2 && bucket < *S.spine_limit_bucket) {
          *S.spine_limit_bucket = bucket;
          ++S.sp.limit_bucket_moves;
        }
        if (bucket < 2) {
          S.spine_low_failed[bucket] = 1;
          ++S.sp.low_bucket_failures[bucket];
        }
        const int off = S.spine_off;
        S.spine_off = 1;
        RunBucketStage(bucket, j0, n_b, lists, bucket_base, list_slot_base, kept_all, nodes, P, inert_mode, S,
                       s, info);
        S.spine_off = off;
        return;
      }
      if ((violated & (kHubViolationMask | kVioCut)) != 0 && (violated & ~(kHubViolationMask | kVioCut)) == 0 &&
          !spine && !S.force_rollback) {
        if (retry_without_broken_hubs(violated, n_work, true, w_gpos)) return;
      }
      if (bucket_hi > bucket + 1) {
        ++S.group_halvings;
        const int group_hi = S.group_hi;
        const int64_t g0 = (int64_t)S.bucket_prefix_host[bucket] + j0, g1 = g0 + n_b;
        const int mid = bucket + (bucket_hi - bucket) / 2;
        const int halves[2][2] = {{bucket, mid}, {mid, bucket_hi}};
        int replayed = 0;
        for (const auto& h : halves) {
          const int64_t lo = std::max<int64_t>(g0, S.bucket_prefix_host[h[0]]);
          const int64_t hi = std::min<int64_t>(g1, S.bucket_prefix_host[h[1]]);
          if (hi <= lo) continue;
          S.group_hi = h[1];
          StageInfo sub;
          RunBucketStage(h[0], (int)(lo - S.bucket_prefix_host[h[0]]), (int)(hi - lo), lists, bucket_base,
                         list_slot_base, kept_all, nodes, P, inert_mode, S, s, info ? &sub : nullptr);
          replayed += sub.replayed;
        }
        S.group_hi = group_hi;
        if (info) info->replayed = replayed;
        return;
      }
      ++S.conservative_replays;
      RunBucketStage(bucket, j0, n_b, lists, bucket_base, list_slot_base, kept_all, nodes, P, 0, S,
                     s, info);
      return;
    }
  }
  if (info) {
    info->replayed = n_work;
    if (d_decomp) {
      info->components = decomp[0];
      info->max_wave_segment = decomp[1];
    } else if (report) {
      int32_t* d_max = TakeZeroed(S, 1);
      hipLaunchKernelGGL(k_max_segment, dim3(Blocks(n_work)), dim3(256), 0, s, n_work, S.num_segs, S.seg_cnt,
                         spine ? spine_thr : 0x7fffffff, d_max);
      const MailSlot m_info = NextMail(*S.mail);
      LaunchMailPost(m_info, S.num_segs, d_max, nullptr, nullptr, s);
      int v[2] = {0, 0};
      MailWait(m_info, 2, v, s);
      info->components = v[0];
      info->max_wave_segment = v[1];
    }
  }
  if (rle && n_work < n_active) {
    hipLaunchKernelGGL(k_resolve_followers, dim3(Blocks(n_active)), dim3(256), 0, s, n_active, lead,
                       S.lead_pos, S.a_gpos, S.l_gpos, kept_all);
  }
  clear_marks();
  clear_hub_marks();
  VSG_HIP(hipGetLastError());
}

__global__ __launch_bounds__(256) void k_run_counts(int n, const int32_t* __restrict__ num_runs,
                                                     const int32_t* __restrict__ seg_off,
                                                     int32_t* __restrict__ seg_cnt) {
  const int r = blockIdx.x * 256 + threadIdx.x;
  const int m = *num_runs;
  if (r >= m) return;
  seg_cnt[r] = (r + 1 < m ? seg_off[r + 1] : n) - seg_off[r];
}

void RunsOfSortedKeys(const ScanScratch& sc, const uint32_t* keys, int n, int32_t* seg_off, int32_t* seg_cnt,
                      int32_t* num_runs, hipStream_t s) {
  if (n <= 0) return;
  FusedScan(sc, RunHeadValue{keys}, RunHeadEmit{seg_off}, RunHeadFinish{num_runs}, n, s);
  hipLaunchKernelGGL(k_run_counts, dim3(Blocks(n)), dim3(256), 0, s, n, num_runs, seg_off, seg_cnt);
  VSG_HIP(hipGetLastError());
}

struct ScanTotalStore {
  int32_t* total;
  __device__ void operator()(int t) const { *total = t; }
};
void DebugExclusiveSum(const ScanScratch& sc, const int32_t* in, int32_t* out, int n, int32_t* total, hipStream_t s) {
  FusedScan(sc, ScanLoadI32{in}, ScanStoreI32{out}, ScanTotalStore{total}, n, s);
}

__global__ __launch_bounds__(256) void k_max_segment(int max_segs, const int32_t* __restrict__ num_segs,
                                                      const int32_t* __restrict__ seg_cnt, int below,
                                                      int32_t* __restrict__ out) {
  const int seg = blockIdx.x * 256 + threadIdx.x;
  int v = 0;
  if (seg < max_segs && seg < *num_segs) {
    v = seg_cnt[seg];
    if (v >= below) v = 0;
  }
  for (int off = 32; off > 0; off >>= 1) v = max(v, __shfl_xor(v, off));
  if ((threadIdx.x & 63) == 0 && v > *out) atomicMax(out, v);
}

__global__ __launch_bounds__(256) void k_keep_virtual_bucket(const ListDesc* __restrict__ lists,
                                                              int num_lists) {
  const int l = blockIdx.y;
  if (l >= num_lists) return;
  const ListDesc L = lists[l];
  if (!L.offsets) return;
  const int beg = L.offsets[kNumBuckets], end = L.offsets[kNumBuckets + 1];
  for (int p = beg + blockIdx.x * 256 + threadIdx.x; p < end; p += gridDim.x * 256) L.kept[p] = 1;
}

void LaunchKeepVirtualBucket(const ListDesc* lists, int num_lists, hipStream_t s) {
  hipLaunchKernelGGL(k_keep_virtual_bucket, dim3(64, num_lists), dim3(256), 0, s, lists,
                     num_lists);
  VSG_HIP(hipGetLastError());
}

}
```

Measured before the change: 213.2.

## Cut hub stages in place at filter-reported position and add cost-based exclusion

The filter kernel now records the earliest hub-violation position with an atomic max, and the compaction kernel posts that cut position and the active count in front of it through the mail slot. A hub stage can then be split at that point without a host readback, keeping the already-filtered front part and skipping a full refilter of it. A cost model chooses between cutting and simply excluding the offending hubs and rerunning. This adds kernels, more mail values and more complex rerun logic, with a risk of correctness divergence, guarded by a hub-check mode.

```diff
diff --git a/include/vsg.h b/include/vsg.h
--- a/include/vsg.h
+++ b/include/vsg.h
@@ -91,6 +91,8 @@
   int64_t hub_exclusion_reruns;
   int64_t hub_off_reruns;
   int64_t group_halvings;
+  int64_t cuts_in_place;
+  int64_t cost_exclusions;
   int64_t conservative_replays;
 } vsg_merge_paths;
 
diff --git a/video_segment_amd/_lib.py b/video_segment_amd/_lib.py
--- a/video_segment_amd/_lib.py
+++ b/video_segment_amd/_lib.py
@@ -76,7 +76,8 @@
         ("spine_side_cuts", C.c_int64),
         ("hub_retries", C.c_int64), ("hub_reasons", C.c_int64 * 6),
         ("hub_exclusion_reruns", C.c_int64), ("hub_off_reruns", C.c_int64),
-        ("group_halvings", C.c_int64), ("conservative_replays", C.c_int64),
+        ("group_halvings", C.c_int64), ("cuts_in_place", C.c_int64), ("cost_exclusions", C.c_int64),
+        ("conservative_replays", C.c_int64),
     ]
 
     def as_dict(self):
diff --git a/video_segment_amd/csrc/capi.cpp b/video_segment_amd/csrc/capi.cpp
--- a/video_segment_amd/csrc/capi.cpp
+++ b/video_segment_amd/csrc/capi.cpp
@@ -123,6 +123,8 @@
   o->hub_exclusion_reruns = mp.hub_exclusion_reruns;
   o->hub_off_reruns = mp.hub_off_reruns;
   o->group_halvings = mp.group_halvings;
+  o->cuts_in_place = mp.cuts_in_place;
+  o->cost_exclusions = mp.cost_exclusions;
   o->conservative_replays = mp.conservative_replays;
 }
 
diff --git a/video_segment_amd/csrc/dense_graph.cpp b/video_segment_amd/csrc/dense_graph.cpp
--- a/video_segment_amd/csrc/dense_graph.cpp
+++ b/video_segment_amd/csrc/dense_graph.cpp
@@ -502,6 +502,23 @@
   S.hub_cut_min_work = getenv("VSG_CUT_MIN_WORK") ? atoi(getenv("VSG_CUT_MIN_WORK")) : 0;
   S.hub_cut_ratio = getenv("VSG_CUT_RATIO") ? std::max(0, atoi(getenv("VSG_CUT_RATIO"))) : 1500;
   S.hub_check = (getenv("VSG_HUB_CHECK") && atoi(getenv("VSG_HUB_CHECK")) != 0) ? 1 : 0;
+  S.cut_in_place = getenv("VSG_CUT_IN_PLACE") ? (atoi(getenv("VSG_CUT_IN_PLACE")) != 0 ? 1 : 0) : 1;
+  S.cut_cost_ns = getenv("VSG_CUT_COST_NS") ? std::max(0ll, atoll(getenv("VSG_CUT_COST_NS")))
+                                            : (S.hub_cut_ratio <= 1 ? 0 : kCutCostNs);
+  S.excl_edge_ns = getenv("VSG_EXCL_EDGE_NS") ? std::max(0ll, atoll(getenv("VSG_EXCL_EDGE_NS"))) : kExclEdgeNs;
+  std::vector<int> force_cut_at;
+  if (const char* e = getenv("VSG_FORCE_CUT_AT")) {
+    for (const char* q = e; *q;) {
+      char* end = nullptr;
+      const long v = std::strtol(q, &end, 10);
+      if (end == q) break;
+      if (v >= 0 && v < 0x7fffffff) force_cut_at.push_back((int)v);
+      if (*end != ',') break;
+      q = end + 1;
+    }
+    std::sort(force_cut_at.begin(), force_cut_at.end());
+  }
+  S.force_cut_at = force_cut_at.empty() ? nullptr : &force_cut_at;
   VSG_HIP(hipMemsetAsync(hub8_.get(), 0, N, stream_));
   S.spine_min = getenv("VSG_SPINE_MIN") ? atoi(getenv("VSG_SPINE_MIN")) : 2048;
   if (S.spine_min > 0) S.spine_min = std::max(S.spine_min, S.small_seg + 2);
@@ -912,6 +929,8 @@
     mp.hub_exclusion_reruns = S.hub_exclusion_reruns;
     mp.hub_off_reruns = S.hub_off_reruns;
     mp.group_halvings = S.group_halvings;
+    mp.cuts_in_place = S.cuts_in_place;
+    mp.cost_exclusions = S.cost_exclusions;
     mp.conservative_replays = S.conservative_replays;
     timings_.spine_paths = S.sp;
     timings_.slab_growths = diag_slab_growths;
diff --git a/video_segment_amd/csrc/dense_graph.h b/video_segment_amd/csrc/dense_graph.h
--- a/video_segment_amd/csrc/dense_graph.h
+++ b/video_segment_amd/csrc/dense_graph.h
@@ -15,6 +15,7 @@
   int64_t hub_cuts = 0, hub_cuts_in_groups = 0, hub_parts_in_later_bucket = 0, spine_side_cuts = 0;
   int64_t hub_retries = 0, hub_reasons[6] = {0, 0, 0, 0, 0, 0};
   int64_t hub_exclusion_reruns = 0, hub_off_reruns = 0, group_halvings = 0, conservative_replays = 0;
+  int64_t cuts_in_place = 0, cost_exclusions = 0;
 };
 
 struct GraphTimings {
diff --git a/video_segment_amd/csrc/device_graph.h b/video_segment_amd/csrc/device_graph.h
--- a/video_segment_amd/csrc/device_graph.h
+++ b/video_segment_amd/csrc/device_graph.h
@@ -17,6 +17,8 @@
 constexpr int kHubMaxAttempts = 4;
 constexpr int kHubMaxSplits = 64;
 constexpr int kHubCutCap = 64;
+constexpr long long kCutCostNs = 200000;
+constexpr long long kExclEdgeNs = 200;
 constexpr int kHubListInts = 4 + kHubExclCap + 3 * kHubCutCap;
 
 struct NodeArrays {
@@ -107,7 +109,7 @@
                unsigned long long* out,
                int32_t* num_out, int n, hipStream_t s);
 
-constexpr int kMailValues = 4;
+constexpr int kMailValues = 8;
 struct MailSlot {
   unsigned long long* dev;
   volatile unsigned long long* host;
@@ -265,6 +267,15 @@
   long long group_halvings;
   long long conservative_replays;
   long long hub_cut_ratio;
+  int cut_in_place;
+  long long cuts_in_place;
+  long long cut_cost_ns, excl_edge_ns;
+  long long cost_exclusions;
+  const std::vector<int>* force_cut_at;
+  struct PreFiltered {
+    int valid = 0;
+    int n_active = 0, n_ti = 0;
+  } pre;
   int hub_check;
   SpinePaths sp;
   int wave_debug;
diff --git a/video_segment_amd/csrc/merge_stage.hip b/video_segment_amd/csrc/merge_stage.hip
--- a/video_segment_amd/csrc/merge_stage.hip
+++ b/video_segment_amd/csrc/merge_stage.hip
@@ -188,6 +188,11 @@
 
 constexpr int kFilterPer = 2;
 constexpr int kFilterEdges = 256 * kFilterPer;
+
+__device__ __forceinline__ void FilterCutAt(int32_t* cut_at, int n_b, int j) {
+  const int v = n_b - j;
+  if (*cut_at < v) atomicMax(cut_at, v);
+}
 
 template <bool kArgs>
 __global__ __launch_bounds__(256) void k_filter(int bucket, int bucket_hi, int j0, int n_b,
@@ -205,7 +210,7 @@
                                                  int32_t* __restrict__ num_ti, FilterSegs segs,
                                                  std::conditional_t<kArgs, FilterSegArgs, int> A, int hubs,
                                                  int32_t* __restrict__ num_hub, int32_t* __restrict__ hub_excl,
-                                                 float split_s) {
+                                                 float split_s, int32_t* __restrict__ cut_at) {
   constexpr int kSegCap = kArgs ? 1 : kFilterEdges;
   __shared__ int wave_cnt[kFilterPer][4], wave_kept[kFilterPer][4];
   __shared__ int s_start[kSegCap], s_pos0[kSegCap];
@@ -456,15 +461,18 @@
               const float u = dh.x - dx.x, v = dh.y - dx.y, w = dh.z - dx.z;
               if ((u * u + v * v + w * w) * (1.0f / 3.0f) > split_s) {
                 HubViolationAt(hub_excl, 0, jf + e * 256 + (int)threadIdx.x);
+                FilterCutAt(cut_at, n_b, jf + e * 256 + (int)threadIdx.x);
                 if (!(*num_hub & 16)) atomicOr(num_hub, 16);
               }
             }
           } else {
             HubViolationAt(hub_excl, 0, jf + e * 256 + (int)threadIdx.x);
+            FilterCutAt(cut_at, n_b, jf + e * 256 + (int)threadIdx.x);
             if (!(fh & kFlagHubBroken)) HubExclude(hub_excl, nodes.flags, h);
           }
         } else if (h1 && h2) {
           HubViolationAt(hub_excl, 0, jf + e * 256 + (int)threadIdx.x);
+          FilterCutAt(cut_at, n_b, jf + e * 256 + (int)threadIdx.x);
           if (s1 <= s2 && !(f1 & kFlagHubBroken)) HubExclude(hub_excl, nodes.flags, ra);
           if (s2 <= s1 && !(f2 & kFlagHubBroken)) HubExclude(hub_excl, nodes.flags, rb);
         }
@@ -576,11 +584,11 @@
   nodes.flags[rb] = bk_flags[2 * i + 1];
 }
 
-__global__ __launch_bounds__(256) void k_clear_kept(int n_b, FilterMasks M,
+__global__ __launch_bounds__(256) void k_clear_kept(int j_lo, int n_b, FilterMasks M,
                                                      const uint32_t* __restrict__ e_gpos,
                                                      uint8_t* __restrict__ kept_all) {
-  const int j = blockIdx.x * 256 + threadIdx.x;
-  if (j >= n_b) return;
+  const int j = (j_lo & ~255) + blockIdx.x * 256 + threadIdx.x;
+  if (j < j_lo || j >= n_b) return;
   if (((M.active[j >> 6] | M.settled[j >> 6]) >> (j & 63)) & 1ull) kept_all[e_gpos[FilterSlot(M, j)]] = 0;
 }
 
@@ -595,7 +603,8 @@
                                                          int32_t* __restrict__ num_active,
                                                          const int32_t* __restrict__ num_ti,
                                                          unsigned long long* __restrict__ mail, unsigned mail_seq,
-                                                         int a_cap, const int32_t* __restrict__ num_hub) {
+                                                         int a_cap, const int32_t* __restrict__ num_hub,
+                                                         const int32_t* __restrict__ cut_at, int force_cut) {
   const int j = blockIdx.x * 256 + threadIdx.x;
   const int w = threadIdx.x >> 6, lane = threadIdx.x & 63;
   const size_t gw0 = (size_t)blockIdx.x * 4;
@@ -611,12 +620,17 @@
       a_gpos[p] = e_gpos[slot];
     }
   }
+  const int cut_v = *cut_at;
+  int cut = cut_v > 0 ? n_b - cut_v : 0x7fffffff;
+  if (force_cut >= 0 && force_cut < cut) cut = force_cut;
+  if (j == cut) MailPost(mail, mail_seq, 4, base + (int)__popcll(m & ((1ull << lane) - 1ull)));
   if (blockIdx.x == gridDim.x - 1 && threadIdx.x == 255) {
     const int total = base + (int)__popcll(m);
     *num_active = total;
     MailPost(mail, mail_seq, 0, total);
     MailPost(mail, mail_seq, 1, *num_ti);
     MailPost(mail, mail_seq, 2, *num_hub);
+    MailPost(mail, mail_seq, 3, cut == 0x7fffffff ? -1 : cut);
   }
 }
 
@@ -1019,11 +1033,51 @@
   if (fb & kFlagHubBroken) nodes.flags[rb] = (uint8_t)(fb & ~(int)kFlagHubBroken);
 }
 
+__global__ __launch_bounds__(256) void k_restore_front(int n_front, int cut, const int32_t* __restrict__ a_ra,
+                                                        const int32_t* __restrict__ a_rb, FilterMasks M,
+                                                        const int32_t* __restrict__ e_ra,
+                                                        const int32_t* __restrict__ e_rb, NodeArrays nodes,
+                                                        int32_t* __restrict__ cc, int min_region_size) {
+  const int i = blockIdx.x * 256 + threadIdx.x;
+  if (i < n_front) {
+    const int ra = a_ra[i], rb = a_rb[i];
+    const int f = nodes.flags[rb];
+    const bool hub = (f & kFlagFinalized) && !(f & (kFlagNoDesc | kFlagHubExcluded)) &&
+                     __float_as_int(nodes.desc_sz[rb].w) >= min_region_size;
+    if (hub) {
+      if (!nodes.hub8[rb]) nodes.hub8[rb] = 1;
+    } else {
+      CcUnion(cc, ra, rb);
+    }
+  }
+  if (i < cut && ((M.tentative[i >> 6] >> (i & 63)) & 1ull)) {
+    const int slot = FilterSlot(M, i);
+    const int r[2] = {e_ra[slot], e_rb[slot]};
+    for (int k = 0; k < 2; ++k) {
+      const int f = nodes.flags[r[k]];
+      if (!(f & kFlagTentative)) nodes.flags[r[k]] = (uint8_t)(f | kFlagTentative);
+    }
+  }
+}
+
 __global__ __launch_bounds__(256) void k_hub_exclude(const int32_t* __restrict__ excl, NodeArrays nodes) {
   const int n = min(excl[0], kHubExclCap);
   for (int i = blockIdx.x * 256 + threadIdx.x; i < n; i += gridDim.x * 256) {
     const int r = excl[4 + i];
     if (!(nodes.flags[r] & kFlagHubExcluded)) AtomicOrFlags(nodes.flags, r, kFlagHubExcluded);
+  }
+}
+
+__global__ void k_hub_list_cut_hubs(int32_t* __restrict__ excl, FilterMasks M, const int32_t* __restrict__ e_rb,
+                                    NodeArrays nodes) {
+  const int n = min(excl[1], kHubCutCap);
+  if (excl[0] + n > kHubExclCap) return;
+  const int32_t* at = excl + 4 + kHubExclCap;
+  for (int i = threadIdx.x; i < n; i += blockDim.x) {
+    const int h = e_rb[FilterSlot(M, at[i])];
+    if (!nodes.hub8[h] || (nodes.flags[h] & kFlagHubBroken)) continue;
+    if (AtomicOrFlags(nodes.flags, h, kFlagHubExcluded) & kFlagHubExcluded) continue;
+    excl[4 + atomicAdd(&excl[0], 1)] = h;
   }
 }
 
@@ -1142,6 +1196,9 @@
   int32_t* d_num_hub = d_num_ti + 2;
   int32_t* d_hub_count = d_num_ti + 3;
   int32_t* d_hub_runs = d_num_ti + 4;
+  int32_t* d_cut_at = d_num_ti + 7;
+  const MergeScratch::PreFiltered pre = S.pre;
+  S.pre.valid = 0;
   const bool spine_possible = S.spine_min > 0 && !S.spine_off && bucket < *S.spine_limit_bucket &&
                               !(bucket < 2 && S.spine_low_skip[bucket]);
   const bool try_hubs = S.hubs && !S.hubs_off && inert_mode != 0 && !spine_possible && S.wide_min <= 0;
@@ -1170,7 +1227,7 @@
   FilterSegs segs = {nullptr, 0};
   FilterSegArgs seg_args;
   bool segs_in_args = false;
-  if (S.bucket_base_host && S.list_off_host && S.lists_host && S.list_slot_base_host && S.seg_dev) {
+  if (!pre.valid && S.bucket_base_host && S.list_off_host && S.lists_host && S.list_slot_base_host && S.seg_dev) {
     const int L = P.num_lists;
     constexpr size_t kRecInts = sizeof(FilterSegRec) / sizeof(int32_t);
     const int64_t g0 = (int64_t)S.bucket_prefix_host[bucket] + j0, g1 = g0 + n_b;
@@ -1217,36 +1274,49 @@
     }
   }
   const float split_s = ((float)bucket * P.inv_scale < P.force_merge_weight) ? P.s_lt_02 : P.s_le_015;
-  const int ef0 = NextEvent(S);
-  if (ef0 >= 0) VSG_HIP(hipEventRecord((*S.ev_pool)[ef0], s));
-  const dim3 filter_grid((unsigned)((n_b + kFilterEdges - 1) / kFilterEdges));
-  if (segs_in_args) {
-    hipLaunchKernelGGL(k_filter<true>, filter_grid, dim3(256), 0, s, bucket, bucket_hi, j0, n_b, lists, bucket_base,
-                       S.bucket_prefix, list_slot_base, kept_all, nodes, P, inert_mode, S.cc, S.e_ra, S.e_rb, S.e_gpos,
-                       S.masks, d_num_ti, segs, seg_args, try_hubs ? 1 : 0, d_num_hub, S.hub_excl, split_s);
+  int force_cut = -1;
+  if (S.force_cut_at && try_hubs && !pre.valid) {
+    for (const int p : *S.force_cut_at) {
+      if (p < n_b) force_cut = p;
+    }
+  }
+  int h[5] = {0, 0, 0, -1, 0};
+  if (pre.valid) {
+    h[0] = pre.n_active;
+    h[1] = pre.n_ti;
+    h[2] = 1;
   } else {
-    hipLaunchKernelGGL(k_filter<false>, filter_grid, dim3(256), 0, s, bucket, bucket_hi, j0, n_b, lists, bucket_base,
-                       S.bucket_prefix, list_slot_base, kept_all, nodes, P, inert_mode, S.cc, S.e_ra, S.e_rb, S.e_gpos,
-                       S.masks, d_num_ti, segs, 0, try_hubs ? 1 : 0, d_num_hub, S.hub_excl, split_s);
-  }
-  const int ef1 = NextEvent(S);
-  if (ef1 >= 0) {
-    VSG_HIP(hipEventRecord((*S.ev_pool)[ef1], s));
-    S.ev_filter->emplace_back(ef0, ef1);
-  }
-  if (try_hubs) hipLaunchKernelGGL(k_hub_check, dim3(16), dim3(256), 0, s, S.hub_excl, nodes, d_num_hub);
-  ExclusiveSum(S.scan, S.masks.block_cnt, S.block_off, (int)Blocks(n_b), s);
-  int h[3] = {0, 0, 0};
-  for (int attempt = 0;; ++attempt) {
-    const MailSlot m_active = NextMail(*S.mail);
-    hipLaunchKernelGGL(k_compact_active, dim3(Blocks(n_b)), dim3(256), 0, s, n_b, S.masks, S.block_off,
-                       S.e_ra, S.e_rb, S.e_gpos, S.a_ra, S.a_rb, S.a_gpos, S.num_active, d_num_ti, m_active.dev,
-                       m_active.seq, S.active_cap, d_num_hub);
-    VSG_HIP(hipGetLastError());
-    MailWait(m_active, 3, h, s);
-    if (h[0] <= S.active_cap) break;
-    VSG_REQUIRE(attempt == 0 && S.grow_active && S.grow_active(h[0]) && h[0] <= S.active_cap, -4,
-                "stage scratch: cannot hold the active edges");
+    const int ef0 = NextEvent(S);
+    if (ef0 >= 0) VSG_HIP(hipEventRecord((*S.ev_pool)[ef0], s));
+    const dim3 filter_grid((unsigned)((n_b + kFilterEdges - 1) / kFilterEdges));
+    if (segs_in_args) {
+      hipLaunchKernelGGL(k_filter<true>, filter_grid, dim3(256), 0, s, bucket, bucket_hi, j0, n_b, lists, bucket_base,
+                         S.bucket_prefix, list_slot_base, kept_all, nodes, P, inert_mode, S.cc, S.e_ra, S.e_rb, S.e_gpos,
+                         S.masks, d_num_ti, segs, seg_args, try_hubs ? 1 : 0, d_num_hub, S.hub_excl, split_s, d_cut_at);
+    } else {
+      hipLaunchKernelGGL(k_filter<false>, filter_grid, dim3(256), 0, s, bucket, bucket_hi, j0, n_b, lists, bucket_base,
+                         S.bucket_prefix, list_slot_base, kept_all, nodes, P, inert_mode, S.cc, S.e_ra, S.e_rb, S.e_gpos,
+                         S.masks, d_num_ti, segs, 0, try_hubs ? 1 : 0, d_num_hub, S.hub_excl, split_s, d_cut_at);
+    }
+    const int ef1 = NextEvent(S);
+    if (ef1 >= 0) {
+      VSG_HIP(hipEventRecord((*S.ev_pool)[ef1], s));
+      S.ev_filter->emplace_back(ef0, ef1);
+    }
+    if (try_hubs) hipLaunchKernelGGL(k_hub_check, dim3(16), dim3(256), 0, s, S.hub_excl, nodes, d_num_hub);
+    ExclusiveSum(S.scan, S.masks.block_cnt, S.block_off, (int)Blocks(n_b), s);
+    for (int attempt = 0;; ++attempt) {
+      const MailSlot m_active = NextMail(*S.mail);
+      hipLaunchKernelGGL(k_compact_active, dim3(Blocks(n_b)), dim3(256), 0, s, n_b, S.masks, S.block_off,
+                         S.e_ra, S.e_rb, S.e_gpos, S.a_ra, S.a_rb, S.a_gpos, S.num_active, d_num_ti, m_active.dev,
+                         m_active.seq, S.active_cap, d_num_hub, d_cut_at, force_cut);
+      VSG_HIP(hipGetLastError());
+      MailWait(m_active, 4, h, s);
+      if (h[3] >= 0) MailWait(m_active, 5, h, s);
+      if (h[0] <= S.active_cap) break;
+      VSG_REQUIRE(attempt == 0 && S.grow_active && S.grow_active(h[0]) && h[0] <= S.active_cap, -4,
+                  "stage scratch: cannot hold the active edges");
+    }
   }
   const int n_active = h[0];
   const int n_ti = h[1];
@@ -1271,18 +1341,20 @@
     return work >= S.hub_cut_min_work && (long long)n_b > S.hub_cut_ratio * (violations + 1) && S.hub_splits_left > 0 &&
            S.bucket_base_host && S.bucket_prefix_host && S.list_off_host && S.list_slot_base_host;
   };
-  auto retry_without_broken_hubs = [&](int violated, int work, bool list_complete, const uint32_t* work_gpos) -> bool {
+  auto retry_without_broken_hubs = [&](int violated, int work, bool list_complete, const uint32_t* work_gpos,
+                                       int mail_cut, int front_active) -> bool {
     for (int q = 0; q < 6; ++q) S.hub_reasons[q] += (violated >> (2 + q)) & 1;
     ++S.hub_retries;
     if (info) ++info->hub_retries;
     std::vector<int> cuts;
     const long long g_stage = (long long)S.bucket_prefix_host[bucket] + j0;
     int head[4] = {0, 0, 0, 0};
-    if (can_cut(work, 0)) {
+    const bool read_back = work_gpos != nullptr || S.hub_check;
+    if (read_back && can_cut(work, 0)) {
       VSG_HIP(hipMemcpyAsync(head, S.hub_excl, sizeof(head), hipMemcpyDeviceToHost, s));
       VSG_HIP(hipStreamSynchronize(s));
     }
-    if (can_cut(work, (long long)head[1] + (work_gpos ? head[2] + head[3] : 0))) {
+    if (read_back && can_cut(work, (long long)head[1] + (work_gpos ? head[2] + head[3] : 0))) {
       int at[3 * kHubCutCap];
       int raw1[kHubCutCap];
       if (S.hub_check && work_gpos) {
@@ -1343,8 +1415,21 @@
       cuts.erase(std::unique(cuts.begin(), cuts.end()), cuts.end());
       while (!cuts.empty() && cuts.back() >= n_b) cuts.pop_back();
       while (!cuts.empty() && cuts.front() < 0) cuts.erase(cuts.begin());
-      if (!work_gpos && cuts.size() > 1) cuts.resize(1);
+      if (!work_gpos) {
+        const int recorded = cuts.empty() ? 0x7fffffff : cuts[0];
+        const int expected = (force_cut >= 0 && force_cut < recorded) ? force_cut : recorded;
+        const int posted = h[3] >= 0 ? h[3] : 0x7fffffff;
+        if (head[1] <= kHubCutCap ? posted != expected : posted > expected) {
+          Throw(-4 , "hub check: stage b=" + std::to_string(bucket) + " j0=" + std::to_string(j0) +
+                                               " n=" + std::to_string(n_b) + ": the filter posted cut position " +
+                                               std::to_string(h[3]) + ", the list says " + std::to_string(expected));
+        }
+      }
       if ((int)cuts.size() > S.hub_splits_left) cuts.resize((size_t)S.hub_splits_left);
+    }
+    if (!work_gpos) {
+      cuts.clear();
+      if (mail_cut >= 0 && mail_cut < n_b && can_cut(work, (long long)(h[2] >> 8))) cuts.push_back(mail_cut);
     }
     if (getenv("VSG_DEBUG_STAGES")) {
       int cnt = 0;
@@ -1390,7 +1475,14 @@
       plain.hubs = 0;
       int prev = 0;
       for (const int c : cuts) {
+        if (front_active >= 0) {
+          ++S.cuts_in_place;
+          S.pre.valid = 1;
+          S.pre.n_active = front_active;
+          S.pre.n_ti = n_ti;
+        }
         part(prev, c - prev, false);
+        S.pre.valid = 0;
         const int b_c = BucketOfPosition(S, bucket, bucket_hi, g_stage + c);
         hipLaunchKernelGGL(k_plain_edge, dim3(1), dim3(1), 0, s, b_c, (int)(g_stage + c - S.bucket_prefix_host[b_c]), lists,
                            bucket_base, list_slot_base, kept_all, nodes, P, plain, S.stats);
@@ -1415,14 +1507,33 @@
     if (S.hub_attempt == 0 && S.hubs_off == 0) ResetHubExclusions(S, nodes, s);
     return true;
   };
-  if (hubs_used && ((h[2] & 6) != 0 || ((h[2] & 16) != 0 && can_cut(n_active, (long long)(h[2] >> 8))))) {
+  const long long filter_violations = h[2] >> 8;
+  const bool cuttable = hubs_used && !pre.valid && h[3] >= 0 && h[3] < n_b && can_cut(n_active, filter_violations);
+  if (hubs_used && ((h[2] & 6) != 0 || ((h[2] & 16) != 0 && cuttable) || (force_cut >= 0 && cuttable))) {
+    const bool by_cost = cuttable && force_cut < 0 && (h[2] & 4) == 0 && S.hub_attempt + 1 < kHubMaxAttempts &&
+                         filter_violations <= kHubCutCap &&
+                         (long long)n_active * S.excl_edge_ns < filter_violations * S.cut_cost_ns;
+    const bool cut = cuttable && !by_cost;
+    const bool in_place = cut && S.cut_in_place;
+    const int c = cut ? h[3] : 0;
     hipLaunchKernelGGL(k_reset_cc, dim3(Blocks(n_active)), dim3(256), 0, s, n_active, S.a_ra, S.a_rb, S.cc,
                        d_violation, nullptr, 0u, nullptr);
-    hipLaunchKernelGGL(k_clear_kept, dim3(Blocks(n_b)), dim3(256), 0, s, n_b, S.masks, S.e_gpos, kept_all);
+    const int c_lo = in_place ? c : 0;
+    hipLaunchKernelGGL(k_clear_kept, dim3(Blocks(n_b - (c_lo & ~255))), dim3(256), 0, s, c_lo, n_b, S.masks, S.e_gpos,
+                       kept_all);
     clear_marks();
+    if (by_cost) {
+      ++S.cost_exclusions;
+      if (h[2] & 16) hipLaunchKernelGGL(k_hub_list_cut_hubs, dim3(1), dim3(64), 0, s, S.hub_excl, S.masks, S.e_rb, nodes);
+    }
     clear_hub_marks();
+    const int n_front = in_place ? h[4] : -1;
+    if (in_place && (n_front > 0 || (n_ti > 0 && c > 0))) {
+      hipLaunchKernelGGL(k_restore_front, dim3(Blocks(std::max(n_front, n_ti > 0 ? c : 0))), dim3(256), 0, s, n_front,
+                         n_ti > 0 ? c : 0, S.a_ra, S.a_rb, S.masks, S.e_ra, S.e_rb, nodes, S.cc, P.min_region_size);
+    }
     VSG_HIP(hipGetLastError());
-    if (retry_without_broken_hubs(kHubVioBroken, n_active, (h[2] & 4) == 0, nullptr)) return;
+    if (retry_without_broken_hubs(kHubVioBroken, n_active, (h[2] & 4) == 0, nullptr, cut ? c : -1, n_front)) return;
     VSG_REQUIRE(false, -4, "hub stage: no way to rerun it");
   }
   if (hubs_used && info) ++info->hub_stages;
@@ -1616,11 +1727,11 @@
       S.hub_list_dirty = 1;
       hipLaunchKernelGGL(k_restore_roots, dim3(Blocks(n_work)), dim3(256), 0, s, n_work, w_ra, w_rb,
                          nodes, S.bk_ds, S.bk_cons, S.bk_flags, S.stats);
-      hipLaunchKernelGGL(k_clear_kept, dim3(Blocks(n_b)), dim3(256), 0, s, n_b, S.masks, S.e_gpos, kept_all);
+      hipLaunchKernelGGL(k_clear_kept, dim3(Blocks(n_b)), dim3(256), 0, s, 0, n_b, S.masks, S.e_gpos, kept_all);
       clear_marks();
       clear_hub_marks();
       VSG_HIP(hipGetLastError());
-      if (spine && violated == 2 && bucket < 2 && !S.force_rollback && retry_without_broken_hubs(2, n_work, true, w_gpos)) {
+      if (spine && violated == 2 && bucket < 2 && !S.force_rollback && retry_without_broken_hubs(2, n_work, true, w_gpos, -1, -1)) {
         return;
       }
       if (spine && violated == 2 && !S.force_rollback) {
@@ -1642,7 +1753,7 @@
       }
       if ((violated & (kHubViolationMask | kVioCut)) != 0 && (violated & ~(kHubViolationMask | kVioCut)) == 0 &&
           !spine && !S.force_rollback) {
-        if (retry_without_broken_hubs(violated, n_work, true, w_gpos)) return;
+        if (retry_without_broken_hubs(violated, n_work, true, w_gpos, -1, -1)) return;
       }
       if (bucket_hi > bucket + 1) {
         ++S.group_halvings;
```

Result: no change. 212.0, median of 2 (-0.6%).
